# wanzysky/SlenderObjDet

Measured on AMD Instinct MI355X. Metric: training img/sec FCOS R50-FPN 1333x800, higher is better.
Workload: dtype bf16; 1 GPU; FCOS R50-FPN (FCOSV2, giou, center-sampling 1.5), fwd+bwd+SGD, synthetic 1333x800 padded to 800x1344 (BASELINE.json configs[1]); global_batch=16, parallelism=dp1

## Files before the change

### include/slender_hip.h

```cpp
#ifndef SLENDER_HIP_H_
#define SLENDER_HIP_H_

#ifdef __cplusplus
extern "C" {
#endif

#define SOD_MAX_LEVELS 8
#define SOD_CONV_MAX_LEVELS 6

#define SOD_CONV_RELU 1
#define SOD_CONV_RES_UP2 2
#define SOD_CONV_CWIN 4

#define SOD_IOU_LOSS_IOU 0
#define SOD_IOU_LOSS_LINEAR 1
#define SOD_IOU_LOSS_GIOU 2

const char* sod_version(void);
int sod_stream_create_cumask(const unsigned* mask_words, int nwords, void** out_stream);
int sod_stream_destroy(void* stream);
int sod_debug_occupy(int wgs, int usec, void* stream);

long long sod_reduce_workspace_bytes(void);

int sod_conv2d_fwd(const void* x, const void* w, const float* bias, const void* res, void* y,
                   int N, int H, int W, int C, int K, int R, int S, int stride, int pad, int dil,
                   long long x_img_stride, long long y_img_stride, long long res_img_stride,
                   int flags, int out_f32, void* stream);
int sod_conv2d_dgrad(const void* dy, const void* wt, const void* accum, const void* relu_mask, void* dx,
                     int N, int H, int W, int C, int K, int R, int S, int stride, int pad, int dil,
                     long long dy_img_stride, long long dx_img_stride, void* stream);
#define SOD_WGRAD_DETERMINISTIC 1
#define SOD_WGRAD_DIAG 2
long long sod_conv2d_wgrad_workspace_bytes(void);
int sod_conv2d_wgrad(const void* dy, const void* x, float* dw, const float* qscale,
                     int N, int H, int W, int C, int K, int R, int S, int stride, int pad, int dil,
                     long long dy_img_stride, long long x_img_stride, int splits, int flags,
                     void* ws, long long ws_bytes, void* stream);

int sod_conv2d_fwd_bits(const void* x, const void* w, const float* bias, const void* res, void* y, void* relu_bits,
                        int N, int H, int W, int C, int K, int R, int S, int stride, int pad, int dil, int flags, void* stream);
int sod_conv2d_dgrad_bits(const void* dy, const void* wt, const void* accum, int accum_even, const void* relu_bits, void* dx,
                          int N, int H, int W, int C, int K, int R, int S, int stride, int pad, int dil, void* stream);

int sod_conv2d_fwd_ml(int nlev, const void* const* x, const void* w, const float* bias, void* const* y,
                      int N, const int* H, const int* W, int C, int K, int R, int S, int stride, int pad, int dil,
                      long long y_img_stride, int flags, int out_f32, void* stream);
int sod_conv2d_fwd_ml_gnsum(int nlev, const void* const* x, const void* w, const float* bias, void* const* y,
                            int N, const int* H, const int* W, int C, int K, int R, int S, int stride, int pad, int dil,
                            long long y_img_stride, int flags, float* gn_sums, int G, void* stream);
int sod_conv2d_dgrad_ml(int nlev, const void* const* dy, const void* wt, void* const* dx,
                        int N, const int* H, const int* W, int C, int K, int R, int S, int stride, int pad, int dil,
                        long long dy_img_stride, void* stream);
int sod_conv2d_dgrad_ml_mask(int nlev, const void* const* dy, const void* wt, const void* const* relu_mask, void* const* dx,
                             int N, const int* H, const int* W, int C, int K, int R, int S, int stride, int pad, int dil,
                             long long dy_img_stride, void* stream);
int sod_conv2d_dgrad_ml_kpitch(int nlev, const void* const* dy, const void* wt_pad, void* const* dx,
                               int N, const int* H, const int* W, int C, int Kp, int Kpitch, int R, int S, int pad, int dil,
                               long long dy_img_stride, void* stream);
int sod_conv2d_dgrad_ml_accum(int nlev, const void* const* dy, const void* wt, const void* const* accum, const void* const* relu_mask,
                              void* const* dx, int N, const int* H, const int* W, int C, int K, int R, int S, int stride, int pad, int dil,
                              long long dy_img_stride, void* stream);
int sod_conv2d_wgrad_ml(int nlev, const void* const* dy, const void* const* x, float* dw, const float* qscale,
                        int N, const int* H, const int* W, int C, int K, int R, int S, int stride, int pad, int dil,
                        long long dy_img_stride, int splits, int flags, void* ws, long long ws_bytes, void* stream);
int sod_conv2d_dgrad_cwin(const void* dy, const void* wt_win, const void* relu_mask, void* dx,
                          int N, int H, int W, int C, int K, int R, int S, int stride, int pad, int dil, void* stream);
int sod_conv_set_tile256(int mode);
int sod_conv_set_pw(int on);
int sod_conv_set_ws3(int mode);
int sod_conv_set_wgrad_variant(int variant);
int sod_conv_set_reverse(int on);
int sod_conv_last_variant(void);
int sod_conv_prof_enable(int on);
int sod_conv_prof_collect(float* ms, int* variant, float* frac, int* mode, int max);

int sod_groupnorm_fwd(const void* x, const float* gamma, const float* beta, void* y, float* mean_rstd,
                      int N, int HW, int C, int G, long long img_stride, float eps, int relu,
                      float* det_ws, long long det_ws_bytes, void* stream);
int sod_groupnorm_bwd(const void* dy, const void* x, const float* gamma, const float* beta, const float* mean_rstd,
                      void* dx, float* dgamma, float* dbeta, float* dxsum , float* red_ws ,
                      int N, int HW, int C, int G, long long img_stride, int relu, float* det_ws, long long det_ws_bytes, void* stream);
int sod_groupnorm_fwd_ml(int nlev, const void* const* x, const float* gamma, const float* beta, void* const* y, float* mean_rstd,
                         int N, const int* hw, int C, int G, float eps, int relu, float* det_ws, long long det_ws_bytes, void* stream);
int sod_groupnorm_apply_ml(int nlev, const void* const* x, const float* gamma, const float* beta, void* const* y, float* sums_to_mean_rstd,
                           int N, const int* hw, int C, int G, float eps, int relu, void* stream);
int sod_groupnorm_bwd_ml(int nlev, const void* const* dy, const void* const* x, const float* gamma, const float* beta,
                         const float* mean_rstd, void* const* dx, float* dgamma, float* dbeta, float* dxsum, float* red_ws,
                         int N, const int* hw, int C, int G, int relu, float* det_ws, long long det_ws_bytes, void* stream);

int sod_relu_fwd(const void* x, void* y, long long n, void* stream);
int sod_relu_bwd(const void* dy, const void* y, void* dx, long long n, void* stream);
int sod_add_bf16(const void* a, const void* b, void* out, long long n, void* stream);
int sod_add_up2_bf16(const void* a, const void* b, void* out, int N, int H, int W, int C, void* stream);
int sod_bias_grad(const void* dy, float* dbias, int N, int HW, int C, long long img_stride, float* det_ws, long long det_ws_bytes, void* stream);
int sod_bias_grad_scaled(const void* dy, float* dbias, const float* scale_num, const float* scale_den, float den_mul, float den_min,
                         int N, int HW, int C, long long img_stride, float* det_ws, long long det_ws_bytes, void* stream);
int sod_bias_grad_ml(int nlev, const void* const* dy, float* dbias, int N, const int* hw, int C, void* stream);
int sod_maxpool3x3s2(const void* x, void* y, int N, int H, int W, int C, void* stream);
int sod_upsample2x_bwd(const void* g, void* dprev, int N, int Hc, int Wc, int C, void* stream);

int sod_weight_prep(const float* w, const float* scale, void* w_krsc, void* w_crsk, int K, int RS, int C, int Cpad, void* stream);
int sod_weight_prep_batched(const float* params, const float* scales, const void* table_dev, int n, long long total_elems,
                            void* krsc_arena, void* crsk_arena, void* stream);
int sod_scale_rows(float* g, const float* scale, int K, long long row, void* stream);

int sod_sgd_step(float* params, const float* grads, float* momentum_buf, const void* segments_dev, int nseg,
                 const float* lr_dev, float lr, float momentum, int nesterov, int first_step, float grad_scale, void* stream);

int sod_adaptive_step(float* params, const float* grads, float* exp_avg, float* exp_avg_sq, const void* segments_dev, int nseg,
                      int mode, float lr, float beta1, float beta2, float eps, float bias_correction1, float bias_correction2_sqrt,
                      float grad_scale, void* stream);

int sod_preprocess_image(const void* img, int is_uint8, int C, int H, int W, void* out, int Hp, int Wp, int Cpad,
                         const float* mean3, const float* std3, void* stream);
int sod_preprocess_batch(int n, const void* const* imgs, int is_uint8, int C, const int* H, const int* W, void* out, int Hp, int Wp,
                         int Cpad, const float* mean3, const float* std3, void* stream);
int sod_stem_fused(int n, const void* const* imgs, const int* H, const int* W, const void* w_packed, const float* bias,
                   void* out, int Hp, int Wp, const float* mean3, const float* std3, void* stream);
int sod_bottleneck_frozen_fwd(const void* x, int N, int H, int W, int Cin, const void* w1, const float* b1, const void* w2,
                              const float* b2, const void* w3, const float* b3, const void* wsc, void* out, void* stream);
int sod_resize_flip_preprocess_batch(int n, const void* const* imgs, const int* H, const int* W, const int* newH, const int* newW,
                                     const int* const* xbounds, const int* const* xcoef, const int* kx,
                                     const int* const* ybounds, const int* const* ycoef, const int* ky, const int* flip,
                                     void* out, int Hp, int Wp, int Cpad, const float* mean3, const float* std3, void* stream);
int sod_nchw_f32_to_nhwc_bf16(const float* x, void* y, int N, int C, int HW, void* stream);

int sod_sigmoid_focal_loss_fwd(const float* logits, const int* labels, const float* dense_targets,
                               long long M, int K, int ld, float alpha, float gamma, float* elem_out,
                               float* sum_out, float* ws, void* stream);
int sod_sigmoid_focal_loss_fwd_grad(const float* logits, const int* labels, long long M, int K, int ld, float alpha, float gamma,
                                    float* sum_out, float* ws, void* dlogits_bf16, int ld_out, void* stream);
int sod_sigmoid_focal_loss_bwd(const float* logits, const int* labels, const float* dense_targets,
                               long long M, int K, int ld, float alpha, float gamma,
                               const float* scale_num, const float* scale_den, float den_mul, float den_min,
                               void* dlogits, int ld_out, int out_bf16, void* stream);
int sod_iou_loss_fwd(const float* pred, const float* target, const float* weight, const int* mask, int mask_bg,
                     long long P, int loss_type, float* elem_out, float* sum_out, float* ws, void* stream);
int sod_iou_loss_bwd(const float* pred, const float* target, const float* weight, const int* mask, int mask_bg,
                     long long P, int loss_type, const float* grad_scale, float* dpred, void* stream);
int sod_fcos_assign(const float* boxes, const int* classes, const int* box_offsets, int N,
                    int nlevels, const int* lvl_h, const int* lvl_w, const int* lvl_stride,
                    const float* lvl_lo, const float* lvl_hi, float radius, int num_classes,
                    int* labels, float* reg_targets, float* ctr_targets, float* stats, float* ws, void* stream);
int sod_fcos_regctr_loss_fwd(const float* box_raw, int ld_box, const float* ctr_logit, int ld_ctr,
                             const int* labels, const float* reg_targets, const float* ctr_targets,
                             const float* scales, int N, int nlevels, const int* lvl_h, const int* lvl_w,
                             const int* lvl_stride, int num_classes, int loss_type, int norm_reg_targets,
                             float* sums, float* ws, void* stream);
int sod_fcos_regctr_loss_bwd(const float* box_raw, int ld_box, const float* ctr_logit, int ld_ctr,
                             const int* labels, const float* reg_targets, const float* ctr_targets,
                             const float* scales, int N, int nlevels, const int* lvl_h, const int* lvl_w,
                             const int* lvl_stride, int num_classes, int loss_type, int norm_reg_targets,
                             const float* grad_reg, const float* grad_ctr, const float* norm, float inv_world,
                             void* dbox, int ld_out, int ctr_col, void* dctr, int ld_dctr, int dctr_col,
                             float* dscales, float* ws, void* stream);
int sod_fcos_assign_topk(const float* boxes, const int* classes, const int* box_offsets, int N,
                         int nlevels, const int* lvl_h, const int* lvl_w, const int* lvl_stride,
                         const float* lvl_lo, const float* lvl_hi, float radius, int num_classes, int topk,
                         int* labels, float* reg_targets, float* ctr_targets, int* gt_index, unsigned char* sel,
                         float* stats3, float* ws, void* stream);
int sod_fcos_regctr_loss_sel_fwd(const float* box_raw, int ld_box, const float* ctr_logit, int ld_ctr,
                                 const int* labels, const float* reg_targets, const float* ctr_targets,
                                 const float* scales, int N, int nlevels, const int* lvl_h, const int* lvl_w,
                                 const int* lvl_stride, int num_classes, int loss_type, int norm_reg_targets,
                                 const unsigned char* sel, float* sums, float* ws, void* stream);
int sod_fcos_regctr_loss_sel_bwd(const float* box_raw, int ld_box, const float* ctr_logit, int ld_ctr,
                                 const int* labels, const float* reg_targets, const float* ctr_targets,
                                 const float* scales, int N, int nlevels, const int* lvl_h, const int* lvl_w,
                                 const int* lvl_stride, int num_classes, int loss_type, int norm_reg_targets,
                                 const unsigned char* sel,
                                 const float* grad_reg, const float* grad_ctr, const float* norm, float inv_world,
                                 void* dbox, int ld_out, int ctr_col, void* dctr, int ld_dctr, int dctr_col,
                                 float* dscales, float* ws, void* stream);
int sod_fcos_finalize_losses(const float* focal_sum, const float* regctr_sums, const float* stats,
                             float inv_world, float* out3, void* stream);

long long sod_nms_workspace_bytes(int n);
int sod_nms(const float* boxes, const long long* order, int n, float iou_threshold, long long* keep, int* num_keep,
            void* mask_ws, void* stream);
int sod_fcos_decode(const float* cls_logits, int ld_cls, const float* box_raw, int ld_box, const float* scales,
                    int N, int nlev, const int* H, const int* W, const int* strides, int num_classes,
                    int ctr_col_box, int ctr_col_cls, int norm_reg_targets, float pre_nms_thresh, int pre_nms_top_n,
                    float* out_boxes, float* out_scores, int* out_classes, int* out_counts, void* stream);
int sod_dense_topk_select(const float* logits, int ld, int N, int nlev, const int* rows, int num_classes, int by_row_max,
                          float score_thresh, int top_n, int* out_rows, float* out_scores, int* out_classes, int* out_counts, void* stream);
long long sod_batched_nms_workspace_bytes(int B, int M, int box_dim);
int sod_batched_nms_prepare(const float* boxes, const float* scores, const int* classes, int B, int M, int box_dim, void* ws, void* stream);
int sod_batched_nms_run(const long long* order, int B, int M, int box_dim, float iou_threshold, int max_keep, long long* keep, int* num_keep,
                        void* ws, void* stream);
int sod_rpn_clip_filter(float* boxes, float* scores, const float* image_hw, int B, int M, int box_dim, float min_size, int* bad_count,
                        void* stream);
int sod_nms_rotated(const float* boxes, const long long* order, int n, float iou_threshold, long long* keep, int* num_keep,
                    void* mask_ws, void* stream);
int sod_box_iou_rotated(const float* boxes1, int n1, const float* boxes2, int n2, float* iou_out, void* stream);
int sod_roi_align_fwd(const void* x, const float* rois, float* out, int R, int N, int H, int W, int C, int PH, int PW,
                      float spatial_scale, int sampling_ratio, int rotated, void* stream);
int sod_roi_align_fwd_f32(const float* x, const float* rois, float* out, int R, int N, int H, int W, int C, int PH, int PW,
                          float spatial_scale, int sampling_ratio, int rotated, void* stream);
int sod_roi_align_bwd(const float* dout, const float* rois, float* dx, int R, int N, int H, int W, int C, int PH, int PW,
                      float spatial_scale, int sampling_ratio, int rotated, void* stream);
int sod_giou_loss_xyxy(const float* boxes1, const float* boxes2, long long P, float eps, float* elem_out, float* sum_out,
                       const float* grad_scale, float* dboxes1, float* ws, void* stream);
int sod_smooth_l1_loss(const float* input, const float* target, long long n, float beta, float* elem_out, float* sum_out,
                       const float* grad_scale, float* dinput, float* ws, void* stream);
int sod_anchor_match(const float* gt_boxes, int G, const float* anchors, int A, float thr_lo, float thr_hi,
                     int label_below, int label_between, int label_above, int allow_low_quality,
                     float* matched_vals, int* matches, signed char* labels, unsigned* gt_best_ws, void* stream);

int sod_deform_conv_fwd_fused(const void* x, const float* offset, const float* mask, const void* w, const float* bias, void* y,
                              int N, int H, int W, int C, int K, int KH, int KW, int stride, int pad, int dil, int deformable_groups,
                              int off_ld, int mask_ld, int mask_is_logit, int relu, void* stream);
int sod_deform_conv_fwd_f32(const float* x, const float* offset, const float* mask, const float* w, const float* bias, float* y,
                            int N, int H, int W, int C, int K, int KH, int KW, int stride, int pad, int dil, int deformable_groups,
                            int off_ld, int mask_ld, int mask_is_logit, void* stream);
int sod_deform_conv_wgrad_fused(const void* dy, const void* x, const float* offset, const float* mask, float* dw, const float* qscale,
                                int N, int H, int W, int C, int K, int KH, int KW, int stride, int pad, int dil, int deformable_groups,
                                int off_ld, int mask_ld, int mask_is_logit, void* ws, long long ws_bytes, void* stream);
int sod_deform_im2col(const void* x, const float* offset, const float* mask, void* cols,
                      int N, int H, int W, int C, int KH, int KW, int stride, int pad, int dil, int deformable_groups,
                      int off_ld, int mask_ld, int mask_is_logit, void* stream);
int sod_deform_conv_bwd_fused(const void* dy, const void* wt, const void* x, const float* offset, const float* mask, float* dx_f32,
                              float* doffset, float* dmask, float* wnorm_ws, int N, int H, int W, int C, int K, int KH, int KW, int stride,
                              int pad, int dil, int deformable_groups, int off_ld, int mask_ld, int mask_is_logit, void* stream);
int sod_deform_conv_set_window_counter(unsigned long long* device_counter);
int sod_deform_conv_set_window_slack(int pixels);
int sod_deform_conv_bwd_fused_supported(int C, int K, int KH, int KW, int stride, int dil, int deformable_groups);
int sod_deform_col2im(const void* dcols, const void* x, const float* offset, const float* mask,
                      float* dx_f32, float* doffset, float* dmask,
                      int N, int H, int W, int C, int KH, int KW, int stride, int pad, int dil, int deformable_groups,
                      int off_ld, int mask_ld, int mask_is_logit, void* stream);

int sod_deform_im2col_f32(const float* x, const float* offset, const float* mask, float* cols,
                          int N, int H, int W, int C, int KH, int KW, int stride, int pad, int dil, int deformable_groups,
                          int off_ld, int mask_ld, int mask_is_logit, void* stream);
int sod_deform_col2im_f32(const float* dcols, const float* x, const float* offset, const float* mask,
                          float* dx_f32, float* doffset, float* dmask,
                          int N, int H, int W, int C, int KH, int KW, int stride, int pad, int dil, int deformable_groups,
                          int off_ld, int mask_ld, int mask_is_logit, void* stream);
int sod_f32_to_bf16(const float* x, void* y, long long n, void* stream);

int sod_retina_targets(const float* anchors, int A, const float* gt_boxes, const int* gt_classes, int G, const int* matches,
                       const signed char* match_labels, int num_classes, const float* weights4, int* gt_labels, float* gt_deltas,
                       void* stream);
int sod_retina_box_loss_fwd(const float* pred, int pitch, const int* gt_labels, const float* gt_deltas, int N, int R, int A,
                            int num_classes, float beta, float* sums2, float* normalizer, float momentum, float* ws, void* stream);
int sod_retina_box_loss_bwd(const float* pred, int pitch, const int* gt_labels, const float* gt_deltas, int N, int R, int A,
                            int num_classes, float beta, const float* grad_num, const float* grad_den, void* dpred_bf16, void* stream);

int sod_anchor_match_rotated(const float* gt_boxes, int G, const float* anchors, int A, float thr_lo, float thr_hi,
                             int label_below, int label_between, int label_above, int allow_low_quality,
                             float* matched_vals, int* matches, signed char* labels, unsigned* gt_best_ws, void* stream);
int sod_roi_label_batched(const float* boxes, const int* counts, int N, int R, int box_dim, const float* gt_boxes, const int* gt_classes,
                          const int* gt_off, float iou_threshold, int label_below, int label_above, int num_classes, int* matches,
                          signed char* classes, void* stream);
int sod_box2box_get_deltas(const float* src, const float* tgt, long long n, int box_dim, const float* weights, float* deltas, void* stream);
int sod_box2box_apply_deltas(const float* deltas, const float* boxes, long long n, int k, int box_dim, int ld, const float* weights,
                             float scale_clamp, float* out, void* stream);
int sod_bce_logits_loss_fwd(const float* logits, const signed char* labels, long long n, float* sum_out, float* ws, void* stream);
int sod_bce_logits_loss_bwd(const float* logits, const signed char* labels, long long n, const float* grad_scale, float scale_mul,
                            float* dlogits, void* stream);
int sod_bce_logits_soft_fwd(const float* logits, const float* targets, const int* labels, int bg_label, long long n, float* sum_out,
                            float* ws, void* stream);
int sod_bce_logits_soft_bwd(const float* logits, const float* targets, const int* labels, int bg_label, long long n,
                            const float* grad_scale, float scale_mul, float* dlogits, void* stream);
int sod_rpn_loc_loss_fwd(const float* pred, const float* target, const signed char* labels, long long n, int box_dim, float beta,
                         float* sum_out, float* ws, void* stream);
int sod_rpn_loc_loss_bwd(const float* pred, const float* target, const signed char* labels, long long n, int box_dim, float beta,
                         const float* grad_scale, float scale_mul, float* dpred, void* stream);
int sod_softmax_ce_fwd(const float* scores, const int* labels, int R, int C, int ld, float* sum_out, float* ws, void* stream);
int sod_softmax_ce_bwd(const float* scores, const int* labels, int R, int C, int ld, const float* grad_scale, float scale_mul,
                       float* dscores, void* stream);
int sod_fastrcnn_box_loss_fwd(const float* pred, const int* gt_classes, const float* gt_deltas, int R, int K, int box_dim, int ld,
                              float beta, float* sum_out, float* ws, void* stream);
int sod_fastrcnn_box_loss_bwd(const float* pred, const int* gt_classes, const float* gt_deltas, int R, int K, int box_dim, int ld,
                              float beta, const float* grad_scale, float scale_mul, float* dpred, void* stream);

int sod_reppoints_dcn_offset(const float* pts, float* out, long long rows, int ld, int num_points, float scale, int subtract_base,
                             int flip_xy, void* stream);
int sod_points2bbox_fwd(const float* pts, const float* add, int ld, int N, int H, int W, float grid_stride, float point_stride,
                        int num_points, float* boxes, long long box_img_stride, unsigned* argidx, long long arg_img_stride, void* stream);
int sod_points2bbox_bwd(const float* dboxes, long long box_img_stride, const unsigned* argidx, long long arg_img_stride, int ld,
                        int N, int H, int W, float point_stride, int num_points, float* dpts_f32, void* dpts_bf16, void* stream);
int sod_points2bbox_moment_fwd(const float* pts, const float* add, int ld, int N, int H, int W, float grid_stride, float point_stride,
                               int num_points, const float* moment_transfer, float* boxes, long long box_img_stride, void* stream);
int sod_points2bbox_moment_bwd(const float* dboxes, long long box_img_stride, const float* pts, const float* add, int ld, int N, int H,
                               int W, float grid_stride, float point_stride, int num_points, const float* moment_transfer,
                               float moment_mul, float* dpts_f32, void* dpts_bf16, float* dmoment2, void* stream);
int sod_reppoints_point_match(const float* centers, const float* strides, int X, const int* lvl_start, int num_levels,
                              const float* gt_boxes, const int* box_offsets, int N, int max_gt, int mode, float scale,
                              int* objectness, float* box_labels, void* stream);
int sod_reppoints_labels(const int* matches, const signed char* match_labels, const float* gt_boxes, const int* gt_classes,
                         const int* box_offsets, const float* centers, const float* image_hw, int N, int X, int num_classes,
                         int* cls_labels, float* refine_boxes, int* objectness, void* stream);
int sod_reppoints_box_loss_fwd(const float* pred, const float* target, const int* labels, const float* strides, int N, int X,
                               int bg_label, float beta, float* sums2, float* ws, void* stream);
int sod_reppoints_box_loss_bwd(const float* pred, const float* target, const int* labels, const float* strides, int N, int X,
                               int bg_label, float beta, const float* grad_num, const float* grad_den, float den_min, float mul,
                               float* dpred, void* stream);
int sod_reppoints_finalize(const float* focal_sum, const float* init_sums2, const float* refine_sums2, float* normalizer,
                           float momentum, int num_images, float init_weight, float* out3, void* stream);

int sod_retina_giou_loss_fwd(const float* pred, int pitch, const int* gt_labels, const float* anchors, const float* matched_boxes,
                             int N, int R, int A, int num_classes, const float* weights4, float scale_clamp, float* sums2,
                             float* normalizer, float momentum, float* ws, void* stream);
int sod_retina_giou_loss_bwd(const float* pred, int pitch, const int* gt_labels, const float* anchors, const float* matched_boxes,
                             int N, int R, int A, int num_classes, const float* weights4, float scale_clamp,
                             const float* grad_num, const float* grad_den, void* dpred_bf16, void* stream);

int sod_border_align_fwd(const float* feature, const float* boxes, float* out, int B, int C, int K, int H, int W, int pool_size,
                         void* stream);
int sod_border_align_bwd(const float* dout, const float* feature, const float* boxes, float* dfeature, int B, int C, int K, int H,
                         int W, int pool_size, void* stream);
int sod_corner_pool_fwd(const float* x, float* y, long long planes, int H, int W, int mode, void* stream);
int sod_corner_pool_bwd(const float* x, const float* dy, float* dx, long long planes, int H, int W, int mode, int tie_latest,
                        void* stream);

int sod_sample_labels(const signed char* labels, int N, int R, int num_samples, float positive_fraction, int bg_label,
                      unsigned long long seed, signed char* out, int* counts, void* stream);
int sod_sample_labels_list(const signed char* labels, int N, int R, int num_samples, float positive_fraction, int bg_label,
                           unsigned long long seed, signed char* out, int* counts, int* idx, int* list_n, void* stream);
int sod_compact_samples(const signed char* mask, int N, int R, int S, int* idx, int* num, void* stream);

int sod_rpn_gather_sampled(int nlev, const void* const* logits, const void* const* deltas, const int* hw, const int* logit_pitch,
                           const int* delta_pitch, const int* idx, int N, int S, int A, int D, float* row_logits, float* row_deltas,
                           void* stream);
int sod_rpn_scatter_sampled(int nlev, void* const* dlogits, void* const* ddeltas, const int* hw, const int* logit_pitch,
                            const int* delta_pitch, const int* idx, int N, int S, int A, int D, const float* row_dlogits,
                            const float* row_ddeltas, void* stream);

int sod_conv2d_fwd_f32(const float* x, const float* w_krsc, const float* bias, const float* res, float* y, int N, int H, int W, int C, int K,
                       int R, int S, int stride, int pad, int dil, long long x_img_stride, long long y_img_stride, int flags, void* stream);
int sod_conv2d_dgrad_f32(const float* dy, const float* w_krsc, const float* accum, const float* relu_mask, float* dx, int N, int H, int W, int C,
                         int K, int R, int S, int stride, int pad, int dil, long long dy_img_stride, int accum_even, void* stream);
int sod_conv2d_wgrad_f32(const float* dy, const float* x, float* dw, const float* qscale, int N, int H, int W, int C, int K, int R, int S,
                         int stride, int pad, int dil, long long dy_img_stride, long long x_img_stride, void* stream);
int sod_groupnorm_fwd_f32(const float* x, const float* gamma, const float* beta, float* y, float* mean_rstd, int N, int HW, int C, int G,
                          float eps, int relu, void* stream);
int sod_groupnorm_bwd_f32(const float* dy, const float* x, const float* gamma, const float* beta, const float* mean_rstd, float* dx,
                          float* dgamma, float* dbeta, float* dxsum, int N, int HW, int C, int G, int relu, void* stream);
int sod_eltwise_f32(int op, const float* a, const float* b, float* out, long long n, void* stream);
int sod_add_up2_f32(const float* a, const float* b, float* out, int N, int H, int W, int C, void* stream);
int sod_upsample2x_bwd_f32(const float* g, float* dprev, int N, int Hc, int Wc, int C, void* stream);
int sod_maxpool3x3s2_f32(const float* x, float* y, int N, int H, int W, int C, void* stream);
int sod_bias_grad_f32(const float* dy, float* dbias, int N, int HW, int C, long long img_stride, void* stream);
int sod_preprocess_image_f32(const void* img, int is_uint8, int C, int H, int W, float* out, int Hp, int Wp, int Cpad, const float* mean3,
                             const float* std3, void* stream);
int sod_weight_prep_f32(const float* w, const float* scale, float* w_krsc, float* w_crsk, int K, int RS, int C, int Cpad, void* stream);
int sod_retina_box_loss_bwd_f32(const float* pred, int pitch, const int* gt_labels, const float* gt_deltas, int N, int R, int A,
                                int num_classes, float beta, const float* grad_num, const float* grad_den, float* dpred, void* stream);
int sod_retina_giou_loss_bwd_f32(const float* pred, int pitch, const int* gt_labels, const float* anchors, const float* matched_boxes,
                                 int N, int R, int A, int num_classes, const float* weights4, float scale_clamp,
                                 const float* grad_num, const float* grad_den, float* dpred, void* stream);
int sod_fcos_regctr_loss_bwd_f32(const float* box_raw, int ld_box, const float* ctr_logit, int ld_ctr, const int* labels,
                                 const float* reg_targets, const float* ctr_targets, const float* scales, int N, int nlevels, const int* lvl_h,
                                 const int* lvl_w, const int* lvl_stride, int num_classes, int loss_type, int norm_reg_targets,
                                 const float* grad_reg, const float* grad_ctr, const float* norm, float inv_world, void* dbox, int ld_out,
                                 int ctr_col, void* dctr, int ld_dctr, int dctr_col, float* dscales, float* ws, void* stream);
int sod_fcos_regctr_loss_sel_bwd_f32(const float* box_raw, int ld_box, const float* ctr_logit, int ld_ctr, const int* labels,
                                     const float* reg_targets, const float* ctr_targets, const float* scales, int N, int nlevels,
                                     const int* lvl_h, const int* lvl_w, const int* lvl_stride, int num_classes, int loss_type,
                                     int norm_reg_targets, const unsigned char* sel, const float* grad_reg, const float* grad_ctr,
                                     const float* norm, float inv_world, void* dbox, int ld_out, int ctr_col, void* dctr, int ld_dctr,
                                     int dctr_col, float* dscales, float* ws, void* stream);

long long sod_coco_match_scratch_doubles(int num_gts, int max_det);
int sod_coco_match(const int* gt_off, const double* gt_box, const unsigned char* gt_crowd, const double* gt_ratio, const int* dt_off,
                   const float* dt_box, int num_seg, int num_img, int max_det, const double* iou_thr, int T, const double* ranges, int A,
                   const long long* scratch_off, double* scratch, unsigned long long* dt_matched, unsigned long long* dt_ignored,
                   int* npig, void* stream);
int sod_coco_accumulate(const int* cat_off, const long long* order, const float* score, const int* rank,
                        const unsigned long long* dt_matched, const unsigned long long* dt_ignored, const int* npig, int K, int T, int A,
                        const int* max_dets, int M, const double* rec_thr, int R, double* precision, double* recall, double* scores,
                        void* stream);
long long sod_proposal_ar_scratch_floats(int num_gts, int limit);
int sod_proposal_ar(const int* gt_off, const float* gt_box, const int* gt_cls, const float* gt_ratio, const int* dt_off,
                    const long long* dt_order, const float* dt_box, const int* dt_cls, int num_img, int limit, int K1, const float* thr,
                    int T, const float* ratio_rng, int R, const float* area_rng, int A, const long long* scratch_off, float* scratch,
                    int* hits, int* counts, float* recalls, void* stream);

long long sod_coco_match_rotated_scratch_floats(int num_gts, int max_det);
int sod_coco_match_rotated(const int* gt_off, const float* gt_box5, const unsigned char* gt_crowd, const double* gt_val,
                           const int* dt_off, const float* dt_box5, const double* dt_val, int num_seg, int num_img, int max_det,
                           const double* iou_thr, int T, const double* ranges, int A, const long long* scratch_off, float* scratch,
                           unsigned long long* dt_matched, unsigned long long* dt_ignored, int* npig, void* stream);

#ifdef __cplusplus
}
#endif
#endif
```

### slenderobjdet_amd/_C.py

```python
import ctypes
import os
from ctypes import c_char_p, c_float, c_int, c_longlong, c_void_p

_HERE = os.path.dirname(os.path.abspath(__file__))
LIB_PATH = os.environ.get("SOD_HIP_LIB") or os.path.join(_HERE, "libslender_hip.so")

_lib = None

_P = c_void_p
_I = c_int
_L = c_longlong
_F = c_float

_SIGS = {
    "sod_conv2d_fwd": [_P, _P, _P, _P, _P, _I, _I, _I, _I, _I, _I, _I, _I, _I, _I, _L, _L, _L, _I, _I, _P],
    "sod_conv2d_dgrad": [_P, _P, _P, _P, _P, _I, _I, _I, _I, _I, _I, _I, _I, _I, _I, _L, _L, _P],
    "sod_conv2d_fwd_bits": [_P, _P, _P, _P, _P, _P, _I, _I, _I, _I, _I, _I, _I, _I, _I, _I, _I, _P],
    "sod_conv2d_dgrad_bits": [_P, _P, _P, _I, _P, _P, _I, _I, _I, _I, _I, _I, _I, _I, _I, _I, _P],
    "sod_conv2d_wgrad": [_P, _P, _P, _P, _I, _I, _I, _I, _I, _I, _I, _I, _I, _I, _L, _L, _I, _I, _P, _L, _P],
    "sod_conv2d_wgrad_workspace_bytes": [],
    "sod_conv2d_fwd_ml": [_I, _P, _P, _P, _P, _I, _P, _P, _I, _I, _I, _I, _I, _I, _I, _L, _I, _I, _P],
    "sod_conv2d_fwd_ml_gnsum": [_I, _P, _P, _P, _P, _I, _P, _P, _I, _I, _I, _I, _I, _I, _I, _L, _I, _P, _I, _P],
    "sod_groupnorm_apply_ml": [_I, _P, _P, _P, _P, _P, _I, _P, _I, _I, _F, _I, _P],
    "sod_conv2d_dgrad_ml": [_I, _P, _P, _P, _I, _P, _P, _I, _I, _I, _I, _I, _I, _I, _L, _P],
    "sod_conv2d_dgrad_ml_mask": [_I, _P, _P, _P, _P, _I, _P, _P, _I, _I, _I, _I, _I, _I, _I, _L, _P],
    "sod_conv2d_dgrad_ml_kpitch": [_I, _P, _P, _P, _I, _P, _P, _I, _I, _I, _I, _I, _I, _I, _L, _P],
    "sod_conv2d_dgrad_ml_accum": [_I, _P, _P, _P, _P, _P, _I, _P, _P, _I, _I, _I, _I, _I, _I, _I, _L, _P],
    "sod_conv2d_wgrad_ml": [_I, _P, _P, _P, _P, _I, _P, _P, _I, _I, _I, _I, _I, _I, _I, _L, _I, _I, _P, _L, _P],
    "sod_groupnorm_fwd": [_P, _P, _P, _P, _P, _I, _I, _I, _I, _L, _F, _I, _P, _L, _P],
    "sod_groupnorm_bwd": [_P, _P, _P, _P, _P, _P, _P, _P, _P, _P, _I, _I, _I, _I, _L, _I, _P, _L, _P],
    "sod_groupnorm_fwd_ml": [_I, _P, _P, _P, _P, _P, _I, _P, _I, _I, _F, _I, _P, _L, _P],
    "sod_groupnorm_bwd_ml": [_I, _P, _P, _P, _P, _P, _P, _P, _P, _P, _P, _I, _P, _I, _I, _I, _P, _L, _P],
    "sod_relu_fwd": [_P, _P, _L, _P],
    "sod_relu_bwd": [_P, _P, _P, _L, _P],
    "sod_add_bf16": [_P, _P, _P, _L, _P],
    "sod_add_up2_bf16": [_P, _P, _P, _I, _I, _I, _I, _P],
    "sod_bias_grad": [_P, _P, _I, _I, _I, _L, _P, _L, _P],
    "sod_bias_grad_scaled": [_P, _P, _P, _P, _F, _F, _I, _I, _I, _L, _P, _L, _P],
    "sod_bias_grad_ml": [_I, _P, _P, _I, _P, _I, _P],
    "sod_maxpool3x3s2": [_P, _P, _I, _I, _I, _I, _P],
    "sod_upsample2x_bwd": [_P, _P, _I, _I, _I, _I, _P],
    "sod_conv2d_dgrad_cwin": [_P, _P, _P, _P, _I, _I, _I, _I, _I, _I, _I, _I, _I, _I, _P],
    "sod_conv_set_tile256": [_I],
    "sod_conv_set_pw": [_I],
    "sod_conv_set_ws3": [_I],
    "sod_conv_set_wgrad_variant": [_I],
    "sod_conv_set_reverse": [_I],
    "sod_conv_last_variant": [],
    "sod_conv_prof_enable": [_I],
    "sod_conv_prof_collect": [_P, _P, _P, _P, _I],
    "sod_weight_prep_batched": [_P, _P, _P, _I, _L, _P, _P, _P],
    "sod_weight_prep": [_P, _P, _P, _P, _I, _I, _I, _I, _P],
    "sod_scale_rows": [_P, _P, _I, _L, _P],
    "sod_sgd_step": [_P, _P, _P, _P, _I, _P, _F, _F, _I, _I, _F, _P],
    "sod_adaptive_step": [_P, _P, _P, _P, _P, _I, _I, _F, _F, _F, _F, _F, _F, _F, _P],
    "sod_preprocess_image": [_P, _I, _I, _I, _I, _P, _I, _I, _I, _P, _P, _P],
    "sod_preprocess_batch": [_I, _P, _I, _I, _P, _P, _P, _I, _I, _I, _P, _P, _P],
    "sod_nchw_f32_to_nhwc_bf16": [_P, _P, _I, _I, _I, _P],
    "sod_stem_fused": [_I, _P, _P, _P, _P, _P, _P, _I, _I, _P, _P, _P],
    "sod_bottleneck_frozen_fwd": [_P, _I, _I, _I, _I, _P, _P, _P, _P, _P, _P, _P, _P, _P],
    "sod_resize_flip_preprocess_batch": [_I, _P, _P, _P, _P, _P, _P, _P, _P, _P, _P, _P, _P, _P, _I, _I, _I, _P, _P, _P],
    "sod_sigmoid_focal_loss_fwd": [_P, _P, _P, _L, _I, _I, _F, _F, _P, _P, _P, _P],
    "sod_sigmoid_focal_loss_fwd_grad": [_P, _P, _L, _I, _I, _F, _F, _P, _P, _P, _I, _P],
    "sod_sigmoid_focal_loss_bwd": [_P, _P, _P, _L, _I, _I, _F, _F, _P, _P, _F, _F, _P, _I, _I, _P],
    "sod_iou_loss_fwd": [_P, _P, _P, _P, _I, _L, _I, _P, _P, _P, _P],
    "sod_iou_loss_bwd": [_P, _P, _P, _P, _I, _L, _I, _P, _P, _P],
    "sod_fcos_assign": [_P, _P, _P, _I, _I, _P, _P, _P, _P, _P, _F, _I, _P, _P, _P, _P, _P, _P],
    "sod_fcos_regctr_loss_fwd": [_P, _I, _P, _I, _P, _P, _P, _P, _I, _I, _P, _P, _P, _I, _I, _I, _P, _P, _P],
    "sod_fcos_regctr_loss_bwd": [_P, _I, _P, _I, _P, _P, _P, _P, _I, _I, _P, _P, _P, _I, _I, _I, _P, _P, _P, _F,
                                 _P, _I, _I, _P, _I, _I, _P, _P, _P],
    "sod_fcos_assign_topk": [_P, _P, _P, _I, _I, _P, _P, _P, _P, _P, _F, _I, _I, _P, _P, _P, _P, _P, _P, _P, _P],
    "sod_fcos_regctr_loss_sel_fwd": [_P, _I, _P, _I, _P, _P, _P, _P, _I, _I, _P, _P, _P, _I, _I, _I, _P, _P, _P, _P],
    "sod_fcos_regctr_loss_sel_bwd": [_P, _I, _P, _I, _P, _P, _P, _P, _I, _I, _P, _P, _P, _I, _I, _I, _P, _P, _P, _P, _F,
                                     _P, _I, _I, _P, _I, _I, _P, _P, _P],
    "sod_fcos_finalize_losses": [_P, _P, _P, _F, _P, _P],
    "sod_nms_workspace_bytes": [_I],
    "sod_fcos_decode": [_P, _I, _P, _I, _P, _I, _I, _P, _P, _P, _I, _I, _I, _I, _F, _I, _P, _P, _P, _P, _P],
    "sod_dense_topk_select": [_P, _I, _I, _I, _P, _I, _I, _F, _I, _P, _P, _P, _P, _P],
    "sod_batched_nms_workspace_bytes": [_I, _I, _I],
    "sod_batched_nms_prepare": [_P, _P, _P, _I, _I, _I, _P, _P],
    "sod_batched_nms_run": [_P, _I, _I, _I, _F, _I, _P, _P, _P, _P],
    "sod_rpn_clip_filter": [_P, _P, _P, _I, _I, _I, _F, _P, _P],
    "sod_nms": [_P, _P, _I, _F, _P, _P, _P, _P],
    "sod_nms_rotated": [_P, _P, _I, _F, _P, _P, _P, _P],
    "sod_box_iou_rotated": [_P, _I, _P, _I, _P, _P],
    "sod_roi_align_fwd": [_P, _P, _P, _I, _I, _I, _I, _I, _I, _I, _F, _I, _I, _P],
    "sod_roi_align_fwd_f32": [_P, _P, _P, _I, _I, _I, _I, _I, _I, _I, _F, _I, _I, _P],
    "sod_roi_align_bwd": [_P, _P, _P, _I, _I, _I, _I, _I, _I, _I, _F, _I, _I, _P],
    "sod_giou_loss_xyxy": [_P, _P, _L, _F, _P, _P, _P, _P, _P, _P],
    "sod_smooth_l1_loss": [_P, _P, _L, _F, _P, _P, _P, _P, _P, _P],
    "sod_anchor_match": [_P, _I, _P, _I, _F, _F, _I, _I, _I, _I, _P, _P, _P, _P, _P],
    "sod_retina_targets": [_P, _I, _P, _P, _I, _P, _P, _I, _P, _P, _P, _P],
    "sod_retina_box_loss_fwd": [_P, _I, _P, _P, _I, _I, _I, _I, _F, _P, _P, _F, _P, _P],
    "sod_retina_giou_loss_fwd": [_P, _I, _P, _P, _P, _I, _I, _I, _I, _P, _F, _P, _P, _F, _P, _P],
    "sod_retina_giou_loss_bwd": [_P, _I, _P, _P, _P, _I, _I, _I, _I, _P, _F, _P, _P, _P, _P],
    "sod_retina_box_loss_bwd": [_P, _I, _P, _P, _I, _I, _I, _I, _F, _P, _P, _P, _P],
    "sod_deform_conv_fwd_fused": [_P, _P, _P, _P, _P, _P, _I, _I, _I, _I, _I, _I, _I, _I, _I, _I, _I, _I, _I, _I, _I, _P],
    "sod_deform_conv_fwd_f32": [_P, _P, _P, _P, _P, _P, _I, _I, _I, _I, _I, _I, _I, _I, _I, _I, _I, _I, _I, _I, _P],
    "sod_deform_conv_wgrad_fused": [_P, _P, _P, _P, _P, _P, _I, _I, _I, _I, _I, _I, _I, _I, _I, _I, _I, _I, _I, _I, _P, _L, _P],
    "sod_deform_im2col": [_P, _P, _P, _P, _I, _I, _I, _I, _I, _I, _I, _I, _I, _I, _I, _I, _I, _P],
    "sod_deform_col2im": [_P, _P, _P, _P, _P, _P, _P, _I, _I, _I, _I, _I, _I, _I, _I, _I, _I, _I, _I, _I, _P],
    "sod_deform_im2col_f32": [_P, _P, _P, _P, _I, _I, _I, _I, _I, _I, _I, _I, _I, _I, _I, _I, _I, _P],
    "sod_deform_col2im_f32": [_P, _P, _P, _P, _P, _P, _P, _I, _I, _I, _I, _I, _I, _I, _I, _I, _I, _I, _I, _I, _P],
    "sod_deform_conv_set_window_counter": [_P],
    "sod_deform_conv_set_window_slack": [_I],
    "sod_deform_conv_bwd_fused_supported": [_I, _I, _I, _I, _I, _I, _I],
    "sod_deform_conv_bwd_fused": [_P, _P, _P, _P, _P, _P, _P, _P, _P, _I, _I, _I, _I, _I, _I, _I, _I, _I, _I, _I, _I, _I, _I, _P],
    "sod_f32_to_bf16": [_P, _P, _L, _P],
    "sod_border_align_fwd": [_P, _P, _P, _I, _I, _I, _I, _I, _I, _P],
    "sod_border_align_bwd": [_P, _P, _P, _P, _I, _I, _I, _I, _I, _I, _P],
    "sod_corner_pool_fwd": [_P, _P, _L, _I, _I, _I, _P],
    "sod_corner_pool_bwd": [_P, _P, _P, _L, _I, _I, _I, _I, _P],
    "sod_anchor_match_rotated": [_P, _I, _P, _I, _F, _F, _I, _I, _I, _I, _P, _P, _P, _P, _P],
    "sod_box2box_get_deltas": [_P, _P, _L, _I, _P, _P, _P],
    "sod_box2box_apply_deltas": [_P, _P, _L, _I, _I, _I, _P, _F, _P, _P],
    "sod_bce_logits_loss_fwd": [_P, _P, _L, _P, _P, _P],
    "sod_bce_logits_loss_bwd": [_P, _P, _L, _P, _F, _P, _P],
    "sod_bce_logits_soft_fwd": [_P, _P, _P, _I, _L, _P, _P, _P],
    "sod_bce_logits_soft_bwd": [_P, _P, _P, _I, _L, _P, _F, _P, _P],
    "sod_rpn_loc_loss_fwd": [_P, _P, _P, _L, _I, _F, _P, _P, _P],
    "sod_rpn_loc_loss_bwd": [_P, _P, _P, _L, _I, _F, _P, _F, _P, _P],
    "sod_softmax_ce_fwd": [_P, _P, _I, _I, _I, _P, _P, _P],
    "sod_softmax_ce_bwd": [_P, _P, _I, _I, _I, _P, _F, _P, _P],
    "sod_fastrcnn_box_loss_fwd": [_P, _P, _P, _I, _I, _I, _I, _F, _P, _P, _P],
    "sod_fastrcnn_box_loss_bwd": [_P, _P, _P, _I, _I, _I, _I, _F, _P, _F, _P, _P],
    "sod_reppoints_dcn_offset": [_P, _P, _L, _I, _I, _F, _I, _I, _P],
    "sod_points2bbox_fwd": [_P, _P, _I, _I, _I, _I, _F, _F, _I, _P, _L, _P, _L, _P],
    "sod_points2bbox_bwd": [_P, _L, _P, _L, _I, _I, _I, _I, _F, _I, _P, _P, _P],
    "sod_points2bbox_moment_fwd": [_P, _P, _I, _I, _I, _I, _F, _F, _I, _P, _P, _L, _P],
    "sod_points2bbox_moment_bwd": [_P, _L, _P, _P, _I, _I, _I, _I, _F, _F, _I, _P, _F, _P, _P, _P, _P],
    "sod_reppoints_point_match": [_P, _P, _I, _P, _I, _P, _P, _I, _I, _I, _F, _P, _P, _P],
    "sod_reppoints_labels": [_P, _P, _P, _P, _P, _P, _P, _I, _I, _I, _P, _P, _P, _P],
    "sod_reppoints_box_loss_fwd": [_P, _P, _P, _P, _I, _I, _I, _F, _P, _P, _P],
    "sod_reppoints_box_loss_bwd": [_P, _P, _P, _P, _I, _I, _I, _F, _P, _P, _F, _F, _P, _P],
    "sod_reppoints_finalize": [_P, _P, _P, _P, _F, _I, _F, _P, _P],
    "sod_conv2d_fwd_f32": [_P, _P, _P, _P, _P, _I, _I, _I, _I, _I, _I, _I, _I, _I, _I, _L, _L, _I, _P],
    "sod_conv2d_dgrad_f32": [_P, _P, _P, _P, _P, _I, _I, _I, _I, _I, _I, _I, _I, _I, _I, _L, _I, _P],
    "sod_conv2d_wgrad_f32": [_P, _P, _P, _P, _I, _I, _I, _I, _I, _I, _I, _I, _I, _I, _L, _L, _P],
    "sod_groupnorm_fwd_f32": [_P, _P, _P, _P, _P, _I, _I, _I, _I, _F, _I, _P],
    "sod_groupnorm_bwd_f32": [_P, _P, _P, _P, _P, _P, _P, _P, _P, _I, _I, _I, _I, _I, _P],
    "sod_eltwise_f32": [_I, _P, _P, _P, _L, _P],
    "sod_add_up2_f32": [_P, _P, _P, _I, _I, _I, _I, _P],
    "sod_upsample2x_bwd_f32": [_P, _P, _I, _I, _I, _I, _P],
    "sod_maxpool3x3s2_f32": [_P, _P, _I, _I, _I, _I, _P],
    "sod_bias_grad_f32": [_P, _P, _I, _I, _I, _L, _P],
    "sod_preprocess_image_f32": [_P, _I, _I, _I, _I, _P, _I, _I, _I, _P, _P, _P],
    "sod_weight_prep_f32": [_P, _P, _P, _P, _I, _I, _I, _I, _P],
    "sod_fcos_regctr_loss_bwd_f32": [_P, _I, _P, _I, _P, _P, _P, _P, _I, _I, _P, _P, _P, _I, _I, _I, _P, _P, _P, _F,
                                     _P, _I, _I, _P, _I, _I, _P, _P, _P],
    "sod_fcos_regctr_loss_sel_bwd_f32": [_P, _I, _P, _I, _P, _P, _P, _P, _I, _I, _P, _P, _P, _I, _I, _I, _P, _P, _P, _P, _F,
                                         _P, _I, _I, _P, _I, _I, _P, _P, _P],
    "sod_sample_labels": [_P, _I, _I, _I, _F, _I, ctypes.c_ulonglong, _P, _P, _P],
    "sod_sample_labels_list": [_P, _I, _I, _I, _F, _I, ctypes.c_ulonglong, _P, _P, _P, _P, _P],
    "sod_compact_samples": [_P, _I, _I, _I, _P, _P, _P],
    "sod_roi_label_batched": [_P, _P, _I, _I, _I, _P, _P, _P, _F, _I, _I, _I, _P, _P, _P],
    "sod_rpn_gather_sampled": [_I, _P, _P, _P, _P, _P, _P, _I, _I, _I, _I, _P, _P, _P],
    "sod_rpn_scatter_sampled": [_I, _P, _P, _P, _P, _P, _P, _I, _I, _I, _I, _P, _P, _P],
    "sod_retina_box_loss_bwd_f32": [_P, _I, _P, _P, _I, _I, _I, _I, _F, _P, _P, _P, _P],
    "sod_retina_giou_loss_bwd_f32": [_P, _I, _P, _P, _P, _I, _I, _I, _I, _P, _F, _P, _P, _P, _P],
    "sod_reduce_workspace_bytes": [],
    "sod_version": [],
    "sod_stream_create_cumask": [_P, _I, _P],
    "sod_stream_destroy": [_P],
    "sod_debug_occupy": [_I, _I, _P],
    "sod_coco_match_scratch_doubles": [_I, _I],
    "sod_coco_match": [_P, _P, _P, _P, _P, _P, _I, _I, _I, _P, _I, _P, _I, _P, _P, _P, _P, _P, _P],
    "sod_coco_accumulate": [_P, _P, _P, _P, _P, _P, _P, _I, _I, _I, _P, _I, _P, _I, _P, _P, _P, _P],
    "sod_proposal_ar_scratch_floats": [_I, _I],
    "sod_proposal_ar": [_P, _P, _P, _P, _P, _P, _P, _P, _I, _I, _I, _P, _I, _P, _I, _P, _I, _P, _P, _P, _P, _P, _P],
    "sod_coco_match_rotated_scratch_floats": [_I, _I],
    "sod_coco_match_rotated": [_P, _P, _P, _P, _P, _P, _P, _I, _I, _I, _P, _I, _P, _I, _P, _P, _P, _P, _P, _P],
}
_RESTYPES = {"sod_reduce_workspace_bytes": c_longlong, "sod_conv2d_wgrad_workspace_bytes": c_longlong, "sod_nms_workspace_bytes": c_longlong, "sod_batched_nms_workspace_bytes": c_longlong, "sod_version": c_char_p,
             "sod_coco_match_scratch_doubles": c_longlong, "sod_proposal_ar_scratch_floats": c_longlong,
             "sod_coco_match_rotated_scratch_floats": c_longlong}


class SlenderHipError(RuntimeError):
    pass


def exported_symbols():
    return sorted(_SIGS)


def load():
    global _lib
    if _lib is not None:
        return _lib
    if not os.path.exists(LIB_PATH):
        raise SlenderHipError(
            f"{LIB_PATH} is missing: build it with `python -c 'import __graft_entry__ as g; g.build()'` "
            "(make -C slenderobjdet_amd/csrc). There is no CPU fallback for the HIP ops."
        )
    import torch

    lib = ctypes.CDLL(LIB_PATH)
    for name, argtypes in _SIGS.items():
        fn = getattr(lib, name)
        fn.argtypes = argtypes
        fn.restype = _RESTYPES.get(name, c_int)
    _lib = lib
    return lib


_ERRS = {-1: "SOD_EARG (bad argument / unsupported shape)", -2: "SOD_ESIZE (operand exceeds 2 GiB)", -3: "SOD_EALIGN"}


def call(name, *args):
    rc = getattr(load(), name)(*args)
    if rc != 0:
        raise SlenderHipError(f"{name} failed: {_ERRS.get(rc, 'hipError_t %d' % rc)}")


def ptr(t):
    if t is None:
        return None
    return ctypes.c_void_p(t.data_ptr())


def stream_ptr(stream=None):
    import torch

    return ctypes.c_void_p((stream if stream is not None else torch.cuda.current_stream()).cuda_stream)


def reduce_workspace_floats():
    return int(load().sod_reduce_workspace_bytes()) // 4
```

### slenderobjdet_amd/csrc/conv_args.h

```cpp
#pragma once
#include "common.h"
#include "../../include/slender_hip.h"
#include <stdlib.h>

namespace sodconv {

enum { MODE_FWD = 0, MODE_DGRAD = 1 };
enum {
  F_BIAS = 1, F_RELU = 2, F_RES = 4, F_RES_UP2 = 8, F_MASK = 16,
  F_WBITS = 64,
  F_MASKBITS = 128,
  F_GNSTATS = 32,
  F_REVERSE = 1024,
  F_RES_EVEN = 512,
};
constexpr int MAXLEV = SOD_CONV_MAX_LEVELS;

struct LevelGeo {
  const void* src;
  void* dst;
  const void* res;
  const void* mask;
  void* bits;
  float* gn_sum;
  uint32_t src_bytes;
  int Hs, Ws, Hp, Wp, P;
  int tile0;
  int pstart;
  int src_img_stride, dst_img_stride, res_img_stride;
  FastDiv div_hw, div_w;
};

struct ConvArgs {
  LevelGeo lev[MAXLEV];
  int nlev;
  const void* w;
  const float* bias;
  uint32_t w_bytes;
  int N, Cred, Nout;
  int R, S, stride, pad, dil;
  int Kred, T;
  int flags;
  int nq_tiles, np_tiles;
  FastDiv div_cpt , div_s, div_stride;
  FastDiv div_rs;
  int gn_G;
  int tap_inner;
  int Cpitch;
  int cwin;
};

inline int conv_tap_inner(int dflt) { return dflt; }

struct GnAcc {
  float s, ss;
  int n;
};
__device__ __forceinline__ void gn_acc_flush(const GnAcc& g, float* sums, int G, int grp) {
  if (g.n >= 0) {
    atomicAdd(sums + ((size_t)g.n * G + grp) * 2, g.s);
    atomicAdd(sums + ((size_t)g.n * G + grp) * 2 + 1, g.ss);
  }
}
__device__ __forceinline__ void gn_acc_add(GnAcc& g, int n, const bf16x8_t& o, float* sums, int G, int grp) {
  float s = 0.f, ss = 0.f;
#pragma unroll
  for (int e = 0; e < 8; ++e) { const float f = (float)o[e]; s += f; ss += f * f; }
  if (n != g.n) { gn_acc_flush(g, sums, G, grp); g.n = n; g.s = 0.f; g.ss = 0.f; }
  g.s += s; g.ss += ss;
}
template <int LPR>
__device__ __forceinline__ void gn_acc_finish(GnAcc& g, uint32_t pa, uint32_t pb, uint32_t P, const FastDiv& div_hw, float* sums, int G, int grp,
                                              bool qok, int lane) {
  if (pa >= P) return;
  if (pb >= P) pb = P - 1;
  const int na = (int)fd_div(pa, div_hw), nb = (int)fd_div(pb, div_hw);
  if (na == nb) {
    float s = (g.n >= 0) ? g.s : 0.f, ss = (g.n >= 0) ? g.ss : 0.f;
#pragma unroll
    for (int o = LPR; o < 64; o <<= 1) { s += __shfl_xor(s, o, 64); ss += __shfl_xor(ss, o, 64); }
    if (lane < LPR && qok) {
      atomicAdd(sums + ((size_t)na * G + grp) * 2, s);
      atomicAdd(sums + ((size_t)na * G + grp) * 2 + 1, ss);
    }
  } else if (qok) {
    gn_acc_flush(g, sums, G, grp);
  }
}

enum ConvTile { TILE_16x256, TILE_64x256, TILE_64x256_K32, TILE_128x128, TILE_128x128_K32 };
int launch_conv128(const ConvArgs& a, int mode, bool out_f32, ConvTile tile, bool generic, hipStream_t st, int* variant);

bool conv256_supported(const ConvArgs& a, int mode);
int launch_conv256(const ConvArgs& a, int mode, bool out_f32, int max_pt_tiles, hipStream_t st);

bool pw_supported(const ConvArgs& a, int mode, bool out_f32, int cus);
int launch_pw(const ConvArgs& a, int mode, hipStream_t st);

bool ws3_supported(const ConvArgs& a, int mode, bool out_f32, int cus, bool any_size);
int launch_ws3(const ConvArgs& a, int mode, hipStream_t st);

struct WLevel {
  const void* dy;
  const void* x;
  uint32_t dy_bytes, x_bytes;
  int Hx, Wx, Ho, Wo, P;
  int v0;
  int dy_img_stride, x_img_stride;
  FastDiv div_hw, div_w;
};

struct WgradArgs {
  WLevel lev[MAXLEV];
  int nlev;
  float* dw;
  const float* qscale;
  int dbg_plain_store;
  float* partial;
  int det;
  int N, C, K;
  int R, S, stride, pad, dil;
  int V, nz, v_per_split;
  int QT, CT;
  FastDiv div_s;
  int diag;
};

enum { WGRAD_DETERMINISTIC = 1, WGRAD_DIAG = 2 };

int launch_wgrad128(WgradArgs& a, int cus, int splits, float* ws, long long ws_bytes, hipStream_t st);
int launch_wgrad_reduce(const WgradArgs& a, hipStream_t st);

bool wgrad256_supported(const WgradArgs& a);
long long wgrad256_workspace_bytes(const WgradArgs& a, int cus);
int launch_wgrad256(WgradArgs& a, int cus, float* ws, long long ws_bytes, hipStream_t st);

bool wgrad9_supported(const WgradArgs& a);
long long wgrad9_workspace_bytes(const WgradArgs& a, int cus);
int wgrad9_tiles_per_block(const WgradArgs& a, int cus);
int launch_wgrad9(const WgradArgs& a, int cus, float* ws, long long ws_bytes, hipStream_t st);

bool wgrad_fold_supported(const WgradArgs& a);
int launch_wgrad_fold(WgradArgs& a, int cus, hipStream_t st);

int launch_wgrad_ring(const WgradArgs& a, int variant, hipStream_t st);

}
```

### slenderobjdet_amd/csrc/conv_dispatch.hip

```cpp
#include "conv_args.h"
#include <stdlib.h>
#include <atomic>
#include <algorithm>

using namespace sodconv;

int device_cus() {
  static const int cus = [] {
    int dev = 0, n = 0;
    if (hipGetDevice(&dev) != hipSuccess || hipDeviceGetAttribute(&n, hipDeviceAttributeMultiprocessorCount, dev) != hipSuccess || n <= 0) n = 256;
    return n;
  }();
  return cus;
}

namespace {

thread_local int g_last_variant = 0;
thread_local int g_conv_reverse = 0;

struct ConvKnobs {
  int conv256 = -1;
  int pw = -1;
  int ws3 = -1;
// ... 185 lines not shown
}

int dispatch_wgrad(WgradArgs& a, int splits, int flags, hipStream_t st, float* ws, long long ws_bytes) {
  const int cus = device_cus();
  a.det = (flags & WGRAD_DETERMINISTIC) ? 1 : 0;
  a.diag = (flags & WGRAD_DIAG) ? 1 : 0;
  if (a.diag && (a.C != a.K || (a.C & 127) || splits < 0)) return SOD_EARG;
  if (splits == -2 && (!ws || !wgrad9_supported(a) || wgrad9_workspace_bytes(a, cus) > ws_bytes)) return SOD_EARG;
  if (splits == -2 || (splits == 0 && use_wgrad9(a, ws, ws_bytes)))
    return timed(st, 9009, 1.f, 2, [&] { return launch_wgrad9(a, cus, ws, ws_bytes, st); });
  if (splits == -1 && (!ws || !wgrad256_supported(a) || wgrad256_workspace_bytes(a, cus) > ws_bytes)) return SOD_EARG;
  if (splits == -1 || (splits == 0 && !a.diag && use_wgrad256(a, ws, ws_bytes)))
    return timed(st, 256, 1.f, 2, [&] { return launch_wgrad256(a, cus, ws, ws_bytes, st); });
  if (splits == 0 && wgrad_fold_supported(a))
    return timed(st, 32004, 1.f, 2, [&] { return launch_wgrad_fold(a, cus, st); });
  a.QT = (a.K + 127) / 128; a.CT = a.diag ? 1 : (a.C + 127) / 128;
  const int tiles = a.QT * a.CT * a.R * a.S;
  int V = 0;
  long long Ptot = 0;
  for (int l = 0; l < a.nlev; ++l) {
    a.lev[l].v0 = V;
    V += (a.lev[l].P + 63) / 64 * 64;
    Ptot += a.lev[l].P;
  }
  a.V = V;
  const int variant = ring_variant_for(a, tiles, splits, ws, ws_bytes);
  if (variant > 0) {
    const int G = (variant % 10000) / 1000;
    int epi = (variant / 10) % 10;
    long long total = splits > 0 ? splits : (long long)G * std::max(1, (G == 1 ? 2 : 1) * cus / tiles);
    const long long maxs = (Ptot + 255) / 256;
    if (total > maxs) total = maxs;
    if (total < 1) total = 1;
    int vps = (int)((V + total - 1) / total);
    vps = (vps + 63) / 64 * 64;
    const int nsplit = (V + vps - 1) / vps;
    a.v_per_split = vps;
    a.nz = (nsplit + G - 1) / G;
    a.dbg_plain_store = 0;
    const long long need = (long long)a.nz * tiles * 128 * 128 * (long long)sizeof(float);
    if (a.det || epi == 1) {
      if (!ws || need > ws_bytes) {
        if (a.det) return SOD_EARG;
        epi = 0;
      }
    }
    a.partial = (a.det || epi == 1) ? ws : nullptr;
    const int v = variant - ((variant / 10) % 10) * 10 + (a.partial ? 10 : 0);
    return timed(st, v % 10000, 1.f, 2, [&] {
      const int rc = launch_wgrad_ring(a, v, st);
      return rc || !a.partial ? rc : launch_wgrad_reduce(a, st);
    });
  }
  return timed(st, 32003, 1.f, 2, [&] { return launch_wgrad128(a, cus, splits, ws, ws_bytes, st); });
}

int fill_wlevel(WgradArgs& a, int l, const void* dy, const void* x, int H, int W, long long dy_img_stride, long long x_img_stride) {
  if (!dy || !x || H <= 0 || W <= 0) return SOD_EARG;
  const int Ho = out_size(H, a.pad, a.dil, a.R, a.stride), Wo = out_size(W, a.pad, a.dil, a.S, a.stride);
  if (Ho <= 0 || Wo <= 0) return SOD_EARG;
  if (dy_img_stride <= 0) dy_img_stride = (long long)Ho * Wo * a.K;
  if (x_img_stride <= 0) x_img_stride = (long long)H * W * a.C;
  const unsigned long long yb = (unsigned long long)a.N * dy_img_stride * 2ull, xb = (unsigned long long)a.N * x_img_stride * 2ull;
  if (yb >= 0x80000000ull || xb >= 0x80000000ull || (long long)a.N * Ho * Wo >= (1ll << 30)) return SOD_ESIZE;
  WLevel& g = a.lev[l];
  g.dy = dy; g.x = x; g.dy_bytes = (uint32_t)yb; g.x_bytes = (uint32_t)xb;
  g.Hx = H; g.Wx = W; g.Ho = Ho; g.Wo = Wo; g.P = a.N * Ho * Wo;
  g.dy_img_stride = (int)dy_img_stride; g.x_img_stride = (int)x_img_stride;
  g.div_hw = make_fastdiv((uint32_t)(Ho * Wo));
  g.div_w = make_fastdiv((uint32_t)Wo);
  return SOD_OK;
}


struct Geo {
  int N;
  const int *H, *W;
  int C, K, R, S, stride, pad, dil;
};

bool out_positive(const Geo& g, int l) {
  return out_size(g.H[l], g.pad, g.dil, g.R, g.stride) > 0 && out_size(g.W[l], g.pad, g.dil, g.S, g.stride) > 0;
}

struct FwdExtra {
  const void* res = nullptr;
  long long res_img_stride = 0;
  void* relu_bits = nullptr;
  float* gn_sums = nullptr;
  int G = 0;
  long long x_img_stride = 0;
  bool reverse = false;
};

int conv_fwd(int nlev, const void* const* x, const void* w, const float* bias, void* const* y, const Geo& g, long long y_img_stride,
             int flags, int out_f32, const FwdExtra& e, void* stream) {
  ConvArgs a{};
  const bool cwin = (flags & SOD_CONV_CWIN) != 0;
  int rc = fill_common(a, nlev, g.N, cwin ? 128 : g.C, g.K, g.R, g.S, g.stride, g.pad, g.dil);
  if (rc) return rc;
  if (cwin) { a.Cpitch = g.C; a.cwin = 1; }
  for (int l = 0; l < nlev; ++l) {
    if (!out_positive(g, l)) return SOD_EARG;
    rc = fill_level(a, l, x[l], y[l], g.H[l], g.W[l], out_size(g.H[l], g.pad, g.dil, g.R, g.stride), out_size(g.W[l], g.pad, g.dil, g.S, g.stride),
                    e.x_img_stride, y_img_stride, out_f32 ? 4 : 2);
    if (rc) return rc;
    if (e.gn_sums) a.lev[l].gn_sum = e.gn_sums + (size_t)l * g.N * e.G * 2;
  }
  a.w = w; a.bias = bias;
  a.gn_G = e.G;
  a.flags = (bias ? F_BIAS : 0) | ((flags & SOD_CONV_RELU) ? F_RELU : 0) | (e.gn_sums ? F_GNSTATS : 0);
  if (e.res) {
    LevelGeo& v = a.lev[0];
    v.res = e.res;
    if (flags & SOD_CONV_RES_UP2) {
      if ((v.Hp & 1) || (v.Wp & 1)) return SOD_EARG;
      a.flags |= F_RES_UP2;
      v.res_img_stride = (int)(e.res_img_stride > 0 ? e.res_img_stride : (long long)(v.Hp / 2) * (v.Wp / 2) * g.K);
    } else {
      a.flags |= F_RES;
      v.res_img_stride = (int)(e.res_img_stride > 0 ? e.res_img_stride : v.dst_img_stride);
    }
  }
  if (e.relu_bits) { a.flags |= F_WBITS; a.lev[0].bits = e.relu_bits; }
  if (e.reverse) a.flags |= F_REVERSE;
  hipStream_t st = (hipStream_t)stream;
  if (e.gn_sums) {
    hipError_t err = hipMemsetAsync(e.gn_sums, 0, sizeof(float) * 2 * (size_t)g.N * e.G * nlev, st);
    if (err != hipSuccess) return (int)err;
  }
  return dispatch_conv(a, MODE_FWD, out_f32 != 0, st);
}

struct DgradExtra {
  const void* const* accum = nullptr;
  bool accum_even = false;
  const void* const* mask = nullptr;
  bool mask_bits = false;
  int Cpitch = 0;
  bool cwin = false;
  long long dx_img_stride = 0;
  bool reverse = false;
};

int conv_dgrad(int nlev, const void* const* dy, const void* wt, void* const* dx, const Geo& g, long long dy_img_stride, const DgradExtra& e,
               void* stream) {
  ConvArgs a{};
  int rc = fill_common(a, nlev, g.N, g.K, g.C, g.R, g.S, g.stride, g.pad, g.dil);
  if (rc) return rc;
  if (e.Cpitch > 0) a.Cpitch = e.Cpitch;
  a.cwin = e.cwin ? 1 : 0;
  for (int l = 0; l < nlev; ++l) {
    if (!out_positive(g, l) || (e.accum && !e.accum[l]) || (e.mask && !e.mask[l])) return SOD_EARG;
    rc = fill_level(a, l, dy[l], dx[l], out_size(g.H[l], g.pad, g.dil, g.R, g.stride), out_size(g.W[l], g.pad, g.dil, g.S, g.stride), g.H[l], g.W[l],
                    dy_img_stride, e.dx_img_stride, 2);
    if (rc) return rc;
    LevelGeo& v = a.lev[l];
    if (e.accum) { v.res = e.accum[l]; v.res_img_stride = e.accum_even ? (g.H[l] / 2) * (g.W[l] / 2) * g.C : v.dst_img_stride; }
    if (e.mask) v.mask = e.mask[l];
  }
  a.w = wt; a.bias = nullptr;
  a.flags = (e.accum ? (e.accum_even ? F_RES_UP2 | F_RES_EVEN : F_RES) : 0) | (e.mask ? (e.mask_bits ? F_MASKBITS : F_MASK) : 0) |
            (e.reverse ? F_REVERSE : 0);
  return dispatch_conv(a, MODE_DGRAD, false, (hipStream_t)stream);
}

int conv_wgrad(int nlev, const void* const* dy, const void* const* x, float* dw, const float* qscale, const Geo& g, long long dy_img_stride,
               long long x_img_stride, int splits, int flags, void* ws, long long ws_bytes, void* stream) {
  if (!dy || !x || !dw || !g.H || !g.W || nlev <= 0 || nlev > MAXLEV || ws_bytes < 0 || ((uintptr_t)ws & 15)) return SOD_EARG;
  if (g.N <= 0 || g.C <= 0 || g.K <= 0 || (g.C & 7) || (g.K & 7) || g.R <= 0 || g.S <= 0 || g.stride <= 0 || g.dil <= 0 || g.pad < 0) return SOD_EARG;
  WgradArgs a{};
  a.nlev = nlev; a.dw = dw; a.qscale = qscale; a.N = g.N; a.C = g.C; a.K = g.K;
  a.R = g.R; a.S = g.S; a.stride = g.stride; a.pad = g.pad; a.dil = g.dil;
  for (int l = 0; l < nlev; ++l) {
    const int rc = fill_wlevel(a, l, dy[l], x[l], g.H[l], g.W[l], dy_img_stride, x_img_stride);
    if (rc) return rc;
  }
  return dispatch_wgrad(a, splits, flags, (hipStream_t)stream, (float*)ws, ws ? ws_bytes : 0);
}

}

extern "C" int sod_conv2d_fwd(const void* x, const void* w, const float* bias, const void* res, void* y,
                              int N, int H, int W, int C, int K, int R, int S, int stride, int pad, int dil,
                              long long x_img_stride, long long y_img_stride, long long res_img_stride,
                              int flags, int out_f32, void* stream) {
  const Geo g{N, &H, &W, C, K, R, S, stride, pad, dil};
  if (!x || !w || !y || !out_positive(g, 0)) return SOD_EARG;
  if ((flags & SOD_CONV_CWIN) && (C != K || (C & 127))) return SOD_EARG;
  FwdExtra e;
  e.res = res; e.res_img_stride = res_img_stride; e.x_img_stride = x_img_stride; e.reverse = g_conv_reverse != 0;
  return conv_fwd(1, &x, w, bias, &y, g, y_img_stride, flags, out_f32, e, stream);
}

extern "C" int sod_conv2d_fwd_bits(const void* x, const void* w, const float* bias, const void* res, void* y, void* relu_bits,
                                   int N, int H, int W, int C, int K, int R, int S, int stride, int pad, int dil, int flags, void* stream) {
  const Geo g{N, &H, &W, C, K, R, S, stride, pad, dil};
  if (!relu_bits || !x || !w || !y || (K & 7) || !out_positive(g, 0)) return SOD_EARG;
  if (flags & SOD_CONV_CWIN) return SOD_EARG;
  FwdExtra e;
  e.res = res; e.relu_bits = relu_bits; e.reverse = g_conv_reverse != 0;
  return conv_fwd(1, &x, w, bias, &y, g, 0, flags, 0, e, stream);
}

extern "C" int sod_conv2d_fwd_ml(int nlev, const void* const* x, const void* w, const float* bias, void* const* y,
                                 int N, const int* H, const int* W, int C, int K, int R, int S, int stride, int pad, int dil,
                                 long long y_img_stride, int flags, int out_f32, void* stream) {
  if (!x || !w || !y || !H || !W) return SOD_EARG;
  return conv_fwd(nlev, x, w, bias, y, Geo{N, H, W, C, K, R, S, stride, pad, dil}, y_img_stride, flags & SOD_CONV_RELU, out_f32, FwdExtra{}, stream);
}

extern "C" int sod_conv2d_fwd_ml_gnsum(int nlev, const void* const* x, const void* w, const float* bias, void* const* y,
                                       int N, const int* H, const int* W, int C, int K, int R, int S, int stride, int pad, int dil,
                                       long long y_img_stride, int flags, float* gn_sums, int G, void* stream) {
  if (!x || !w || !y || !H || !W || !gn_sums) return SOD_EARG;
  if (G <= 0 || K != G * 8) return SOD_EARG;
  FwdExtra e;
  e.gn_sums = gn_sums; e.G = G;
  return conv_fwd(nlev, x, w, bias, y, Geo{N, H, W, C, K, R, S, stride, pad, dil}, y_img_stride, flags & SOD_CONV_RELU, 0, e, stream);
}

extern "C" int sod_conv2d_dgrad(const void* dy, const void* wt, const void* accum, const void* relu_mask, void* dx,
                                int N, int H, int W, int C, int K, int R, int S, int stride, int pad, int dil,
                                long long dy_img_stride, long long dx_img_stride, void* stream) {
  const Geo g{N, &H, &W, C, K, R, S, stride, pad, dil};
  if (!dy || !wt || !dx || !out_positive(g, 0)) return SOD_EARG;
  DgradExtra e;
  e.accum = accum ? &accum : nullptr; e.mask = relu_mask ? &relu_mask : nullptr;
  e.dx_img_stride = dx_img_stride; e.reverse = g_conv_reverse != 0;
  return conv_dgrad(1, &dy, wt, &dx, g, dy_img_stride, e, stream);
}

extern "C" int sod_conv2d_dgrad_cwin(const void* dy, const void* wt_win, const void* relu_mask, void* dx,
                                     int N, int H, int W, int C, int K, int R, int S, int stride, int pad, int dil, void* stream) {
  const Geo g{N, &H, &W, C, 128, R, S, stride, pad, dil};
  if (!dy || !wt_win || !dx || C != K || (C & 127) || !out_positive(g, 0)) return SOD_EARG;
  DgradExtra e;
  e.mask = relu_mask ? &relu_mask : nullptr; e.Cpitch = K; e.cwin = true;
  return conv_dgrad(1, &dy, wt_win, &dx, g, 0, e, stream);
}

extern "C" int sod_conv2d_dgrad_bits(const void* dy, const void* wt, const void* accum, int accum_even, const void* relu_bits, void* dx,
                                     int N, int H, int W, int C, int K, int R, int S, int stride, int pad, int dil, void* stream) {
  const Geo g{N, &H, &W, C, K, R, S, stride, pad, dil};
  if (!dy || !wt || !dx || !relu_bits || (C & 7)) return SOD_EARG;
  if (accum_even && (!accum || (H & 1) || (W & 1))) return SOD_EARG;
  if (!out_positive(g, 0)) return SOD_EARG;
  DgradExtra e;
  e.accum = accum ? &accum : nullptr; e.accum_even = accum_even != 0;
  e.mask = &relu_bits; e.mask_bits = true;
  return conv_dgrad(1, &dy, wt, &dx, g, 0, e, stream);
}

extern "C" int sod_conv2d_dgrad_ml(int nlev, const void* const* dy, const void* wt, void* const* dx,
                                   int N, const int* H, const int* W, int C, int K, int R, int S, int stride, int pad, int dil,
                                   long long dy_img_stride, void* stream) {
  if (!dy || !wt || !dx || !H || !W) return SOD_EARG;
  return conv_dgrad(nlev, dy, wt, dx, Geo{N, H, W, C, K, R, S, stride, pad, dil}, dy_img_stride, DgradExtra{}, stream);
}

extern "C" int sod_conv2d_dgrad_ml_mask(int nlev, const void* const* dy, const void* wt, const void* const* relu_mask, void* const* dx,
                                        int N, const int* H, const int* W, int C, int K, int R, int S, int stride, int pad, int dil,
                                        long long dy_img_stride, void* stream) {
  if (!dy || !wt || !dx || !relu_mask || !H || !W) return SOD_EARG;
  DgradExtra e;
  e.mask = relu_mask;
  return conv_dgrad(nlev, dy, wt, dx, Geo{N, H, W, C, K, R, S, stride, pad, dil}, dy_img_stride, e, stream);
}

extern "C" int sod_conv2d_dgrad_ml_kpitch(int nlev, const void* const* dy, const void* wt_pad, void* const* dx,
                                          int N, const int* H, const int* W, int C, int Kp, int Kpitch, int R, int S, int pad, int dil,
                                          long long dy_img_stride, void* stream) {
  if (!dy || !wt_pad || !dx || !H || !W || Kpitch <= 0 || (Kpitch & 7) || Kp < Kpitch || (Kp & 63)) return SOD_EARG;
  DgradExtra e;
  e.Cpitch = Kpitch;
  return conv_dgrad(nlev, dy, wt_pad, dx, Geo{N, H, W, C, Kp, R, S, 1, pad, dil}, dy_img_stride, e, stream);
}

extern "C" int sod_conv2d_dgrad_ml_accum(int nlev, const void* const* dy, const void* wt, const void* const* accum, const void* const* relu_mask,
                                         void* const* dx, int N, const int* H, const int* W, int C, int K, int R, int S, int stride, int pad, int dil,
                                         long long dy_img_stride, void* stream) {
  if (!dy || !wt || !dx || !accum || !H || !W) return SOD_EARG;
  DgradExtra e;
  e.accum = accum; e.mask = relu_mask;
  return conv_dgrad(nlev, dy, wt, dx, Geo{N, H, W, C, K, R, S, stride, pad, dil}, dy_img_stride, e, stream);
}

extern "C" int sod_conv2d_wgrad(const void* dy, const void* x, float* dw, const float* qscale,
                                int N, int H, int W, int C, int K, int R, int S, int stride, int pad, int dil,
                                long long dy_img_stride, long long x_img_stride, int splits, int flags,
                                void* ws, long long ws_bytes, void* stream) {
  return conv_wgrad(1, &dy, &x, dw, qscale, Geo{N, &H, &W, C, K, R, S, stride, pad, dil}, dy_img_stride, x_img_stride, splits, flags, ws, ws_bytes,
                    stream);
}

extern "C" long long sod_conv2d_wgrad_workspace_bytes(void) { return 160ll << 20; }

extern "C" int sod_conv2d_wgrad_ml(int nlev, const void* const* dy, const void* const* x, float* dw, const float* qscale,
                                   int N, const int* H, const int* W, int C, int K, int R, int S, int stride, int pad, int dil,
                                   long long dy_img_stride, int splits, int flags, void* ws, long long ws_bytes, void* stream) {
  return conv_wgrad(nlev, dy, x, dw, qscale, Geo{N, H, W, C, K, R, S, stride, pad, dil}, dy_img_stride, 0, splits, flags, ws, ws_bytes, stream);
}

extern "C" int sod_conv_last_variant(void) { return g_last_variant; }

extern "C" int sod_conv_prof_enable(int on) {
  ConvProf& p = g_prof;
  if (on && !p.ev) {
    constexpr int CAP = 8192;
    p.ev = (hipEvent_t*)malloc(sizeof(hipEvent_t) * 2 * CAP);
    p.variant = (int*)malloc(sizeof(int) * CAP);
    p.mode = (int*)malloc(sizeof(int) * CAP);
    p.frac = (float*)malloc(sizeof(float) * CAP);
    if (!p.ev || !p.variant || !p.mode || !p.frac) return SOD_EARG;
    for (int i = 0; i < 2 * CAP; ++i)
      if (hipEventCreate(&p.ev[i]) != hipSuccess) return SOD_EARG;
    p.cap = CAP;
  }
  p.on.store(on ? 1 : 0);
  return SOD_OK;
}

extern "C" int sod_conv_prof_collect(float* ms, int* variant, float* frac, int* mode, int max) {
  ConvProf& p = g_prof;
  const int have = p.n.load();
  const int n = have < max ? have : max;
  if (n > 0 && (!ms || !variant || !frac || !mode)) return SOD_EARG;
  for (int i = 0; i < n; ++i) {
    if (hipEventSynchronize(p.ev[2 * i + 1]) != hipSuccess) return SOD_EARG;
    float t = 0.f;
    if (hipEventElapsedTime(&t, p.ev[2 * i], p.ev[2 * i + 1]) != hipSuccess) return SOD_EARG;
    ms[i] = t; variant[i] = p.variant[i]; frac[i] = p.frac[i]; mode[i] = p.mode[i];
  }
  p.n.store(0);
  return n;
}

extern "C" int sod_conv_set_reverse(int on) {
  g_conv_reverse = on ? 1 : 0;
  return SOD_OK;
}

extern "C" int sod_conv_set_wgrad_variant(int variant) {
  if (variant < -1) return SOD_EARG;
  knobs().wgrad_variant = variant;
  return SOD_OK;
}

extern "C" int sod_conv_set_ws3(int mode) {
  if (mode < -1 || mode > 2) return SOD_EARG;
  knobs().ws3 = mode;
  return SOD_OK;
}

extern "C" int sod_conv_set_pw(int on) {
  if (on < -1 || on > 1) return SOD_EARG;
  knobs().pw = on;
  return SOD_OK;
}

extern "C" int sod_conv_set_tile256(int mode) {
  if (mode < -1 || mode > 2) return SOD_EARG;
  knobs().conv256 = mode;
  return SOD_OK;
}
```

### slenderobjdet_amd/csrc/conv_wgrad9.hip

```cpp
#include "conv_args.h"
#include <stdlib.h>

namespace sodconv {
namespace {

constexpr int G9_D = 3;
constexpr int G9_XROWB = 128, G9_YROWB = 256;
constexpr int G9_NXC = 10, G9_RX = 64 * G9_NXC;
constexpr int G9_XBYTES = (G9_RX + 64) * G9_XROWB;
constexpr int G9_YTILE = 64 * G9_YROWB;
constexpr int G9_LDS = G9_XBYTES + 4 * G9_YTILE;
constexpr int G9_SLAB = 128 * 64 * 9;

#ifndef SOD_W9_ABL
#define SOD_W9_ABL 0
#endif

template <int OFF_LO, int OFF_HI>
__device__ __forceinline__ bf16x8_t tr_read2(uint32_t addr) {
  s16x4_t lo, hi;
#if SOD_W9_ABL & 2
  asm volatile("; no read %0 %1 %2" : "=&v"(lo), "=&v"(hi) : "v"(addr));
#else
  asm volatile("ds_read_b64_tr_b16 %0, %2 offset:%3\n\tds_read_b64_tr_b16 %1, %2 offset:%4"
               : "=&v"(lo), "=&v"(hi) : "v"(addr), "n"(OFF_LO), "n"(OFF_HI));
#endif
  s16x8_t v = {lo[0], lo[1], lo[2], lo[3], hi[0], hi[1], hi[2], hi[3]};
  return __builtin_bit_cast(bf16x8_t, v);
}

#if SOD_W9_ABL & 4
#define G9_MFMA(ACC, A, B) asm volatile("; no mfma %0 %1 %2" : "+v"(ACC) : "v"(A), "v"(B))
#else
#define G9_MFMA(ACC, A, B) ACC = __builtin_amdgcn_mfma_f32_16x16x32_bf16(A, B, ACC, 0, 0, 0)
#endif
#define G9_WAIT_LGKM(N) do { asm volatile("s_waitcnt lgkmcnt(" #N ")" ::: "memory"); __builtin_amdgcn_sched_barrier(0); } while (0)

}

struct W9Level {
  const void* dy;
  const void* x;
  uint32_t dy_bytes, x_bytes;
  int H, W, Wp, HWp;
  int Npad;
  int T, t0;
  int E;
  int dy_img_stride, x_img_stride;
  FastDiv div_hwp, div_wp;
};

struct W9Args {
  W9Level lev[MAXLEV];
  int nlev;
  float* dw;
  const float* qscale;
  float* partial;
  int N, C, K, QT, CT;
  int Ttot, nz, t_per_split;
};

namespace {

__global__ __launch_bounds__(512, 2) void conv_wgrad9_kernel(const W9Args a) {
  extern __shared__ __attribute__((aligned(16))) char smem[];
  const int tid = threadIdx.x, lane = tid & 63;
  const int wave = __builtin_amdgcn_readfirstlane(tid >> 6);
  const int wr = wave >> 2, wc = wave & 3;
  const uint32_t bid = xcd_remap(blockIdx.x, gridDim.x);
  const int tiles = a.QT * a.CT;
  const int tile = (int)(bid % (uint32_t)tiles), z = (int)(bid / (uint32_t)tiles);
  const int ct = tile % a.CT, qt = tile / a.CT;
  const int q0 = qt * 128, c0 = ct * 64;
  const int kt_beg = z * a.t_per_split;
  int kt_end = kt_beg + a.t_per_split; if (kt_end > a.Ttot) kt_end = a.Ttot;

  const int x_row = wave * 8 + (lane >> 3);
  const int x_ps = lane & 7;
  const int x_log = ((((x_ps >> 1) ^ ((x_row >> 1) & 3)) << 1) | (x_ps & 1));
  const uint32_t x_cadd = (uint32_t)(c0 + x_log * 8) * 2u;
  const int y_row0 = wave * 4 + (lane >> 4);
  const int y_ps = lane & 15;
  const int y_log = ((((y_ps >> 1) ^ (y_row0 & 7)) << 1) | (y_ps & 1));
  const uint32_t y_qadd = (uint32_t)(q0 + y_log * 8) * 2u;
  const bool y_live = q0 + y_log * 8 < a.K;

  const int tg = lane >> 4, tq = (lane & 15) >> 2, tp = lane & 3;
  const int il = 4 * tg + tq;
  uint32_t aoff[4];
#pragma unroll
  for (int i = 0; i < 4; ++i) aoff[i] = (uint32_t)G9_XBYTES + (uint32_t)il * G9_YROWB + (uint32_t)(((wr * 4 + i) ^ (il & 7)) << 5) + (uint32_t)tp * 8u;
  const uint32_t bxor = (uint32_t)(wc << 5) | (uint32_t)(tp << 3);

  f32x4_t acc[4][9];
#pragma unroll
  for (int i = 0; i < 4; ++i)
#pragma unroll
    for (int t = 0; t < 9; ++t) acc[i][t] = f32x4_t{0.f, 0.f, 0.f, 0.f};

  for (int lv = 0; lv < a.nlev; ++lv) {
    const W9Level& g = a.lev[lv];
    int sa = (kt_beg > g.t0 ? kt_beg : g.t0) - g.t0;
    int sb = (kt_end < g.t0 + g.T ? kt_end : g.t0 + g.T) - g.t0;
    if (sa >= sb) continue;
    const int T = sb - sa, j0 = sa * 64, E = g.E;
    const int W = g.W, Wp = g.Wp, HWp = g.HWp, sh0 = g.W + 2;
    auto yrsrc = __builtin_amdgcn_make_buffer_rsrc(const_cast<void*>(g.dy), 0, g.dy_bytes, 0x00020000);
    auto xrsrc = __builtin_amdgcn_make_buffer_rsrc(const_cast<void*>(g.x), 0, g.x_bytes, 0x00020000);

    auto pix = [&](int j, uint32_t& n, uint32_t& hw) -> bool {
      if ((unsigned)j >= (unsigned)g.Npad) return false;
      n = fd_div((uint32_t)j, g.div_hwp);
      const uint32_t rem = (uint32_t)j - n * (uint32_t)HWp;
      const uint32_t hp = fd_div(rem, g.div_wp);
      const uint32_t wp = rem - hp * (uint32_t)Wp;
      hw = (hp - 1u) * (uint32_t)W + wp;
      return hp != 0u && wp < (uint32_t)W;
    };
    auto stage_x = [&](int m, int slot) {
      uint32_t n, hw, off = SOD_OOB;
      if (pix(j0 + 64 * m + x_row - sh0, n, hw)) off = (n * (uint32_t)g.x_img_stride + hw * (uint32_t)a.C) * 2u + x_cadd;
      char* dst = smem + (slot * 64 + wave * 8) * G9_XROWB;
      __builtin_amdgcn_raw_ptr_buffer_load_lds(xrsrc, SOD_LDS(dst), 16, off, 0, 0, 0);
      if (slot == 0) __builtin_amdgcn_raw_ptr_buffer_load_lds(xrsrc, SOD_LDS(dst + G9_RX * G9_XROWB), 16, off, 0, 0, 0);
    };
    auto stage_y = [&](int t) {
      char* dst = smem + G9_XBYTES + (t & 3) * G9_YTILE + wave * 4 * G9_YROWB;
#pragma unroll
      for (int k = 0; k < 2; ++k) {
        uint32_t n, hw, off = SOD_OOB;
        if (t < T && y_live && pix(j0 + 64 * t + k * 32 + y_row0, n, hw)) off = (n * (uint32_t)g.dy_img_stride + hw * (uint32_t)a.K) * 2u + y_qadd;
        __builtin_amdgcn_raw_ptr_buffer_load_lds(yrsrc, SOD_LDS(dst + k * 32 * G9_YROWB), 16, off, 0, 0, 0);
      }
    };

    int sh[9];
#pragma unroll
    for (int t = 0; t < 9; ++t) sh[t] = sh0 + (t / 3 - 1) * Wp + (t % 3 - 1);

    int xslot = 0;
    for (int m = 0; m <= E; ++m) { stage_x(m, xslot); xslot = (xslot + 1 == G9_NXC) ? 0 : xslot + 1; }
    stage_y(0);
#pragma unroll
    for (int d = 1; d < G9_D; ++d) {
      stage_x(E + d, xslot); xslot = (xslot + 1 == G9_NXC) ? 0 : xslot + 1;
      stage_y(d);
    }
    const uint32_t hwp_mul = g.div_hwp.mul, hwp_shr = g.div_hwp.shr, wp_mul = g.div_wp.mul, wp_shr = g.div_wp.shr;
    const uint32_t Npad = (uint32_t)g.Npad, xis = (uint32_t)g.x_img_stride, yis = (uint32_t)g.dy_img_stride, aC = (uint32_t)a.C, aK = (uint32_t)a.K;
#define G9_PIX1(J, N_, REM, INR) { const uint32_t j_ = (uint32_t)(J); INR = j_ < Npad; N_ = (__umulhi(j_, hwp_mul) + j_) >> hwp_shr; REM = j_ - N_ * (uint32_t)HWp; }
#define G9_PIX2(REM, HW, OK) { const uint32_t hp_ = (__umulhi(REM, wp_mul) + REM) >> wp_shr; const uint32_t wq_ = REM - hp_ * (uint32_t)Wp; \
                               HW = (hp_ - 1u) * (uint32_t)W + wq_; OK = OK && hp_ != 0u && wq_ < (uint32_t)W; }
#define G9_PIX3(TAB, N_, HW, OK, IS, CH) { const uint32_t v_ = OK ? (N_ * (IS) + HW * (CH)) * 2u : SOD_OOB;                                \
                                           asm volatile("ds_write_b32 %0, %1" :: "v"((uint32_t)(uintptr_t)SOD_LDS(TAB)), "v"(v_) : "memory"); }
    uint32_t* const tab = reinterpret_cast<uint32_t*>(smem + G9_LDS);
    uint32_t pn, prem, phw; bool pok;
    if (wave == 0) {
      G9_PIX1(j0 + 64 * (G9_D + E) + lane - sh0, pn, prem, pok) G9_PIX2(prem, phw, pok) G9_PIX3(tab + lane, pn, phw, pok, xis, aC)
      G9_PIX1(j0 + 64 * G9_D + lane, pn, prem, pok) pok = pok && G9_D < T; G9_PIX2(prem, phw, pok) G9_PIX3(tab + 64 + lane, pn, phw, pok, yis, aK)
    }
#define G9_BADDR(DST, XB, TAP) { int sbt_ = (XB) + sh[TAP]; if (sbt_ >= G9_RX) sbt_ -= G9_RX; const uint32_t row_ = (uint32_t)sbt_ + (uint32_t)il; \
                                 DST = ((row_ << 7) | ((row_ << 4) & 0x60u)) ^ bxor; }
    uint32_t baddr[9];
#pragma unroll
    for (int tap = 0; tap < 9; ++tap) G9_BADDR(baddr[tap], 0, tap)
    int xb = 0;
    asm volatile("s_waitcnt lgkmcnt(0)" ::: "memory");

    for (int t = 0; t < T; ++t) {
#if !(SOD_W9_ABL & 16)
      asm volatile("s_waitcnt vmcnt(6)" ::: "memory");
#endif
#if !(SOD_W9_ABL & 8)
      __builtin_amdgcn_s_barrier();
#endif
      const uint32_t* tb = tab + (t & 1) * 128;
      uint32_t ox, oy0, oy1;
      asm volatile("ds_read_b32 %0, %1" : "=v"(ox) : "v"((uint32_t)(uintptr_t)SOD_LDS(tb + x_row)));
      asm volatile("ds_read_b32 %0, %1" : "=v"(oy0) : "v"((uint32_t)(uintptr_t)SOD_LDS(tb + 64 + y_row0)));
      asm volatile("ds_read_b32 %0, %1 offset:128" : "=v"(oy1) : "v"((uint32_t)(uintptr_t)SOD_LDS(tb + 64 + y_row0)));
      const uint32_t ybase = (uint32_t)((t & 3) * G9_YTILE);
      const int xb_prev = xb;
      xb += 64; if (xb >= G9_RX) xb -= G9_RX;
      const int jn = j0 + 64 * (t + 1);
      const bool ylive = t + 1 + G9_D < T;
      const bool mine = (wave == ((t + 1) & 7));
      uint32_t* const tn = tab + ((t + 1) & 1) * 128 + lane;
      int binc[9];
#pragma unroll
      for (int tap = 0; tap < 9; ++tap) {
        int s0_ = xb_prev + sh[tap]; if (s0_ >= G9_RX) s0_ -= G9_RX;
        binc[tap] = (s0_ + 64 >= G9_RX) ? (64 - G9_RX) * G9_XROWB : 64 * G9_XROWB;
      }

      bf16x8_t af0[4], af1[4], b0, b1, b2;
#pragma unroll
      for (int i = 0; i < 4; ++i) af0[i] = tr_read2<0, 4096>(ybase + aoff[i]);
      b0 = tr_read2<0, 2048>(baddr[0]);
      b1 = tr_read2<0, 2048>(baddr[1]);

#define G9_MMA(AF, B, TAP, WORK)                                                                                   \
  _Pragma("unroll") for (int i = 0; i < 4; ++i)                                                                   \
      G9_MFMA(acc[i][TAP], AF[i], B);                                                                             \
  __builtin_amdgcn_sched_barrier(0);                                                                               \
  WORK                                                                                                             \
  __builtin_amdgcn_sched_barrier(0);
#if !(SOD_W9_ABL & 32)
      __builtin_amdgcn_s_setprio(1);
#endif
      b2 = tr_read2<0, 2048>(baddr[2]);       G9_WAIT_LGKM(4);  G9_MMA(af0, b0, 0, if (mine) G9_PIX1(jn + 64 * (G9_D + E) + lane - sh0, pn, prem, pok))
      {
        char* xd = smem + (xslot * 64 + wave * 8) * G9_XROWB;
#if SOD_W9_ABL & 1
        ox = oy0 = oy1 = SOD_OOB;
#endif
        __builtin_amdgcn_raw_ptr_buffer_load_lds(xrsrc, SOD_LDS(xd), 16, ox + x_cadd, 0, 0, 0);
        if (xslot == 0) __builtin_amdgcn_raw_ptr_buffer_load_lds(xrsrc, SOD_LDS(xd + G9_RX * G9_XROWB), 16, ox + x_cadd, 0, 0, 0);
        xslot = (xslot + 1 == G9_NXC) ? 0 : xslot + 1;
        char* yd = smem + G9_XBYTES + ((t + G9_D) & 3) * G9_YTILE + wave * 4 * G9_YROWB;
        __builtin_amdgcn_raw_ptr_buffer_load_lds(yrsrc, SOD_LDS(yd), 16, y_live ? oy0 + y_qadd : SOD_OOB, 0, 0, 0);
        __builtin_amdgcn_raw_ptr_buffer_load_lds(yrsrc, SOD_LDS(yd + 32 * G9_YROWB), 16, y_live ? oy1 + y_qadd : SOD_OOB, 0, 0, 0);
      }
      __builtin_amdgcn_sched_barrier(0);
      b0 = tr_read2<0, 2048>(baddr[3]);       G9_WAIT_LGKM(4);  G9_MMA(af0, b1, 1, if (mine) G9_PIX2(prem, phw, pok))
      b1 = tr_read2<0, 2048>(baddr[4]);       G9_WAIT_LGKM(4);  G9_MMA(af0, b2, 2, if (mine) G9_PIX3(tn, pn, phw, pok, xis, aC))
      b2 = tr_read2<0, 2048>(baddr[5]);       G9_WAIT_LGKM(4);  G9_MMA(af0, b0, 3, if (mine) { G9_PIX1(jn + 64 * G9_D + lane, pn, prem, pok) pok = pok && ylive; })
      b0 = tr_read2<0, 2048>(baddr[6]);
#pragma unroll
      for (int i = 0; i < 4; ++i) af1[i] = tr_read2<8192, 8192 + 4096>(ybase + aoff[i]);
                                              G9_WAIT_LGKM(12); G9_MMA(af0, b1, 4, if (mine) G9_PIX2(prem, phw, pok))
      b1 = tr_read2<0, 2048>(baddr[7]);       G9_WAIT_LGKM(12); G9_MMA(af0, b2, 5, if (mine) G9_PIX3(tn + 64, pn, phw, pok, yis, aK))
      b2 = tr_read2<0, 2048>(baddr[8]);       G9_WAIT_LGKM(12); G9_MMA(af0, b0, 6, )
      b0 = tr_read2<4096, 6144>(baddr[0]);    G9_WAIT_LGKM(4);  G9_MMA(af0, b1, 7, )
      b1 = tr_read2<4096, 6144>(baddr[1]);    G9_WAIT_LGKM(4);  G9_MMA(af0, b2, 8, )
      b2 = tr_read2<4096, 6144>(baddr[2]);    G9_WAIT_LGKM(4);  G9_MMA(af1, b0, 0, baddr[0] += (uint32_t)binc[0];)
      b0 = tr_read2<4096, 6144>(baddr[3]);    G9_WAIT_LGKM(4);  G9_MMA(af1, b1, 1, baddr[1] += (uint32_t)binc[1];)
      b1 = tr_read2<4096, 6144>(baddr[4]);    G9_WAIT_LGKM(4);  G9_MMA(af1, b2, 2, baddr[2] += (uint32_t)binc[2];)
      b2 = tr_read2<4096, 6144>(baddr[5]);    G9_WAIT_LGKM(4);  G9_MMA(af1, b0, 3, baddr[3] += (uint32_t)binc[3];)
      b0 = tr_read2<4096, 6144>(baddr[6]);    G9_WAIT_LGKM(4);  G9_MMA(af1, b1, 4, baddr[4] += (uint32_t)binc[4];)
      b1 = tr_read2<4096, 6144>(baddr[7]);    G9_WAIT_LGKM(4);  G9_MMA(af1, b2, 5, baddr[5] += (uint32_t)binc[5];)
      b2 = tr_read2<4096, 6144>(baddr[8]);    G9_WAIT_LGKM(4);  G9_MMA(af1, b0, 6, baddr[6] += (uint32_t)binc[6];)
                                              G9_WAIT_LGKM(2);  G9_MMA(af1, b1, 7, baddr[7] += (uint32_t)binc[7];)
                                              G9_WAIT_LGKM(0);  G9_MMA(af1, b2, 8, baddr[8] += (uint32_t)binc[8];)
      __builtin_amdgcn_s_setprio(0);
#undef G9_MMA
    }
#undef G9_PIX1
#undef G9_PIX2
#undef G9_PIX3
#undef G9_BADDR
    asm volatile("s_waitcnt vmcnt(0)" ::: "memory");
    __builtin_amdgcn_s_barrier();
  }

  float* slab = a.partial + ((size_t)z * (size_t)tiles + (size_t)tile) * G9_SLAB + (size_t)wave * (36 * 256) + (size_t)lane * 4;
#pragma unroll
  for (int i = 0; i < 4; ++i)
#pragma unroll
    for (int t = 0; t < 9; ++t) *reinterpret_cast<f32x4_t*>(slab + (i * 9 + t) * 256) = acc[i][t];
}

__global__ __launch_bounds__(256) void wgrad9_reduce_kernel(const W9Args a) {
  const int tiles = a.QT * a.CT;
  const uint32_t idx = blockIdx.x * 256u + threadIdx.x;
  const int lane = idx & 63;
  const uint32_t fi = idx >> 6;
  const int tile = (int)(fi / 288u), frag = (int)(fi % 288u);
  if (tile >= tiles) return;
  const float* src = a.partial + (size_t)tile * G9_SLAB + (size_t)frag * 256 + (size_t)lane * 4;
  const size_t zstride = (size_t)tiles * G9_SLAB;
  f32x4_t s0 = {0.f, 0.f, 0.f, 0.f}, s1 = s0, s2 = s0, s3 = s0;
  int zz = 0;
  for (; zz + 4 <= a.nz; zz += 4) {
    const f32x4_t v0 = *reinterpret_cast<const f32x4_t*>(src + (size_t)zz * zstride);
    const f32x4_t v1 = *reinterpret_cast<const f32x4_t*>(src + (size_t)(zz + 1) * zstride);
    const f32x4_t v2 = *reinterpret_cast<const f32x4_t*>(src + (size_t)(zz + 2) * zstride);
    const f32x4_t v3 = *reinterpret_cast<const f32x4_t*>(src + (size_t)(zz + 3) * zstride);
    s0 += v0; s1 += v1; s2 += v2; s3 += v3;
  }
  for (; zz < a.nz; ++zz) s0 += *reinterpret_cast<const f32x4_t*>(src + (size_t)zz * zstride);
  const f32x4_t sum = (s0 + s1) + (s2 + s3);
  const int wave = frag / 36, i = (frag % 36) / 9, tap = frag % 9;
  const int wr = wave >> 2, wc = wave & 3, fr = lane & 15, fg = lane >> 4;
  const int ct = tile % a.CT, qt = tile / a.CT;
  const int c = ct * 64 + wc * 16 + fr;
#pragma unroll
  for (int e = 0; e < 4; ++e) {
    const int q = qt * 128 + wr * 64 + i * 16 + fg * 4 + e;
    if (q >= a.K) continue;
    float* dst = a.dw + ((size_t)q * 9 + tap) * a.C + c;
    *dst += sum[e] * (a.qscale ? a.qscale[q] : 1.f);
  }
}

int w9_fill(const WgradArgs& a, W9Args& w) {
  w.nlev = a.nlev; w.dw = a.dw; w.qscale = a.qscale; w.N = a.N; w.C = a.C; w.K = a.K;
  w.QT = (a.K + 127) / 128; w.CT = a.C / 64;
  int t0 = 0;
  for (int l = 0; l < a.nlev; ++l) {
    const WLevel& s = a.lev[l];
    W9Level& g = w.lev[l];
    g.dy = s.dy; g.x = s.x; g.dy_bytes = s.dy_bytes; g.x_bytes = s.x_bytes;
    g.H = s.Hx; g.W = s.Wx; g.Wp = s.Wx + 1; g.HWp = (s.Hx + 1) * (s.Wx + 1);
    g.Npad = a.N * g.HWp;
    g.T = (g.Npad + 63) / 64; g.t0 = t0; t0 += g.T;
    g.E = (2 * (s.Wx + 2) + 63) / 64;
    g.dy_img_stride = s.dy_img_stride; g.x_img_stride = s.x_img_stride;
    g.div_hwp = make_fastdiv((uint32_t)g.HWp); g.div_wp = make_fastdiv((uint32_t)g.Wp);
  }
  w.Ttot = t0;
  return t0;
}

}

bool wgrad9_supported(const WgradArgs& a) {
  if (a.R != 3 || a.S != 3 || a.stride != 1 || a.pad != 1 || a.dil != 1 || a.diag) return false;
  if ((a.K & 7) || (a.C & 63) || a.K < 128 || a.C < 64) return false;
  long long tot = 0;
  for (int l = 0; l < a.nlev; ++l) {
    const WLevel& s = a.lev[l];
    if (s.Ho != s.Hx || s.Wo != s.Wx || s.Wx > 190) return false;
    if ((2 * (s.Wx + 2) + 63) / 64 + G9_D + 1 > G9_NXC) return false;
    const long long np = (long long)a.N * (s.Hx + 1) * (s.Wx + 1);
    if (np >= (1ll << 30)) return false;
    tot += np;
  }
  return tot >= 1 && tot < (1ll << 30);
}

static int w9_splits(const W9Args& w, int cus, int* per_out) {
  const int tiles = w.QT * w.CT;
  int nz = cus / tiles; if (nz < 1) nz = 1;
  if (nz > w.Ttot) nz = w.Ttot;
  const int per = (w.Ttot + nz - 1) / nz;
  *per_out = per;
  return (w.Ttot + per - 1) / per;
}

long long wgrad9_workspace_bytes(const WgradArgs& a, int cus) {
  W9Args w{};
  w9_fill(a, w);
  int per = 0;
  const int nz = w9_splits(w, cus, &per);
  return (long long)nz * w.QT * w.CT * G9_SLAB * (long long)sizeof(float);
}

int wgrad9_tiles_per_block(const WgradArgs& a, int cus) {
  W9Args w{};
  w9_fill(a, w);
  int per = 0;
  w9_splits(w, cus, &per);
  return per;
}

int launch_wgrad9(const WgradArgs& a, int cus, float* ws, long long ws_bytes, hipStream_t st) {
  if (!wgrad9_supported(a)) return SOD_EARG;
  W9Args w{};
  w9_fill(a, w);
  int per = 0;
  w.nz = w9_splits(w, cus, &per);
  w.t_per_split = per;
  const int tiles = w.QT * w.CT;
  const long long need = (long long)w.nz * tiles * G9_SLAB * (long long)sizeof(float);
  if (!ws || need > ws_bytes) return SOD_EARG;
  if ((long long)tiles * 18432 >= (1ll << 31)) return SOD_ESIZE;
  w.partial = ws;
  const hipError_t e = sod_max_dynamic_lds_once<conv_wgrad9_kernel>(G9_LDS + 1024);
  if (e != hipSuccess) return (int)e;
  SOD_LAUNCH(conv_wgrad9_kernel, dim3(w.nz * tiles), dim3(512), G9_LDS + 1024, st, w);
  SOD_LAUNCH(wgrad9_reduce_kernel, dim3(tiles * 72), dim3(256), 0, st, w);
  SOD_CHECK_LAUNCH();
  return SOD_OK;
}

}
```

### slenderobjdet_amd/csrc/stem_fused.hip

```cpp
#include "common.h"
#include "../../include/slender_hip.h"

namespace {

constexpr int ST_MAX_IMAGES = 64;
constexpr int ST_PT = 39;
constexpr int ST_PSTR = 48;
constexpr int ST_CT = 17;
constexpr int ST_NPX = ST_CT * ST_CT;
constexpr int ST_OSTR = 72;
constexpr int ST_PATCH_BYTES = 3 * ST_PT * ST_PSTR * 2;
constexpr int ST_LDS = ST_PATCH_BYTES + ST_NPX * ST_OSTR * 2;

struct StemArgs {
  const uint8_t* img[ST_MAX_IMAGES];
  int H[ST_MAX_IMAGES], W[ST_MAX_IMAGES];
  const __bf16* w;
  const float* bias;
  __bf16* out;
  int N, Hc, Wc, Hq, Wq;
  float mean[3], stdv[3];
};

__global__ __launch_bounds__(256) void stem_fused_kernel(const StemArgs a) {
  extern __shared__ __attribute__((aligned(16))) char smem[];
  __bf16* patch = reinterpret_cast<__bf16*>(smem);
  __bf16* cout = reinterpret_cast<__bf16*>(smem + ST_PATCH_BYTES);
  const int tid = threadIdx.x, lane = tid & 63;
  const int wave = __builtin_amdgcn_readfirstlane(tid >> 6);
  const int tx = blockIdx.x, ty = blockIdx.y, n = blockIdx.z;
  const int H = a.H[n], W = a.W[n];
  const uint8_t* __restrict__ img = a.img[n];
  const int cy0 = 16 * ty - 1, cx0 = 16 * tx - 1;
  const int iy0 = 2 * cy0 - 3, ix0 = 2 * cx0 - 3;

  const int fr = lane & 15, fg = lane >> 4;
  bf16x8_t af[4][6];
#pragma unroll
  for (int mi = 0; mi < 4; ++mi)
#pragma unroll
    for (int ks = 0; ks < 6; ++ks) af[mi][ks] = *reinterpret_cast<const bf16x8_t*>(a.w + ((mi * 16 + fr) * 24 + ks * 4 + fg) * 8);

  __bf16* lut = cout;
  for (int i = tid; i < 3 * 256; i += 256) lut[i] = (__bf16)(((float)(i & 255) - a.mean[i >> 8]) / a.stdv[i >> 8]);
  constexpr int PER_THREAD = (3 * ST_PT + 4) / 5;
  const int px = tid % 48, r0 = tid / 48;
  const int ix = ix0 + px;
  const bool colok = tid < 240 && px < ST_PT && (unsigned)ix < (unsigned)W;
  auto irsrc = __builtin_amdgcn_make_buffer_rsrc(const_cast<uint8_t*>(img), 0, (uint32_t)(3 * H * W), 0x00020000);
  uint8_t raw[PER_THREAD];
#pragma unroll
  for (int j = 0; j < PER_THREAD; ++j) {
    const int t = r0 + 5 * j;
    const int c = t >= 2 * ST_PT ? 2 : (t >= ST_PT ? 1 : 0), py = t - c * ST_PT;
    const int iy = iy0 + py;
    const bool ok = colok && t < 3 * ST_PT && (unsigned)iy < (unsigned)H;
    raw[j] = __builtin_amdgcn_raw_buffer_load_b8(irsrc, ok ? (uint32_t)((c * H + iy) * W + ix) : SOD_OOB, 0, 0);
  }
  __syncthreads();
#pragma unroll
  for (int j = 0; j < PER_THREAD; ++j) {
    const int t = r0 + 5 * j;
    if (tid < 240 && t < 3 * ST_PT) {
      const int c = t >= 2 * ST_PT ? 2 : (t >= ST_PT ? 1 : 0), py = t - c * ST_PT;
      const bool ok = colok && (unsigned)(iy0 + py) < (unsigned)H;
      const __bf16 v = lut[(c << 8) + raw[j]];
      patch[t * ST_PSTR + px] = ok ? v : (__bf16)0.f;
    }
  }
  __syncthreads();

  float bv[4][4];
#pragma unroll
  for (int mi = 0; mi < 4; ++mi)
#pragma unroll
    for (int e = 0; e < 4; ++e) bv[mi][e] = a.bias[mi * 16 + fg * 4 + e];
  for (int nt = wave; nt < (ST_NPX + 15) / 16; nt += 4) {
    const int px = nt * 16 + fr;
    const int pc = px < ST_NPX ? px : ST_NPX - 1;
    const int cy = pc / ST_CT, cx = pc - cy * ST_CT;
    f32x4_t acc[4];
#pragma unroll
    for (int mi = 0; mi < 4; ++mi) acc[mi] = f32x4_t{0.f, 0.f, 0.f, 0.f};
#pragma unroll
    for (int ks = 0; ks < 6; ++ks) {
      const int kc = ks * 4 + fg;
      bf16x8_t bf;
      if (kc < 21) {
        const int c = kc / 7, r = kc - c * 7;
        const uint32_t* src = reinterpret_cast<const uint32_t*>(patch + (c * ST_PT + 2 * cy + r) * ST_PSTR + 2 * cx);
        typedef __attribute__((ext_vector_type(4))) unsigned int u4;
        const u4 raw = {src[0], src[1], src[2], src[3]};
        bf = __builtin_bit_cast(bf16x8_t, raw);
      } else {
#pragma unroll
        for (int e = 0; e < 8; ++e) bf[e] = (__bf16)0.f;
      }
#pragma unroll
      for (int mi = 0; mi < 4; ++mi) acc[mi] = __builtin_amdgcn_mfma_f32_16x16x32_bf16(af[mi][ks], bf, acc[mi], 0, 0, 0);
    }
    if (px < ST_NPX) {
#pragma unroll
      for (int mi = 0; mi < 4; ++mi) {
        bf16x4_t o;
#pragma unroll
        for (int e = 0; e < 4; ++e) o[e] = (__bf16)fmaxf(acc[mi][e] + bv[mi][e], 0.f);
        *reinterpret_cast<bf16x4_t*>(cout + px * ST_OSTR + mi * 16 + fg * 4) = o;
      }
    }
  }
  __syncthreads();

  for (int item = tid; item < 64 * 8; item += 256) {
    const int ch = item & 7, pp = item >> 3;
    const int py = pp >> 3, pxx = pp & 7;
    const int gy = ty * 8 + py, gx = tx * 8 + pxx;
    if (gy >= a.Hq || gx >= a.Wq) continue;
    float m[8];
#pragma unroll
    for (int e = 0; e < 8; ++e) m[e] = -3.0e38f;
#pragma unroll
    for (int dy = 0; dy < 3; ++dy) {
      const int ly = 2 * py + dy;
      if ((unsigned)(cy0 + ly) >= (unsigned)a.Hc) continue;
#pragma unroll
      for (int dx = 0; dx < 3; ++dx) {
        const int lx = 2 * pxx + dx;
        if ((unsigned)(cx0 + lx) >= (unsigned)a.Wc) continue;
        const bf16x8_t v = *reinterpret_cast<const bf16x8_t*>(cout + (ly * ST_CT + lx) * ST_OSTR + ch * 8);
#pragma unroll
        for (int e = 0; e < 8; ++e) m[e] = fmaxf(m[e], (float)v[e]);
      }
    }
    bf16x8_t o;
#pragma unroll
    for (int e = 0; e < 8; ++e) o[e] = (__bf16)m[e];
    *reinterpret_cast<bf16x8_t*>(a.out + (((long long)n * a.Hq + gy) * a.Wq + gx) * 64 + ch * 8) = o;
  }
}

}

extern "C" int sod_stem_fused(int n, const void* const* imgs, const int* H, const int* W, const void* w_packed, const float* bias,
                              void* out, int Hp, int Wp, const float* mean3, const float* std3, void* stream) {
  if (!imgs || !H || !W || !w_packed || !bias || !out || !mean3 || !std3) return SOD_EARG;
  if (n <= 0 || n > ST_MAX_IMAGES || Hp <= 0 || Wp <= 0 || (Hp & 3) || (Wp & 3)) return SOD_EARG;
  StemArgs a{};
  for (int i = 0; i < n; ++i) {
    if (!imgs[i] || H[i] <= 0 || W[i] <= 0 || H[i] > Hp || W[i] > Wp) return SOD_EARG;
    a.img[i] = (const uint8_t*)imgs[i]; a.H[i] = H[i]; a.W[i] = W[i];
  }
  a.w = (const __bf16*)w_packed; a.bias = bias; a.out = (__bf16*)out; a.N = n;
  a.Hc = (Hp + 6 - 7) / 2 + 1; a.Wc = (Wp + 6 - 7) / 2 + 1;
  a.Hq = (a.Hc + 2 - 3) / 2 + 1; a.Wq = (a.Wc + 2 - 3) / 2 + 1;
  for (int c = 0; c < 3; ++c) { a.mean[c] = mean3[c]; a.stdv[c] = std3[c]; }
  const hipError_t e = sod_max_dynamic_lds_once<stem_fused_kernel>(ST_LDS);
  if (e != hipSuccess) return (int)e;
  SOD_LAUNCH(stem_fused_kernel, dim3((a.Wq + 7) / 8, (a.Hq + 7) / 8, n), dim3(256), ST_LDS, (hipStream_t)stream, a);
  SOD_CHECK_LAUNCH();
  return SOD_OK;
}
```

### slenderobjdet_amd/layers/functional.py

```python
import ctypes
import os

import torch

from .. import _C
from .._C import call, ptr, stream_ptr

IOU_TYPES = {"iou": 0, "linear_iou": 1, "giou": 2}

PRECISION = "bf16"
ACT_DTYPE = torch.bfloat16


def set_precision(p):
    global PRECISION, ACT_DTYPE
    if p not in ("bf16", "fp32"):
        raise ValueError(f"precision must be 'bf16' or 'fp32', got {p!r}")
    prev, PRECISION = PRECISION, p
    ACT_DTYPE = torch.float32 if p == "fp32" else torch.bfloat16
    return prev


def is_f32():
    return PRECISION == "fp32"


def _precision_dispatch(fn):
    import functools

    @functools.wraps(fn)
    def wrapper(*args, **kwargs):
        if PRECISION == "fp32":
            from . import functional_f32 as F32

            impl = getattr(F32, fn.__name__, None)
            if impl is None:
                raise _C.SlenderHipError(f"{fn.__name__} has no fp32 validation variant")
            return impl(*args, **kwargs)
        return fn(*args, **kwargs)
    return wrapper

RELU_TAP = None

PROFILE = None
PROFILE_KINDS = None


PROFILE_LIB = False


def _prof_begin(stream=None, kind=None):
    if PROFILE is None or (PROFILE_KINDS is not None and kind not in PROFILE_KINDS):
        return None
    if PROFILE_LIB and kind in ("conv_fwd", "conv_dgrad", "conv_wgrad"):
        return "lib"
    e = torch.cuda.Event(enable_timing=True)
    e.record(stream)
    return e


def _nbytes(t):
    return 0 if t is None else t.numel() * t.element_size()


def _prof_end(kind, flops, e0, desc=None, stream=None):
    if e0 is None:
        return
    if e0 == "lib":
        PROFILE.append((kind, flops, None, None, desc, None))
        return
    e1 = torch.cuda.Event(enable_timing=True)
    e1.record(stream)
    variant = int(_C.load().sod_conv_last_variant()) if kind in ("conv_fwd", "conv_dgrad") else 0
    PROFILE.append((kind, flops, e0, e1, desc, variant))


WGRAD_SIDE_STREAM = os.environ.get("SOD_WGRAD_STREAM", "1") != "0"
_side_streams = {}
_side_keep = []
_side_join_queued = False


_aux_streams = {}


def cu_mask_words(lo, hi, total=256):
    words = [0] * ((total + 31) // 32)
    for i in range(max(0, lo), min(hi, total)):
        words[i // 32] |= 1 << (i % 32)
    return words


def make_stream(device, priority=0, role=None):
    spec = os.environ.get(f"SOD_CUMASK_{role}") if role else None
    if not spec:
        return torch.cuda.Stream(device=device, priority=priority)
    lo, hi = (int(v) for v in spec.split(":"))
    words = cu_mask_words(lo, hi)
    arr = (ctypes.c_uint * len(words))(*words)
    out = ctypes.c_void_p()
    with torch.cuda.device(device):
        call("sod_stream_create_cumask", ctypes.cast(arr, ctypes.c_void_p), len(words), ctypes.byref(out))
    return torch.cuda.ExternalStream(out.value, device=device)


def register_compute_stream(device, stream):
    lst = _aux_streams.setdefault(device.index, [])
    if all(s.cuda_stream != stream.cuda_stream for s in lst):
        lst.append(stream)


def aux_compute_streams(device):
    return list(_aux_streams.get(device.index, ()))




def wgrad_side_streams(device):
    return list(_side_streams.get(device.index, ())) if _side_join_queued else []


HOLD_HEAD_WGRAD = os.environ.get("SOD_HOLD_HEAD_WGRAD", "1") != "0"
_held = []


def hold_or_call(fn):
    if HOLD_HEAD_WGRAD and _side_join_queued_or_in_backward():
        _held.append(fn)
    else:
        fn()


def _side_join_queued_or_in_backward():
    global _side_join_queued
    if _side_join_queued:
        return True
    try:
        torch.autograd.Variable._execution_engine.queue_callback(_wgrad_join)
    except RuntimeError:
        return False
    _side_join_queued = True
    return True


def release_held():
    if _held:
        items = list(_held)
        _held.clear()
        for fn in items:
            fn()


def drop_held():
    _held.clear()


def _wgrad_join():
    global _side_join_queued
    release_held()
    _side_join_queued = False
    for idx, sides in _side_streams.items():
        main = torch.cuda.current_stream(idx)
        for side in sides:
            main.wait_stream(side)
    _side_keep.clear()


def wgrad_join():
    if _side_streams:
        _wgrad_join()


import threading as _threading

_batch_tls = _threading.local()


class wgrad_batch:
    def __enter__(self):
        self.outer = getattr(_batch_tls, "items", None)
        if self.outer is None:
            _batch_tls.items = []
        return self

    def __exit__(self, et, ev, tb):
        if self.outer is None:
            items, _batch_tls.items = _batch_tls.items, None
            if et is None and items:
                _batch_tls.flushing, _batch_tls.waited = True, set()
                try:
                    for fn in items:
                        fn()
                finally:
                    _batch_tls.flushing, _batch_tls.waited = False, None
        return False


def _batch_defer(fn):
    items = getattr(_batch_tls, "items", None)
    if items is None or not WGRAD_BATCH:
        return False
    items.append(fn)
    return True


def batch_or_call(fn):
    if not _batch_defer(fn):
        fn()


WGRAD_BATCH = True


def _wgrad_stream(device, tensors, key=None):
    global _side_join_queued
    if not WGRAD_SIDE_STREAM or device.type != "cuda":
        return None
    if not _side_join_queued:
        try:
            torch.autograd.Variable._execution_engine.queue_callback(_wgrad_join)
        except RuntimeError:
            return None
        _side_join_queued = True
    sides = _side_streams.get(device.index)
    if sides is None:
        sides = _side_streams[device.index] = [make_stream(device, 1, "WGRAD")]
    side = sides[0]
    cur = torch.cuda.current_stream(device)
    if getattr(_batch_tls, "flushing", False):
        tag = (side.cuda_stream, cur.cuda_stream)
        if tag not in _batch_tls.waited:
            side.wait_stream(cur)
            _batch_tls.waited.add(tag)
    else:
        side.wait_stream(cur)
    _side_keep.extend(t for t in tensors if t is not None)
    return side
CONV_RELU = 1
CONV_RES_UP2 = 2


def _chk(t, dtype=None, name="tensor"):
    if t is None:
        return
    if not t.is_cuda:
        raise _C.SlenderHipError(f"{name} must be a CUDA/HIP tensor (the HIP ops have no CPU fallback)")
    if not t.is_contiguous():
        raise _C.SlenderHipError(f"{name} must be contiguous")
    if dtype is not None and t.dtype != dtype:
        raise _C.SlenderHipError(f"{name} must be {dtype}, got {t.dtype}")


_ws_cache = {}


def reduce_ws(device):
    key = (device.index, torch.cuda.current_stream().cuda_stream)
    ws = _ws_cache.get(key)
    if ws is None:
        ws = torch.empty(_C.reduce_workspace_floats(), dtype=torch.float32, device=device)
        _ws_cache[key] = ws
    return ws


def conv_out_size(H, W, R, S, stride, pad, dil):
    Ho = (H + 2 * pad - dil * (R - 1) - 1) // stride + 1
    Wo = (W + 2 * pad - dil * (S - 1) - 1) // stride + 1
    return Ho, Wo


def conv2d_fwd(x, w, bias=None, res=None, stride=1, pad=0, dil=1, relu=False, res_up2=False, out_f32=False,
               out=None, y_img_stride=0, x_img_stride=0, x_shape=None, c_real=None, relu_bits=None):
    _chk(x, torch.bfloat16, "x"); _chk(w, torch.bfloat16, "w"); _chk(bias, torch.float32, "bias"); _chk(res, torch.bfloat16, "res")
    N, H, W, C = x_shape if x_shape is not None else x.shape
    K, R, S, Cw = w.shape
    cwin = Cw != C and is_channel_window(C, K, Cw)
    if Cw != C and not cwin:
        raise _C.SlenderHipError(f"weight channels {Cw} != input channels {C}")
    Ho, Wo = conv_out_size(H, W, R, S, stride, pad, dil)
    if out is None:
        out = torch.empty((N, Ho, Wo, K), dtype=torch.float32 if out_f32 else torch.bfloat16, device=x.device)
    flags = (CONV_RELU if relu else 0) | (CONV_RES_UP2 if res_up2 else 0) | (CONV_CWIN if cwin else 0)
    if cwin and (relu_bits is not None or res is not None):
        raise _C.SlenderHipError("conv2d_fwd: the channel-window mode takes neither a residual nor 1-bit ReLU masks")
    e0 = _prof_begin(None, "conv_fwd")
    if relu_bits is not None:
        _chk(relu_bits, torch.uint8, "relu_bits")
        if out_f32 or res_up2 or x_img_stride or y_img_stride or relu_bits.numel() * 8 != out.numel():
            raise _C.SlenderHipError("conv2d_fwd: relu_bits needs a dense bf16 output of 8 * relu_bits.numel() elements")
        call("sod_conv2d_fwd_bits", ptr(x), ptr(w), ptr(bias), ptr(res), ptr(out), ptr(relu_bits), N, H, W, C, K, R, S, stride, pad, dil, flags,
             stream_ptr())
    else:
        call("sod_conv2d_fwd", ptr(x), ptr(w), ptr(bias), ptr(res), ptr(out), N, H, W, C, K, R, S, stride, pad, dil,
             x_img_stride, y_img_stride, 0, flags, 1 if out_f32 else 0, stream_ptr())
    _prof_end("conv_fwd", 2.0 * N * Ho * Wo * K * R * S * (c_real or (Cw if cwin else C)), e0,
              (N, H, W, C, K, R, stride, _nbytes(res) + _nbytes(relu_bits)))
    if relu and RELU_TAP is not None and not x_img_stride and not y_img_stride:
        RELU_TAP("conv", w.data_ptr(), out)
    return out


CONV_CWIN = 4
WGRAD_DIAG = 2
CWIN = 128


def is_channel_window(C, K, Cw):
    return Cw == CWIN and C == K and C > CWIN and C % CWIN == 0 and not is_f32()


def conv2d_dgrad(dy, wt, x_hw, stride=1, pad=0, dil=1, accum=None, relu_mask=None, dy_img_stride=0, dy_shape=None, out=None, relu_bits=None,
                 accum_even=False):
    _chk(dy, torch.bfloat16, "dy"); _chk(wt, torch.bfloat16, "wt"); _chk(accum, torch.bfloat16, "accum"); _chk(relu_mask, torch.bfloat16, "relu_mask")
    N = dy_shape[0] if dy_shape is not None else dy.shape[0]
    C, R, S, K = wt.shape
    H, W = x_hw
    if out is None:
        out = torch.empty((N, H, W, C), dtype=torch.bfloat16, device=dy.device)
    if dy_shape is None and dy.shape[-1] != K and is_channel_window(C, dy.shape[-1], K):
        if accum is not None or relu_bits is not None or dy_img_stride:
            raise _C.SlenderHipError("conv2d_dgrad: the channel-window mode takes a ReLU mask tensor only")
        e0 = _prof_begin(None, "conv_dgrad")
        call("sod_conv2d_dgrad_cwin", ptr(dy), ptr(wt), ptr(relu_mask), ptr(out), N, H, W, C, C, R, S, stride, pad, dil, stream_ptr())
        Ho, Wo = conv_out_size(H, W, R, S, stride, pad, dil)
        _prof_end("conv_dgrad", 2.0 * N * Ho * Wo * C * R * S * K, e0, (N, H, W, C, C, R, stride))
        return out
    e0 = _prof_begin(None, "conv_dgrad")
    if relu_bits is not None:
        _chk(relu_bits, torch.uint8, "relu_bits")
        if relu_mask is not None or dy_img_stride or relu_bits.numel() * 8 != out.numel():
            raise _C.SlenderHipError("conv2d_dgrad: relu_bits replaces relu_mask and needs 8 * relu_bits.numel() == dx.numel()")
        if accum_even and (accum is None or tuple(accum.shape) != (N, H // 2, W // 2, C) or H % 2 or W % 2):
            raise _C.SlenderHipError("conv2d_dgrad: accum_even needs accum of shape (N, H/2, W/2, C) with even H, W")
        call("sod_conv2d_dgrad_bits", ptr(dy), ptr(wt), ptr(accum), 1 if accum_even else 0, ptr(relu_bits), ptr(out), N, H, W, C, K, R, S, stride,
             pad, dil, stream_ptr())
    else:
        if accum_even:
            raise _C.SlenderHipError("conv2d_dgrad: accum_even is available with relu_bits only")
        call("sod_conv2d_dgrad", ptr(dy), ptr(wt), ptr(accum), ptr(relu_mask), ptr(out), N, H, W, C, K, R, S, stride, pad, dil,
             dy_img_stride, 0, stream_ptr())
    Ho, Wo = conv_out_size(H, W, R, S, stride, pad, dil)
    _prof_end("conv_dgrad", 2.0 * N * Ho * Wo * K * R * S * C, e0,
              (N, H, W, C, K, R, stride, _nbytes(accum) + _nbytes(relu_mask) + _nbytes(relu_bits)))
    return out


DETERMINISTIC = os.environ.get("SOD_DETERMINISTIC", "0") == "1"
WGRAD_DETERMINISTIC = 1

_wgrad_ws = {}


def wgrad_workspace(device, stream=None):
    key = (device.index, (stream or torch.cuda.current_stream(device)).cuda_stream)
    ws = _wgrad_ws.get(key)
    if ws is None:
        ws = _wgrad_ws[key] = torch.empty(int(_C.load().sod_conv2d_wgrad_workspace_bytes()), dtype=torch.uint8, device=device)
    return ws


def conv2d_wgrad(dy, x, dw, R, S, stride=1, pad=0, dil=1, dy_img_stride=0, x_img_stride=0, K=None, x_shape=None, splits=0, qscale=None,
                 k_real=None, c_real=None):
    _chk(dy, torch.bfloat16, "dy"); _chk(x, torch.bfloat16, "x"); _chk(dw, torch.float32, "dw")
    if _batch_defer(lambda: conv2d_wgrad(dy, x, dw, R, S, stride, pad, dil, dy_img_stride, x_img_stride, K, x_shape, splits, qscale, k_real, c_real)):
        return dw
    N, H, W, C = x_shape if x_shape is not None else x.shape
    if K is None:
        K = dy.shape[-1]
    side = _wgrad_stream(dw.device, (dy, x, qscale), dw.data_ptr())
    ws = wgrad_workspace(dw.device, side)
    diag = dw.shape[-1] != C and is_channel_window(C, K, dw.shape[-1])
    e0 = _prof_begin(side, "conv_wgrad")
    call("sod_conv2d_wgrad", ptr(dy), ptr(x), ptr(dw), ptr(qscale), N, H, W, C, K, R, S, stride, pad, dil, dy_img_stride, x_img_stride,
         splits, (WGRAD_DETERMINISTIC if DETERMINISTIC else 0) | (WGRAD_DIAG if diag else 0), ptr(ws), ws.numel(), stream_ptr(side))
    Ho, Wo = conv_out_size(H, W, R, S, stride, pad, dil)
    _prof_end("conv_wgrad", 2.0 * N * Ho * Wo * (k_real or K) * R * S * (c_real or (CWIN if diag else C)), e0, (N, H, W, C, K, R, stride), side)
    return dw


def _ptr_arr(ts):
    return (ctypes.c_void_p * len(ts))(*[t.data_ptr() for t in ts])


def conv2d_fwd_ml(xs, w, bias=None, stride=1, pad=0, dil=1, relu=False, out_f32=False, outs=None, y_img_stride=0, k_real=None):
    _chk(w, torch.bfloat16, "w"); _chk(bias, torch.float32, "bias")
    for x in xs:
        _chk(x, torch.bfloat16, "x")
    N, C = xs[0].shape[0], xs[0].shape[3]
    K, R, S, Cw = w.shape
    if Cw != C:
        raise _C.SlenderHipError(f"weight channels {Cw} != input channels {C}")
    hs, ws = [x.shape[1] for x in xs], [x.shape[2] for x in xs]
    if outs is None:
        outs = [torch.empty((N,) + conv_out_size(h, wd, R, S, stride, pad, dil) + (K,), dtype=torch.float32 if out_f32 else torch.bfloat16,
                            device=xs[0].device) for h, wd in zip(hs, ws)]
    e0 = _prof_begin(None, "conv_fwd")
    call("sod_conv2d_fwd_ml", len(xs), _ptr_arr(xs), ptr(w), ptr(bias), _ptr_arr(outs), N, _int_arr(hs), _int_arr(ws), C, K, R, S,
         stride, pad, dil, y_img_stride, CONV_RELU if relu else 0, 1 if out_f32 else 0, stream_ptr())
    fl = sum(2.0 * N * ho * wo * (k_real or K) * R * S * C for ho, wo in (conv_out_size(h, wd, R, S, stride, pad, dil) for h, wd in zip(hs, ws)))
    _prof_end("conv_fwd", fl, e0, ("ml", N, tuple(hs), C, K, R, stride, tuple(ws)))
    if relu and RELU_TAP is not None and not y_img_stride:
        for o in outs:
            RELU_TAP("conv", w.data_ptr(), o)
    return outs


def conv_gn_fwd_ml(xs, w, bias, gamma, beta, G, eps=1e-5, relu=True, pad=1):
    _chk(w, torch.bfloat16, "w"); _chk(bias, torch.float32, "bias"); _chk(gamma, torch.float32, "gamma"); _chk(beta, torch.float32, "beta")
    for x in xs:
        _chk(x, torch.bfloat16, "x")
    N, C = xs[0].shape[0], xs[0].shape[3]
    K, R, S, Cw = w.shape
    if Cw != C or K != 8 * G:
        raise _C.SlenderHipError("conv_gn_fwd_ml: needs matching channels and 8 channels per group")
    hs, ws = [x.shape[1] for x in xs], [x.shape[2] for x in xs]
    outs = [torch.empty((N,) + conv_out_size(h, wd, R, S, 1, pad, 1) + (K,), dtype=torch.bfloat16, device=xs[0].device) for h, wd in zip(hs, ws)]
    stats = torch.empty((len(xs), N, G, 2), dtype=torch.float32, device=xs[0].device)
    e0 = _prof_begin(None, "conv_fwd")
    call("sod_conv2d_fwd_ml_gnsum", len(xs), _ptr_arr(xs), ptr(w), ptr(bias), _ptr_arr(outs), N, _int_arr(hs), _int_arr(ws), C, K, R, S,
         1, pad, 1, 0, 0, ptr(stats), G, stream_ptr())
    fl = sum(2.0 * N * o.shape[1] * o.shape[2] * K * R * S * C for o in outs)
    _prof_end("conv_fwd", fl, e0, ("ml", N, tuple(hs), C, K, R, 1, tuple(ws)))
    ys = [torch.empty_like(o) for o in outs]
    hw = [o.shape[1] * o.shape[2] for o in outs]
    call("sod_groupnorm_apply_ml", len(outs), _ptr_arr(outs), ptr(gamma), ptr(beta), _ptr_arr(ys), ptr(stats), N, ctypes.cast(_int_arr(hw), ctypes.c_void_p),
         K, G, eps, 1 if relu else 0, stream_ptr())
    if relu and RELU_TAP is not None:
        for y in ys:
            RELU_TAP("gn", gamma.data_ptr(), y)
    return outs, ys, stats


def conv2d_dgrad_ml(dys, wt, x_hws, stride=1, pad=0, dil=1, dy_img_stride=0, N=None, k_real=None, relu_masks=None, accums=None, k_pitch=None):
    _chk(wt, torch.bfloat16, "wt")
    C, R, S, K = wt.shape
    if N is None:
        N = dys[0].shape[0]
    dev = dys[0].device
    outs = [torch.empty((N, h, w, C), dtype=torch.bfloat16, device=dev) for h, w in x_hws]
    e0 = _prof_begin(None, "conv_dgrad")
    if k_pitch is not None and k_pitch != K:
        if relu_masks is not None or accums is not None or stride != 1:
            raise _C.SlenderHipError("conv2d_dgrad_ml: k_pitch comes without masks / accums, stride 1")
        call("sod_conv2d_dgrad_ml_kpitch", len(dys), _ptr_arr(dys), ptr(wt), _ptr_arr(outs), N, _int_arr([h for h, _ in x_hws]),
             _int_arr([w for _, w in x_hws]), C, K, int(k_pitch), R, S, pad, dil, dy_img_stride, stream_ptr())
    elif accums is not None:
        if len(accums) != len(outs) or (relu_masks is not None and len(relu_masks) != len(outs)):
            raise _C.SlenderHipError("conv2d_dgrad_ml: accums (and relu_masks) come one per level")
        for t, o in zip(list(accums) + list(relu_masks or ()), list(outs) * 2):
            _chk(t, torch.bfloat16, "accum / relu_mask")
            if tuple(t.shape) != tuple(o.shape) or not t.is_contiguous():
                raise _C.SlenderHipError("conv2d_dgrad_ml: accums / relu_masks must be contiguous tensors of the data gradients' shapes")
        call("sod_conv2d_dgrad_ml_accum", len(dys), _ptr_arr(dys), ptr(wt), _ptr_arr(accums), _ptr_arr(relu_masks) if relu_masks is not None else None,
             _ptr_arr(outs), N, _int_arr([h for h, _ in x_hws]), _int_arr([w for _, w in x_hws]), C, K, R, S, stride, pad, dil, dy_img_stride, stream_ptr())
    elif relu_masks is not None:
        for t, o in zip(relu_masks, outs):
            _chk(t, torch.bfloat16, "relu_mask")
            if tuple(t.shape) != tuple(o.shape):
                raise _C.SlenderHipError("conv2d_dgrad_ml: relu_masks must have the data gradients' shapes")
        call("sod_conv2d_dgrad_ml_mask", len(dys), _ptr_arr(dys), ptr(wt), _ptr_arr(relu_masks), _ptr_arr(outs), N, _int_arr([h for h, _ in x_hws]),
             _int_arr([w for _, w in x_hws]), C, K, R, S, stride, pad, dil, dy_img_stride, stream_ptr())
    else:
        call("sod_conv2d_dgrad_ml", len(dys), _ptr_arr(dys), ptr(wt), _ptr_arr(outs), N, _int_arr([h for h, _ in x_hws]), _int_arr([w for _, w in x_hws]),
             C, K, R, S, stride, pad, dil, dy_img_stride, stream_ptr())
    fl = sum(2.0 * N * ho * wo * (k_real or K) * R * S * C for ho, wo in (conv_out_size(h, w, R, S, stride, pad, dil) for h, w in x_hws))
    _prof_end("conv_dgrad", fl, e0, ("ml", N, tuple(h for h, _ in x_hws), C, K, R, stride, tuple(w for _, w in x_hws)))
    return outs


def conv2d_wgrad_ml(dys, xs, dw, R, S, stride=1, pad=0, dil=1, dy_img_stride=0, K=None, splits=0, qscale=None, k_real=None):
    _chk(dw, torch.float32, "dw")
    if _batch_defer(lambda: conv2d_wgrad_ml(dys, xs, dw, R, S, stride, pad, dil, dy_img_stride, K, splits, qscale, k_real)):
        return dw
    N, C = xs[0].shape[0], xs[0].shape[3]
    if K is None:
        K = dys[0].shape[-1]
    hs, ws_ = [x.shape[1] for x in xs], [x.shape[2] for x in xs]
    side = _wgrad_stream(dw.device, list(dys) + list(xs) + [qscale], dw.data_ptr())
    ws = wgrad_workspace(dw.device, side)
    e0 = _prof_begin(side, "conv_wgrad")
    call("sod_conv2d_wgrad_ml", len(xs), _ptr_arr(dys), _ptr_arr(xs), ptr(dw), ptr(qscale), N, _int_arr(hs), _int_arr(ws_), C, K, R, S,
         stride, pad, dil, dy_img_stride, splits, WGRAD_DETERMINISTIC if DETERMINISTIC else 0, ptr(ws), ws.numel(), stream_ptr(side))
    fl = sum(2.0 * N * ho * wo * (k_real or K) * R * S * C for ho, wo in (conv_out_size(h, w, R, S, stride, pad, dil) for h, w in zip(hs, ws_)))
    _prof_end("conv_wgrad", fl, e0, ("ml", N, tuple(hs), C, K, R, stride, tuple(ws_)), side)
    return dw


def weight_prep(w_master, scale=None, want_krsc=True, want_crsk=True, cpad=None):
    _chk(w_master, torch.float32, "w"); _chk(scale, torch.float32, "scale")
    K, R, S, C = w_master.shape
    cpad = C if cpad is None else cpad
    wk = (torch.zeros if cpad != C else torch.empty)((K, R, S, cpad), dtype=torch.bfloat16, device=w_master.device) if want_krsc else None
    wc = torch.empty((C, R, S, K), dtype=torch.bfloat16, device=w_master.device) if want_crsk else None
    call("sod_weight_prep", ptr(w_master), ptr(scale), ptr(wk), ptr(wc), K, R * S, C, cpad, stream_ptr())
    return wk, wc


def _det_ws(device, stream=None):
    if not DETERMINISTIC:
        return None, 0
    ws = wgrad_workspace(device, stream)
    return ptr(ws), ws.numel()


def groupnorm_fwd(x, gamma, beta, G, eps=1e-5, relu=False):
    _chk(x, torch.bfloat16, "x"); _chk(gamma, torch.float32, "gamma"); _chk(beta, torch.float32, "beta")
    N, C = x.shape[0], x.shape[-1]
    HW = x.numel() // (N * C)
    y = torch.empty_like(x)
    stats = torch.empty((N, G, 2), dtype=torch.float32, device=x.device)
    call("sod_groupnorm_fwd", ptr(x), ptr(gamma), ptr(beta), ptr(y), ptr(stats), N, HW, C, G, 0, eps, 1 if relu else 0, *_det_ws(x.device), stream_ptr())
    if relu and RELU_TAP is not None:
        RELU_TAP("gn", gamma.data_ptr(), y)
    return y, stats


def groupnorm_bwd(dy, x, gamma, beta, stats, G, dgamma, dbeta, relu=False, dxsum=None):
    _chk(dy, torch.bfloat16, "dy"); _chk(x, torch.bfloat16, "x"); _chk(dgamma, torch.float32, "dgamma"); _chk(dbeta, torch.float32, "dbeta")
    N, C = x.shape[0], x.shape[-1]
    HW = x.numel() // (N * C)
    dx = torch.empty_like(x)
    red = torch.empty((N, G, 2), dtype=torch.float32, device=x.device)
    call("sod_groupnorm_bwd", ptr(dy), ptr(x), ptr(gamma), ptr(beta), ptr(stats), ptr(dx), ptr(dgamma), ptr(dbeta), ptr(dxsum), ptr(red),
         N, HW, C, G, 0, 1 if relu else 0, *_det_ws(x.device), stream_ptr())
    return dx


def groupnorm_fwd_ml(xs, gamma, beta, G, eps=1e-5, relu=False):
    _chk(gamma, torch.float32, "gamma"); _chk(beta, torch.float32, "beta")
    for x in xs:
        _chk(x, torch.bfloat16, "x")
    N, C = xs[0].shape[0], xs[0].shape[-1]
    hw = [x.numel() // (N * C) for x in xs]
    ys = [torch.empty_like(x) for x in xs]
    stats = torch.empty((len(xs), N, G, 2), dtype=torch.float32, device=xs[0].device)
    call("sod_groupnorm_fwd_ml", len(xs), _ptr_arr(xs), ptr(gamma), ptr(beta), _ptr_arr(ys), ptr(stats), N, ctypes.cast(_int_arr(hw), ctypes.c_void_p),
         C, G, eps, 1 if relu else 0, *_det_ws(xs[0].device), stream_ptr())
    if relu and RELU_TAP is not None:
        for y in ys:
            RELU_TAP("gn", gamma.data_ptr(), y)
    return ys, stats


def groupnorm_bwd_ml(dys, xs, gamma, beta, stats, G, dgamma, dbeta, relu=False, dxsum=None):
    _chk(dgamma, torch.float32, "dgamma"); _chk(dbeta, torch.float32, "dbeta"); _chk(stats, torch.float32, "stats")
    for t in list(dys) + list(xs):
        _chk(t, torch.bfloat16, "dy/x")
    N, C = xs[0].shape[0], xs[0].shape[-1]
    hw = [x.numel() // (N * C) for x in xs]
    dxs = [torch.empty_like(x) for x in xs]
    red = torch.empty((len(xs), N, G, 2), dtype=torch.float32, device=xs[0].device)
    call("sod_groupnorm_bwd_ml", len(xs), _ptr_arr(dys), _ptr_arr(xs), ptr(gamma), ptr(beta), ptr(stats), _ptr_arr(dxs), ptr(dgamma), ptr(dbeta),
         ptr(dxsum), ptr(red), N, ctypes.cast(_int_arr(hw), ctypes.c_void_p), C, G, 1 if relu else 0, *_det_ws(xs[0].device), stream_ptr())
    return dxs


def relu_fwd(x):
    _chk(x, torch.bfloat16, "x")
    y = torch.empty_like(x)
    call("sod_relu_fwd", ptr(x), ptr(y), x.numel(), stream_ptr())
    if RELU_TAP is not None:
        RELU_TAP("relu", 0, y)
    return y


def relu_bwd(dy, y):
    _chk(dy, torch.bfloat16, "dy"); _chk(y, torch.bfloat16, "y")
    dx = torch.empty_like(dy)
    call("sod_relu_bwd", ptr(dy), ptr(y), ptr(dx), dy.numel(), stream_ptr())
    return dx


def add_bf16(a, b):
    _chk(a, torch.bfloat16, "a"); _chk(b, torch.bfloat16, "b")
    o = torch.empty_like(a)
    call("sod_add_bf16", ptr(a), ptr(b), ptr(o), a.numel(), stream_ptr())
    return o


def bias_grad(dy, dbias, N, HW, C, img_stride=0, scale_num=None, scale_den=None, den_mul=1.0, den_min=1.0):
    _chk(dy, torch.bfloat16, "dy"); _chk(dbias, torch.float32, "dbias")
    _chk(scale_num, torch.float32, "scale_num"); _chk(scale_den, torch.float32, "scale_den")
    if _batch_defer(lambda: bias_grad(dy, dbias, N, HW, C, img_stride, scale_num, scale_den, den_mul, den_min)):
        return dbias
    side = _wgrad_stream(dbias.device, (dy, scale_num, scale_den), dbias.data_ptr())
    if scale_num is None and scale_den is None:
        call("sod_bias_grad", ptr(dy), ptr(dbias), N, HW, C, img_stride, *_det_ws(dbias.device, side), stream_ptr(side))
    else:
        call("sod_bias_grad_scaled", ptr(dy), ptr(dbias), ptr(scale_num), ptr(scale_den), float(den_mul), float(den_min), N, HW, C, img_stride,
             *_det_ws(dbias.device, side), stream_ptr(side))
    return dbias


def bias_grad_ml(dys, dbias):
    _chk(dbias, torch.float32, "dbias")
    for t in dys:
        _chk(t, torch.bfloat16, "dy")
    N, C = dys[0].shape[0], dys[0].shape[-1]
    if _batch_defer(lambda: bias_grad_ml(dys, dbias)):
        return dbias
    if DETERMINISTIC or len(dys) > 6:
        for g in dys:
            bias_grad(g, dbias, N, g.numel() // (N * C), C)
        return dbias
    side = _wgrad_stream(dbias.device, list(dys), dbias.data_ptr())
    hw = [g.numel() // (N * C) for g in dys]
    call("sod_bias_grad_ml", len(dys), _ptr_arr(dys), ptr(dbias), N, ctypes.cast(_int_arr(hw), ctypes.c_void_p), C, stream_ptr(side))
    return dbias


def maxpool3x3s2(x):
    _chk(x, torch.bfloat16, "x")
    N, H, W, C = x.shape
    Ho, Wo = (H + 2 - 3) // 2 + 1, (W + 2 - 3) // 2 + 1
    y = torch.empty((N, Ho, Wo, C), dtype=torch.bfloat16, device=x.device)
    call("sod_maxpool3x3s2", ptr(x), ptr(y), N, H, W, C, stream_ptr())
    return y


def upsample2x_bwd(g):
    _chk(g, torch.bfloat16, "g")
    N, H, W, C = g.shape
    d = torch.empty((N, H // 2, W // 2, C), dtype=torch.bfloat16, device=g.device)
    call("sod_upsample2x_bwd", ptr(g), ptr(d), N, H // 2, W // 2, C, stream_ptr())
    return d


def preprocess_image(img, out, mean, std):
    if img.dtype not in (torch.uint8, torch.float32):
        raise _C.SlenderHipError("image must be uint8 or float32")
    _chk(img, None, "image"); _chk(out, torch.bfloat16, "out")
    C, H, W = img.shape
    Hp, Wp, Cp = out.shape
    m = (ctypes.c_float * 3)(*[float(v) for v in mean])
    s = (ctypes.c_float * 3)(*[float(v) for v in std])
    call("sod_preprocess_image", ptr(img), 1 if img.dtype == torch.uint8 else 0, C, H, W, ptr(out), Hp, Wp, Cp,
         ctypes.cast(m, ctypes.c_void_p), ctypes.cast(s, ctypes.c_void_p), stream_ptr())
    return out


def preprocess_batch(imgs, out, mean, std):
    dt = imgs[0].dtype
    if dt not in (torch.uint8, torch.float32) or any(i.dtype != dt for i in imgs) or len(imgs) > 64:
        for i, im in enumerate(imgs):
            preprocess_image(im.contiguous() if im.dtype in (torch.uint8, torch.float32) else im.float().contiguous(), out[i], mean, std)
        return out
    _chk(out, torch.bfloat16, "out")
    imgs = [i.contiguous() for i in imgs]
    for i in imgs:
        _chk(i, None, "image")
    n, Hp, Wp, Cp = out.shape
    C = imgs[0].shape[0]
    m = (ctypes.c_float * 3)(*[float(v) for v in mean])
    s = (ctypes.c_float * 3)(*[float(v) for v in std])
    call("sod_preprocess_batch", len(imgs), _ptr_arr(imgs), 1 if dt == torch.uint8 else 0, C, _int_arr([i.shape[1] for i in imgs]),
         _int_arr([i.shape[2] for i in imgs]), ptr(out), Hp, Wp, Cp, ctypes.cast(m, ctypes.c_void_p), ctypes.cast(s, ctypes.c_void_p), stream_ptr())
    return out


class RawImageBatch:

    def __init__(self, imgs, sizes, padded_hw, mean, std):
        self.imgs, self.sizes, self.padded_hw, self.mean, self.std = imgs, sizes, padded_hw, mean, std
        self._tensor = None

    @property
    def shape(self):
        return (len(self.imgs), self.padded_hw[0], self.padded_hw[1], 8)

    @property
    def device(self):
        return self.imgs[0].device

    def materialize(self):
        if self._tensor is None:
            Hp, Wp = self.padded_hw
            batch = torch.empty((len(self.imgs), Hp, Wp, 8), dtype=torch.bfloat16, device=self.device)
            self._tensor = preprocess_batch(self.imgs, batch, self.mean, self.std)
        return self._tensor


def stem_pack_weights(w_bf16):
    K = w_bf16.shape[0]
    w = w_bf16[..., :3].permute(0, 3, 1, 2).contiguous()
    out = torch.zeros((K, 24, 8), dtype=torch.bfloat16, device=w_bf16.device)
    out[:, :21, :7] = w.reshape(K, 21, 7)
    return out.contiguous()


def stem_fused(raw, w_packed, bias):
    _chk(w_packed, torch.bfloat16, "w_packed"); _chk(bias, torch.float32, "bias")
    n = len(raw.imgs)
    Hp, Wp = raw.padded_hw
    if n > 64 or Hp % 4 or Wp % 4 or tuple(w_packed.shape) != (64, 24, 8):
        raise _C.SlenderHipError("stem_fused: unsupported batch / weight shape")
    for im in raw.imgs:
        _chk(im, torch.uint8, "image")
        if im.dim() != 3 or im.shape[0] != 3:
            raise _C.SlenderHipError("stem_fused: images must be (3, H, W) uint8")
    out = torch.empty((n, Hp // 4, Wp // 4, 64), dtype=torch.bfloat16, device=raw.device)
    prof = PROFILE is not None and (PROFILE_KINDS is None or "conv_fwd" in PROFILE_KINDS)
    if prof:
        e0 = torch.cuda.Event(enable_timing=True)
        e0.record()
    m = (ctypes.c_float * 3)(*[float(v) for v in raw.mean])
    s_ = (ctypes.c_float * 3)(*[float(v) for v in raw.std])
    call("sod_stem_fused", n, _ptr_arr(raw.imgs), _int_arr([i.shape[1] for i in raw.imgs]), _int_arr([i.shape[2] for i in raw.imgs]), ptr(w_packed), ptr(bias),
         ptr(out), Hp, Wp, ctypes.cast(m, ctypes.c_void_p), ctypes.cast(s_, ctypes.c_void_p), stream_ptr())
    if prof:
        e1 = torch.cuda.Event(enable_timing=True)
        e1.record()
        PROFILE.append(("conv_fwd", 2.0 * n * (Hp // 2) * (Wp // 2) * 64 * 49 * 3, e0, e1, (n, Hp, Wp, 3, 64, 7, 2), -7))
    return out


def bottleneck_frozen_fwd(x, w1, b1, w2, b2, w3, b3, wsc=None):
    for t, nm in ((x, "x"), (w1, "w1"), (w2, "w2"), (w3, "w3"), (wsc, "wsc")):
        _chk(t, torch.bfloat16, nm)
    for t, nm in ((b1, "b1"), (b2, "b2"), (b3, "b3")):
        _chk(t, torch.float32, nm)
    N, H, W, Cin = x.shape
    if (tuple(w1.shape) != (64, 1, 1, Cin) or tuple(w2.shape) != (64, 3, 3, 64) or tuple(w3.shape) != (256, 1, 1, 64)
            or (wsc is not None and tuple(wsc.shape) != (256, 1, 1, Cin)) or b1.numel() != 64 or b2.numel() != 64 or b3.numel() != 256):
        raise _C.SlenderHipError("bottleneck_frozen_fwd: unsupported block shape")
    out = torch.empty((N, H, W, 256), dtype=torch.bfloat16, device=x.device)
    prof = PROFILE is not None and (PROFILE_KINDS is None or "conv_fwd" in PROFILE_KINDS)
    if prof:
        e0 = torch.cuda.Event(enable_timing=True)
        e0.record()
    call("sod_bottleneck_frozen_fwd", ptr(x), N, H, W, Cin, ptr(w1), ptr(b1), ptr(w2), ptr(b2), ptr(w3), ptr(b3), ptr(wsc), ptr(out), stream_ptr())
    if prof:
        e1 = torch.cuda.Event(enable_timing=True)
        e1.record()
        macs = Cin * 64 + 9 * 64 * 64 + 64 * 256 + (Cin * 256 if wsc is not None else 0)
        PROFILE.append(("conv_fwd", 2.0 * N * H * W * macs, e0, e1, (N, H, W, Cin, 256, "bneck", 1), -8))
    return out


def nchw_f32_to_nhwc_bf16(x):
    _chk(x, torch.float32, "x")
    N, C, H, W = x.shape
    y = torch.empty((N, H, W, C), dtype=torch.bfloat16, device=x.device)
    call("sod_nchw_f32_to_nhwc_bf16", ptr(x), ptr(y), N, C, H * W, stream_ptr())
    return y


def focal_loss_fwd(logits, labels=None, dense=None, alpha=0.25, gamma=2.0, K=None, want_elem=False):
    _chk(logits, torch.float32, "logits"); _chk(labels, torch.int32, "labels"); _chk(dense, torch.float32, "targets")
    ld = logits.shape[-1]
    K = ld if K is None else K
    M = logits.numel() // ld
    elem = torch.empty((M, K), dtype=torch.float32, device=logits.device) if want_elem else None
    out = torch.empty(1, dtype=torch.float32, device=logits.device)
    call("sod_sigmoid_focal_loss_fwd", ptr(logits), ptr(labels), ptr(dense), M, K, ld, alpha, gamma, ptr(elem), ptr(out),
         ptr(reduce_ws(logits.device)), stream_ptr())
    return out, elem


def focal_loss_fwd_grad(logits, labels, alpha=0.25, gamma=2.0, K=None, ld_out=None, out=None):
    _chk(logits, torch.float32, "logits"); _chk(labels, torch.int32, "labels")
    ld = logits.shape[-1]
    K = ld if K is None else K
    M = logits.numel() // ld
    ld_out = K if ld_out is None else ld_out
    if out is None:
        out = torch.empty((M, ld_out), dtype=torch.bfloat16, device=logits.device)
    s = torch.empty(1, dtype=torch.float32, device=logits.device)
    call("sod_sigmoid_focal_loss_fwd_grad", ptr(logits), ptr(labels), M, K, ld, alpha, gamma, ptr(s), ptr(reduce_ws(logits.device)), ptr(out), ld_out,
         stream_ptr())
    return s, out


def focal_loss_bwd(logits, labels=None, dense=None, alpha=0.25, gamma=2.0, K=None, scale_num=None, scale_den=None,
                   den_mul=1.0, den_min=1.0, ld_out=None, out_bf16=False, out=None):
    _chk(logits, torch.float32, "logits")
    ld = logits.shape[-1]
    K = ld if K is None else K
    M = logits.numel() // ld
    ld_out = K if ld_out is None else ld_out
    if out is None:
        out = torch.empty((M, ld_out), dtype=torch.bfloat16 if out_bf16 else torch.float32, device=logits.device)
    call("sod_sigmoid_focal_loss_bwd", ptr(logits), ptr(labels), ptr(dense), M, K, ld, alpha, gamma, ptr(scale_num), ptr(scale_den),
         den_mul, den_min, ptr(out), ld_out, 1 if out_bf16 else 0, stream_ptr())
    return out


def iou_loss_fwd(pred, target, weight=None, loss_type="iou", mask=None, mask_bg=-1, want_elem=False):
    _chk(pred, torch.float32, "pred"); _chk(target, torch.float32, "target"); _chk(weight, torch.float32, "weight"); _chk(mask, torch.int32, "mask")
    P = pred.shape[0]
    elem = torch.empty(P, dtype=torch.float32, device=pred.device) if want_elem else None
# ... 679 lines not shown
```

### slenderobjdet_amd/layers/nn.py

```python
import math

import torch
from torch import nn
from torch.autograd.function import once_differentiable

from . import functional as HF


def _arena_of(mod):
    return getattr(mod, "_arena", None)


class DeferSlot:
    _offers = {}

    def __init__(self):
        self.g = self.mod = None
        self.comp = None

    @classmethod
    def reset(cls):
        cls._offers.clear()

    @classmethod
# ... 98 lines not shown

    def prepare(self, force=False):
        arena = _arena_of(self)
        key = (self.weight._version, self.bias._version if self.bias is not None else 0,
               arena.generation if (arena is not None and self.weight.requires_grad) else -1, self.weight.data_ptr(), HF.PRECISION)
        if not force and key == self._prep_key:
            return
        if arena is not None and getattr(self, "_b_krsc", None) is not None and self.weight.requires_grad and not HF.is_f32():
            return self._prepare_batched(arena, key)
        w = self.weight.detach()
        if self.frozen_bn:
            bn_key = (self.bn_weight._version, self.bn_bias._version, self.bn_running_mean._version, self.bn_running_var._version,
                      self.bn_weight.data_ptr(), self.bias._version if self.bias is not None else 0, "own")
            if bn_key != getattr(self, "_bn_key", None):
                scale = self.bn_weight * torch.rsqrt(self.bn_running_var + 1e-5)
                shift = self.bn_bias - self.bn_running_mean * scale
                self.bn_scale = scale.contiguous()
                self.bias_eff = (shift + (self.bias.detach() * scale if self.bias is not None else 0)).contiguous()
                self._bn_key = bn_key
        else:
            self.bn_scale = None
            self.bias_eff = self.bias.detach() if self.bias is not None else None
        need_t = self.weight.requires_grad or True
        self.w_bf16, self.wt_bf16 = HF.weight_prep(w.contiguous(), self.bn_scale, True, need_t, self.cin_pad)
        self._prep_key = key

    def forward(self, x, res=None, res_up2=False):
        self.prepare()
        return _ConvFn.apply(x, res, self.weight, self, res_up2)


WINDOWED = _os.environ.get("SOD_GROUPED_WINDOW", "1") != "0"


class HipGroupedConv2d(HipConv2d):

    def __init__(self, in_channels, out_channels, kernel_size, stride=1, padding=0, dilation=1, groups=1, **kw):
        if in_channels % groups or out_channels % groups:
            raise ValueError(f"groups={groups} must divide in_channels={in_channels} and out_channels={out_channels}")
        super().__init__(in_channels, out_channels, kernel_size, stride, padding, dilation, **kw)
        self.groups = groups
        self.weight = nn.Parameter(torch.empty(out_channels, kernel_size, kernel_size, in_channels // groups))

    batched_prep_shape = None

    def init_msra(self):
        fan_out = self.out_channels * self.kernel_size * self.kernel_size
        nn.init.normal_(self.weight, 0.0, math.sqrt(2.0 / fan_out))

    def windowed(self):
        C, K, g = self.in_channels, self.out_channels, self.groups
        return (WINDOWED and not HF.is_f32() and C == K and C > HF.CWIN and C % HF.CWIN == 0 and HF.CWIN % (C // g) == 0)

    def window_weight(self, w):
        K, R, S, Cg = w.shape
        T, gt = K // HF.CWIN, HF.CWIN // Cg
        d = w.new_zeros(T, gt, Cg, R, S, gt, Cg)
        idx = torch.arange(gt, device=w.device)
        d[:, idx, :, :, :, idx, :] = w.reshape(T, gt, Cg, R, S, Cg).permute(1, 0, 2, 3, 4, 5)
        return d.reshape(K, R, S, HF.CWIN)

    def window_blocks(self, win):
        K, R, S, _ = win.shape
        Cg = self.in_channels // self.groups
        T, gt = K // HF.CWIN, HF.CWIN // Cg
        idx = torch.arange(gt, device=win.device)
        v = win.reshape(T, gt, Cg, R, S, gt, Cg)
        return v[:, idx, :, :, :, idx, :].permute(1, 0, 2, 3, 4, 5).reshape(K, R, S, Cg)

    def dense_weight(self, w):
        K, R, S, Cg = w.shape
        g = self.groups
        d = w.new_zeros(K, R, S, Cg * g)
        idx = torch.arange(g, device=w.device)
        d.view(g, K // g, R, S, g, Cg)[idx, :, :, :, idx, :] = w.reshape(g, K // g, R, S, Cg)
        return d

    def blocks_of(self, dense):
        K, R, S, C = dense.shape
        g = self.groups
        idx = torch.arange(g, device=dense.device)
        return dense.view(g, K // g, R, S, g, C // g)[idx, :, :, :, idx, :].reshape(K, R, S, C // g)

    def weight_kcrs(self):
        return self.weight.detach().permute(0, 3, 1, 2).contiguous()

    def prepare(self, force=False):
        arena = _arena_of(self)
        key = (self.weight._version, arena.generation if (arena is not None and self.weight.requires_grad) else -1, self.weight.data_ptr(),
               self._bn_state() if self.frozen_bn else None, HF.PRECISION)
        if not force and key == self._prep_key:
            return
        if self.frozen_bn:
            scale = self.bn_weight * torch.rsqrt(self.bn_running_var + 1e-5)
            self.bn_scale = scale.contiguous()
            self.bias_eff = (self.bn_bias - self.bn_running_mean * scale + (self.bias.detach() * scale if self.bias is not None else 0)).contiguous()
        else:
            self.bn_scale = None
            self.bias_eff = self.bias.detach() if self.bias is not None else None
        with torch.no_grad():
            if self.windowed():
                win = self.window_weight(self.weight.detach())
                if self.bn_scale is not None:
                    win = win * self.bn_scale.view(-1, 1, 1, 1)
                T = self.out_channels // HF.CWIN
                win_t = win.reshape(T, HF.CWIN, self.kernel_size, self.kernel_size, HF.CWIN).permute(0, 4, 2, 3, 1).reshape(win.shape)
                self.w_bf16 = HF.weight_prep(win.contiguous(), None, True, False, None)[0]
                self.wt_bf16 = HF.weight_prep(win_t.contiguous(), None, True, False, None)[0]
                self._prep_key = key
                return
            dense = self.dense_weight(self.weight.detach())
        self.w_bf16, self.wt_bf16 = HF.weight_prep(dense.contiguous(), self.bn_scale, True, True, None)
        self._prep_key = key

    def wgrad_into(self, arena, g, x):
        HF.batch_or_call(lambda: self._wgrad_into_now(arena, g, x))

    def _wgrad_into_now(self, arena, g, x):
        K, k, C = self.out_channels, self.kernel_size, self.in_channels
        win = self.windowed()
        dense = torch.zeros((K, k, k, HF.CWIN if win else C), dtype=torch.float32, device=g.device)
        prev, HF.WGRAD_SIDE_STREAM = HF.WGRAD_SIDE_STREAM, False
        try:
            HF.conv2d_wgrad(g, x, dense, k, k, self.stride, self.padding, self.dilation, qscale=self.bn_scale)
        finally:
            HF.WGRAD_SIDE_STREAM = prev
        arena.grad_view(self.weight).add_(self.window_blocks(dense) if win else self.blocks_of(dense))
        arena.mark_ready(self.weight)


class _ConvFn(torch.autograd.Function):
    @staticmethod
    def forward(ctx, x, res, weight, mod, res_up2):
        y = HF.conv2d_fwd(x, mod.w_bf16, mod.bias_eff, res, mod.stride, mod.padding, mod.dilation, relu=mod.relu, res_up2=res_up2,
                          out_f32=mod.out_f32, c_real=mod.in_channels if mod.cin_pad else None)
        ctx.mod, ctx.res_up2, ctx.has_res = mod, res_up2, res is not None
        ctx.slot = None
        if DEFER_LATERAL_DGRAD and x.requires_grad and mod.kernel_size == 1 and mod.stride == 1 and not mod.mask_input and not mod.relu:
            ctx.slot = DeferSlot.take(x)
        train_w = mod.weight.requires_grad
        if train_w or x.requires_grad or (res is not None and res.requires_grad):
            ctx.save_for_backward(x, y if mod.relu else None)
            if train_w and _arena_of(mod) is not None:
                _arena_of(mod).note_use(mod.weight)
                if mod.bias is not None:
                    _arena_of(mod).note_use(mod.bias)
        return y

    @staticmethod
    @once_differentiable
    def backward(ctx, dy):
        mod = ctx.mod
        x, y = ctx.saved_tensors
        dy = dy.contiguous()
        if dy.dtype == torch.float32:
            dy = HF.f32_to_bf16(dy)
        g = HF.relu_bwd(dy, y) if (mod.relu and not mod.grad_premasked) else dy
        arena = _arena_of(mod)
        N, H, W, C = x.shape
        HF.release_held()
        if mod.weight.requires_grad:
            with HF.wgrad_batch():
                if getattr(mod, "groups", 1) > 1:
                    mod.wgrad_into(arena, g, x)
                else:
                    dw = arena.grad_view(mod.weight)
                    HF.conv2d_wgrad(g, x, dw, mod.kernel_size, mod.kernel_size, mod.stride, mod.padding, mod.dilation, qscale=mod.bn_scale)
                    arena.mark_ready(mod.weight)
                if mod.bias is not None:
                    HF.bias_grad(g, arena.grad_view(mod.bias), N, g.shape[1] * g.shape[2], mod.out_channels)
                    arena.mark_ready(mod.bias)
        dx = None
        if ctx.needs_input_grad[0]:
            if ctx.slot is not None:
                ctx.slot.g, ctx.slot.mod = g, mod
            else:
                dx = HF.conv2d_dgrad(g, mod.wt_bf16, (H, W), mod.stride, mod.padding, mod.dilation,
                                     relu_mask=x if mod.mask_input else None)
        dres = None
        if ctx.has_res and ctx.needs_input_grad[1]:
            dres = HF.upsample2x_bwd(g) if ctx.res_up2 else g
        return dx, dres, None, None, None


class HipGroupNorm(nn.Module):

    def __init__(self, num_groups, num_channels, eps=1e-5):
        super().__init__()
        self.num_groups, self.num_channels, self.eps = num_groups, num_channels, eps
        self.weight = nn.Parameter(torch.ones(num_channels))
        self.bias = nn.Parameter(torch.zeros(num_channels))


class GradPark:
    current = None

    def __init__(self):
        self.consumer_ptrs = set()
        self.parked = {}
        self.done = False
        self.hooked = False

    def put(self, ptr, g):
        self.parked[ptr] = g
        if not self.hooked:
            torch.autograd.Variable._execution_engine.queue_callback(self._check)
            self.hooked = True

    def _check(self):
        self.hooked = False
        if self.parked:
            self.parked.clear()
            raise RuntimeError("GradPark: the ROI pooler parked feature gradients and the RPN head's backward never collected them "
                               "(meta_arch.rcnn.GRAD_PARK = False restores autograd's accumulation)")


class SiblingFold:

    def __init__(self):
        self.partial = self.event = self.stream = None
        self.hooked = False

    def put(self, dxs):
        self.partial = list(dxs)
        self.stream = torch.cuda.current_stream(dxs[0].device)
        self.event = torch.cuda.Event()
        self.event.record(self.stream)
        if not self.hooked:
            torch.autograd.Variable._execution_engine.queue_callback(self._check)
            self.hooked = True

    def take(self):
        part, self.partial = self.partial, None
        cur = torch.cuda.current_stream(part[0].device)
        if cur.cuda_stream != self.stream.cuda_stream:
            cur.wait_event(self.event)
            for t in part:
                t.record_stream(cur)
        return part

    def _check(self):
        self.hooked = False
        if self.partial is not None:
            self.partial = None
            raise RuntimeError("SiblingFold: one tower parked its input gradient and the other never ran in this backward pass "
                               "(SOD_TOWER_FOLD=0 restores autograd's accumulation)")


class ConvGnRelu(nn.Module):

    def __init__(self, channels, num_groups=32):
        super().__init__()
        self.conv = HipConv2d(channels, channels, 3, 1, 1, bias=True)
        self.gn = HipGroupNorm(num_groups, channels)

    def forward(self, xs, fold=None):
        single = isinstance(xs, torch.Tensor)
        if single:
            xs = [xs]
        self.conv.prepare()
        out = _ConvGnReluFn.apply(self.conv.weight, self, fold, *xs)
        return out[0] if single else list(out)


class _ConvGnReluFn(torch.autograd.Function):
    @staticmethod
    def forward(ctx, weight, unit, fold, *xs):
        conv, gn = unit.conv, unit.gn
        ctx.fold = fold
        gw, gb = gn.weight.detach(), gn.bias.detach()
        relu = True
        if (GN_EPILOGUE_STATS and not HF.DETERMINISTIC and not HF.is_f32() and conv.out_channels == 8 * gn.num_groups
                and conv.stride == 1 and conv.dilation == 1 and 2 * conv.padding == conv.kernel_size - 1):
            y1s, y2s, stats = HF.conv_gn_fwd_ml(list(xs), conv.w_bf16, conv.bias_eff, gw, gb, gn.num_groups, gn.eps, relu=relu, pad=conv.padding)
        else:
            y1s = HF.conv2d_fwd_ml(list(xs), conv.w_bf16, conv.bias_eff, conv.stride, conv.padding, conv.dilation)
            y2s, stats = HF.groupnorm_fwd_ml(y1s, gw, gb, gn.num_groups, gn.eps, relu=relu)
        ctx.unit, ctx.nl, ctx.relu = unit, len(xs), relu
        ctx.save_for_backward(*xs, *y1s, stats)
        arena = _arena_of(conv)
        if arena is not None and conv.weight.requires_grad:
            for p in (conv.weight, conv.bias, gn.weight, gn.bias):
                if p is not None:
                    arena.note_use(p)
        return tuple(y2s)

    @staticmethod
    @once_differentiable
    def backward(ctx, *dy2s):
        conv, gn = ctx.unit.conv, ctx.unit.gn
        nl = ctx.nl
        saved = ctx.saved_tensors
        xs, y1s, stats = saved[:nl], saved[nl:2 * nl], saved[2 * nl]
        arena = _arena_of(conv)
        gw, gb = gn.weight.detach(), gn.bias.detach()
        dgw, dgb = arena.grad_view(gn.weight), arena.grad_view(gn.bias)
        relu, k = ctx.relu, conv.kernel_size
        dbias = arena.grad_view(conv.bias) if conv.bias is not None else None
        dy1s = HF.groupnorm_bwd_ml([d.contiguous() for d in dy2s], list(y1s), gw, gb, stats, gn.num_groups, dgw, dgb, relu=relu, dxsum=dbias)
        arena.mark_ready(gn.weight)
        arena.mark_ready(gn.bias)
        if conv.bias is not None:
            arena.mark_ready(conv.bias)
        def wgrad():
            HF.conv2d_wgrad_ml(dy1s, list(xs), arena.grad_view(conv.weight), k, k, conv.stride, conv.padding, conv.dilation)
            arena.mark_ready(conv.weight)
        HF.hold_or_call(wgrad)
        dxs = [None] * nl
        if any(ctx.needs_input_grad[3:]):
            fold, ctx.fold = ctx.fold, None
            hw = [(x.shape[1], x.shape[2]) for x in xs]
            if fold is not None and all(ctx.needs_input_grad[3:]):
                if fold.partial is None:
                    fold.put(HF.conv2d_dgrad_ml(dy1s, conv.wt_bf16, hw, conv.stride, conv.padding, conv.dilation))
                else:
                    dxs = HF.conv2d_dgrad_ml(dy1s, conv.wt_bf16, hw, conv.stride, conv.padding, conv.dilation, accums=fold.take())
            else:
                dxs = HF.conv2d_dgrad_ml(dy1s, conv.wt_bf16, hw, conv.stride, conv.padding, conv.dilation)
        return (None, None, None, *dxs)


class _ReluToken:

    def __init__(self, outs):
        self.out_ptrs = [(t.data_ptr(), tuple(t.shape)) for t in outs]
        self.premasked = False

    def matches(self, xs):
        return len(xs) == len(self.out_ptrs) and all((x.data_ptr(), tuple(x.shape)) == k for x, k in zip(xs, self.out_ptrs))


RELU_CHAIN = True


class ConvReluML(nn.Module):

    def __init__(self, channels):
        super().__init__()
        self.conv = HipConv2d(channels, channels, 3, 1, 1, bias=True)
        self._last_token = None

    def forward(self, xs, chained=None):
        self.conv.prepare()
        tok = None
        if RELU_CHAIN and chained is not None and chained._last_token is not None and chained._last_token.matches(xs):
            tok = chained._last_token
        return list(_ConvReluMLFn.apply(self.conv.weight, self, tok, *xs))


class _ConvReluMLFn(torch.autograd.Function):
    @staticmethod
    def forward(ctx, weight, unit, in_token, *xs):
        conv = unit.conv
        ys = HF.conv2d_fwd_ml(list(xs), conv.w_bf16, conv.bias_eff, 1, 1, 1, relu=True)
        ctx.unit, ctx.nl = unit, len(xs)
        ctx.save_for_backward(*xs, *ys)
        ctx.in_token = in_token
        ctx.token = unit._last_token = None
        arena = _arena_of(conv)
        if arena is not None and conv.weight.requires_grad:
            arena.note_use(conv.weight)
            arena.note_use(conv.bias)
            ctx.token = unit._last_token = _ReluToken(ys)
        if in_token is not None and all(x.requires_grad for x in xs):
            in_token.premasked = True
        else:
            ctx.in_token = None
        return tuple(ys)

    @staticmethod
    @once_differentiable
    def backward(ctx, *dys):
        conv, nl = ctx.unit.conv, ctx.nl
        saved = ctx.saved_tensors
        xs, ys = saved[:nl], saved[nl:]
        arena = _arena_of(conv)
        if ctx.token is not None and ctx.token.premasked:
            gs = [dy.contiguous() for dy in dys]
        else:
            gs = [HF.relu_bwd(dy.contiguous(), y) for dy, y in zip(dys, ys)]
        def wgrad():
            with HF.wgrad_batch():
                HF.conv2d_wgrad_ml(gs, list(xs), arena.grad_view(conv.weight), 3, 3, 1, 1, 1)
                arena.mark_ready(conv.weight)
                HF.bias_grad_ml(gs, arena.grad_view(conv.bias))
                arena.mark_ready(conv.bias)
        HF.hold_or_call(wgrad)
        dxs = [None] * nl
        if any(ctx.needs_input_grad[3:]):
            hw = [(x.shape[1], x.shape[2]) for x in xs]
            dxs = HF.conv2d_dgrad_ml(gs, conv.wt_bf16, hw, 1, 1, 1, relu_masks=list(xs) if ctx.in_token is not None else None)
        return (None, None, None, *dxs)


class ConvML(nn.Module):

    def __init__(self, in_channels, out_channels, kernel_size=1, padding=0, relu=False, out_f32=False):
        super().__init__()
        self.conv = HipConv2d(in_channels, out_channels, kernel_size, 1, padding, bias=True)
        self.relu, self.out_f32 = relu, out_f32

    def forward(self, xs):
        self.conv.prepare()
        return list(_ConvMLFn.apply(self.conv.weight, self, *xs))


class _ConvMLFn(torch.autograd.Function):
    @staticmethod
    def forward(ctx, weight, unit, *xs):
        conv = unit.conv
        ys = HF.conv2d_fwd_ml(list(xs), conv.w_bf16, conv.bias_eff, 1, conv.padding, 1, relu=unit.relu, out_f32=unit.out_f32)
        ctx.unit, ctx.nl = unit, len(xs)
        ctx.save_for_backward(*xs, *(ys if unit.relu else ()))
        arena = _arena_of(conv)
        if arena is not None and conv.weight.requires_grad:
            arena.note_use(conv.weight)
            arena.note_use(conv.bias)
        return tuple(ys)

    @staticmethod
    @once_differentiable
    def backward(ctx, *dys):
        unit, nl = ctx.unit, ctx.nl
        conv = unit.conv
        saved = ctx.saved_tensors
        xs, ys = saved[:nl], saved[nl:]
        arena = _arena_of(conv)
        gs = []
        for i, dy in enumerate(dys):
            dy = dy.contiguous()
            if dy.dtype == torch.float32:
                dy = HF.f32_to_bf16(dy)
            gs.append(HF.relu_bwd(dy, ys[i]) if unit.relu else dy)
        k = conv.kernel_size
        with HF.wgrad_batch():
            HF.conv2d_wgrad_ml(gs, list(xs), arena.grad_view(conv.weight), k, k, 1, conv.padding, 1)
            arena.mark_ready(conv.weight)
            HF.bias_grad_ml(gs, arena.grad_view(conv.bias))
            arena.mark_ready(conv.bias)
        dxs = [None] * nl
        if any(ctx.needs_input_grad[2:]):
            dxs = HF.conv2d_dgrad_ml(gs, conv.wt_bf16, [(x.shape[1], x.shape[2]) for x in xs], 1, conv.padding, 1)
        return (None, None, *dxs)


class _AddUp2Fn(torch.autograd.Function):

    @staticmethod
    def forward(ctx, a, b):
        return HF.add_up2(a, b)

    @staticmethod
    @once_differentiable
    def backward(ctx, dy):
        dy = dy.contiguous()
        return (dy if ctx.needs_input_grad[0] else None), (HF.upsample2x_bwd(dy) if ctx.needs_input_grad[1] else None)


def add_up2(a, b):
    return _AddUp2Fn.apply(a, b)


class _GnReluFn(torch.autograd.Function):

    @staticmethod
    def forward(ctx, x, weight, gn, relu):
        y, stats = HF.groupnorm_fwd(x, gn.weight.detach(), gn.bias.detach(), gn.num_groups, gn.eps, relu=relu)
        ctx.gn, ctx.relu = gn, relu
        ctx.save_for_backward(x, stats)
        arena = _arena_of(gn)
        if arena is not None:
            arena.note_use(gn.weight)
            arena.note_use(gn.bias)
        return y

    @staticmethod
    @once_differentiable
    def backward(ctx, dy):
        gn = ctx.gn
        x, stats = ctx.saved_tensors
        arena = _arena_of(gn)
        dx = HF.groupnorm_bwd(dy.contiguous(), x, gn.weight.detach(), gn.bias.detach(), stats, gn.num_groups,
                              arena.grad_view(gn.weight), arena.grad_view(gn.bias), relu=ctx.relu)
        arena.mark_ready(gn.weight)
        arena.mark_ready(gn.bias)
        return dx, None, None, None


def group_norm_relu(x, gn, relu=True):
    return _GnReluFn.apply(x, gn.weight, gn, relu)


class _ReluFn(torch.autograd.Function):
    @staticmethod
    def forward(ctx, x):
        y = HF.relu_fwd(x)
        ctx.save_for_backward(y)
        return y

    @staticmethod
    @once_differentiable
    def backward(ctx, dy):
        (y,) = ctx.saved_tensors
        return HF.relu_bwd(dy.contiguous(), y)


def relu(x):
    return _ReluFn.apply(x)


class _MaxPoolFn(torch.autograd.Function):
    @staticmethod
    def forward(ctx, x):
        if x.requires_grad:
            raise NotImplementedError("max-pool backward is not built: the stem is frozen (MODEL.BACKBONE.FREEZE_AT >= 1)")
        return HF.maxpool3x3s2(x)


def max_pool_3x3_s2(x):
    return _MaxPoolFn.apply(x)


class Scale(nn.Module):

    def __init__(self, init_value=1.0):
        super().__init__()
        self.scale = nn.Parameter(torch.FloatTensor([init_value]))

    def forward(self, input):
        return input * self.scale


def attach_arena(model, arena):
    for m in model.modules():
        m._arena = arena
    model.register_forward_pre_hook(lambda mod, inputs: arena.on_forward(torch.is_grad_enabled() and mod.training))
```

Before: 668.6 img/s.

## Batch held head wgrads into one multi-problem launch; make stem kernel persistent

```diff
diff --git a/include/slender_hip.h b/include/slender_hip.h
--- a/include/slender_hip.h
+++ b/include/slender_hip.h
@@ -64,6 +64,8 @@
 int sod_conv2d_wgrad_ml(int nlev, const void* const* dy, const void* const* x, float* dw, const float* qscale,
                         int N, const int* H, const int* W, int C, int K, int R, int S, int stride, int pad, int dil,
                         long long dy_img_stride, int splits, int flags, void* ws, long long ws_bytes, void* stream);
+int sod_conv2d_wgrad_ml_batch(int nprob, int nlev, const void* const* dy, const void* const* x, float* const* dw,
+                              int N, const int* H, const int* W, int C, int K, void* ws, long long ws_bytes, void* stream);
 int sod_conv2d_dgrad_cwin(const void* dy, const void* wt_win, const void* relu_mask, void* dx,
                           int N, int H, int W, int C, int K, int R, int S, int stride, int pad, int dil, void* stream);
 int sod_conv_set_tile256(int mode);
@@ -118,6 +120,7 @@
                          int Cpad, const float* mean3, const float* std3, void* stream);
 int sod_stem_fused(int n, const void* const* imgs, const int* H, const int* W, const void* w_packed, const float* bias,
                    void* out, int Hp, int Wp, const float* mean3, const float* std3, void* stream);
+int sod_stem_set_max_workgroups(int n);
 int sod_bottleneck_frozen_fwd(const void* x, int N, int H, int W, int Cin, const void* w1, const float* b1, const void* w2,
                               const float* b2, const void* w3, const float* b3, const void* wsc, void* out, void* stream);
 int sod_resize_flip_preprocess_batch(int n, const void* const* imgs, const int* H, const int* W, const int* newH, const int* newW,
diff --git a/slenderobjdet_amd/_C.py b/slenderobjdet_amd/_C.py
--- a/slenderobjdet_amd/_C.py
+++ b/slenderobjdet_amd/_C.py
@@ -27,6 +27,7 @@
     "sod_conv2d_dgrad_ml_kpitch": [_I, _P, _P, _P, _I, _P, _P, _I, _I, _I, _I, _I, _I, _I, _L, _P],
     "sod_conv2d_dgrad_ml_accum": [_I, _P, _P, _P, _P, _P, _I, _P, _P, _I, _I, _I, _I, _I, _I, _I, _L, _P],
     "sod_conv2d_wgrad_ml": [_I, _P, _P, _P, _P, _I, _P, _P, _I, _I, _I, _I, _I, _I, _I, _L, _I, _I, _P, _L, _P],
+    "sod_conv2d_wgrad_ml_batch": [_I, _I, _P, _P, _P, _I, _P, _P, _I, _I, _P, _L, _P],
     "sod_groupnorm_fwd": [_P, _P, _P, _P, _P, _I, _I, _I, _I, _L, _F, _I, _P, _L, _P],
     "sod_groupnorm_bwd": [_P, _P, _P, _P, _P, _P, _P, _P, _P, _P, _I, _I, _I, _I, _L, _I, _P, _L, _P],
     "sod_groupnorm_fwd_ml": [_I, _P, _P, _P, _P, _P, _I, _P, _I, _I, _F, _I, _P, _L, _P],
@@ -58,6 +59,7 @@
     "sod_preprocess_batch": [_I, _P, _I, _I, _P, _P, _P, _I, _I, _I, _P, _P, _P],
     "sod_nchw_f32_to_nhwc_bf16": [_P, _P, _I, _I, _I, _P],
     "sod_stem_fused": [_I, _P, _P, _P, _P, _P, _P, _I, _I, _P, _P, _P],
+    "sod_stem_set_max_workgroups": [_I],
     "sod_bottleneck_frozen_fwd": [_P, _I, _I, _I, _I, _P, _P, _P, _P, _P, _P, _P, _P, _P],
     "sod_resize_flip_preprocess_batch": [_I, _P, _P, _P, _P, _P, _P, _P, _P, _P, _P, _P, _P, _P, _I, _I, _I, _P, _P, _P],
     "sod_sigmoid_focal_loss_fwd": [_P, _P, _P, _L, _I, _I, _F, _F, _P, _P, _P, _P],
diff --git a/slenderobjdet_amd/csrc/conv_args.h b/slenderobjdet_amd/csrc/conv_args.h
--- a/slenderobjdet_amd/csrc/conv_args.h
+++ b/slenderobjdet_amd/csrc/conv_args.h
@@ -139,6 +139,7 @@
 long long wgrad9_workspace_bytes(const WgradArgs& a, int cus);
 int wgrad9_tiles_per_block(const WgradArgs& a, int cus);
 int launch_wgrad9(const WgradArgs& a, int cus, float* ws, long long ws_bytes, hipStream_t st);
+int launch_wgrad9_batch(const WgradArgs* probs, int P, int cus, float* ws, long long ws_bytes, hipStream_t st);
 
 bool wgrad_fold_supported(const WgradArgs& a);
 int launch_wgrad_fold(WgradArgs& a, int cus, hipStream_t st);
diff --git a/slenderobjdet_amd/csrc/conv_dispatch.hip b/slenderobjdet_amd/csrc/conv_dispatch.hip
--- a/slenderobjdet_amd/csrc/conv_dispatch.hip
+++ b/slenderobjdet_amd/csrc/conv_dispatch.hip
@@ -511,6 +511,26 @@
   return conv_wgrad(nlev, dy, x, dw, qscale, Geo{N, H, W, C, K, R, S, stride, pad, dil}, dy_img_stride, 0, splits, flags, ws, ws_bytes, stream);
 }
 
+extern "C" int sod_conv2d_wgrad_ml_batch(int nprob, int nlev, const void* const* dy, const void* const* x, float* const* dw,
+                                         int N, const int* H, const int* W, int C, int K, void* ws, long long ws_bytes, void* stream) {
+  if (!dy || !x || !dw || !H || !W || nprob < 1 || nprob > 8 || nlev <= 0 || nlev > MAXLEV || !ws || ws_bytes < 0 || ((uintptr_t)ws & 15)) return SOD_EARG;
+  if (N <= 0 || C <= 0 || K <= 0 || (C & 7) || (K & 7)) return SOD_EARG;
+  WgradArgs probs[8];
+  for (int p = 0; p < nprob; ++p) {
+    WgradArgs& a = probs[p];
+    a = WgradArgs{};
+    if (!dw[p]) return SOD_EARG;
+    a.nlev = nlev; a.dw = dw[p]; a.N = N; a.C = C; a.K = K;
+    a.R = 3; a.S = 3; a.stride = 1; a.pad = 1; a.dil = 1;
+    for (int l = 0; l < nlev; ++l) {
+      const int rc = fill_wlevel(a, l, dy[p * nlev + l], x[p * nlev + l], H[l], W[l], 0, 0);
+      if (rc) return rc;
+    }
+  }
+  const hipStream_t st = (hipStream_t)stream;
+  return timed(st, 9009, 1.f, 2, [&] { return launch_wgrad9_batch(probs, nprob, device_cus(), (float*)ws, ws_bytes, st); });
+}
+
 extern "C" int sod_conv_last_variant(void) { return g_last_variant; }
 
 extern "C" int sod_conv_prof_enable(int on) {
diff --git a/slenderobjdet_amd/csrc/conv_wgrad9.hip b/slenderobjdet_amd/csrc/conv_wgrad9.hip
--- a/slenderobjdet_amd/csrc/conv_wgrad9.hip
+++ b/slenderobjdet_amd/csrc/conv_wgrad9.hip
@@ -39,8 +39,6 @@
 }
 
 struct W9Level {
-  const void* dy;
-  const void* x;
   uint32_t dy_bytes, x_bytes;
   int H, W, Wp, HWp;
   int Npad;
@@ -50,10 +48,18 @@
   FastDiv div_hwp, div_wp;
 };
 
+constexpr int W9_MAXP = 8;
+
+struct W9Prob {
+  const void* dy[MAXLEV];
+  const void* x[MAXLEV];
+  float* dw;
+};
+
 struct W9Args {
   W9Level lev[MAXLEV];
-  int nlev;
-  float* dw;
+  W9Prob prob[W9_MAXP];
+  int nlev, P;
   const float* qscale;
   float* partial;
   int N, C, K, QT, CT;
@@ -69,7 +75,10 @@
   const int wr = wave >> 2, wc = wave & 3;
   const uint32_t bid = xcd_remap(blockIdx.x, gridDim.x);
   const int tiles = a.QT * a.CT;
-  const int tile = (int)(bid % (uint32_t)tiles), z = (int)(bid / (uint32_t)tiles);
+  const uint32_t zp = bid / (uint32_t)tiles;
+  const int tile = (int)(bid - zp * (uint32_t)tiles);
+  const int z = (int)(zp / (uint32_t)a.P), p = (int)(zp - (uint32_t)z * (uint32_t)a.P);
+  const W9Prob& pr = a.prob[p];
   const int ct = tile % a.CT, qt = tile / a.CT;
   const int q0 = qt * 128, c0 = ct * 64;
   const int kt_beg = z * a.t_per_split;
@@ -105,8 +114,8 @@
     if (sa >= sb) continue;
     const int T = sb - sa, j0 = sa * 64, E = g.E;
     const int W = g.W, Wp = g.Wp, HWp = g.HWp, sh0 = g.W + 2;
-    auto yrsrc = __builtin_amdgcn_make_buffer_rsrc(const_cast<void*>(g.dy), 0, g.dy_bytes, 0x00020000);
-    auto xrsrc = __builtin_amdgcn_make_buffer_rsrc(const_cast<void*>(g.x), 0, g.x_bytes, 0x00020000);
+    auto yrsrc = __builtin_amdgcn_make_buffer_rsrc(const_cast<void*>(pr.dy[lv]), 0, g.dy_bytes, 0x00020000);
+    auto xrsrc = __builtin_amdgcn_make_buffer_rsrc(const_cast<void*>(pr.x[lv]), 0, g.x_bytes, 0x00020000);
 
     auto pix = [&](int j, uint32_t& n, uint32_t& hw) -> bool {
       if ((unsigned)j >= (unsigned)g.Npad) return false;
@@ -253,7 +262,7 @@
     __builtin_amdgcn_s_barrier();
   }
 
-  float* slab = a.partial + ((size_t)z * (size_t)tiles + (size_t)tile) * G9_SLAB + (size_t)wave * (36 * 256) + (size_t)lane * 4;
+  float* slab = a.partial + (size_t)bid * G9_SLAB + (size_t)wave * (36 * 256) + (size_t)lane * 4;
 #pragma unroll
   for (int i = 0; i < 4; ++i)
 #pragma unroll
@@ -265,10 +274,12 @@
   const uint32_t idx = blockIdx.x * 256u + threadIdx.x;
   const int lane = idx & 63;
   const uint32_t fi = idx >> 6;
-  const int tile = (int)(fi / 288u), frag = (int)(fi % 288u);
-  if (tile >= tiles) return;
-  const float* src = a.partial + (size_t)tile * G9_SLAB + (size_t)frag * 256 + (size_t)lane * 4;
-  const size_t zstride = (size_t)tiles * G9_SLAB;
+  const int pt = (int)(fi / 288u), frag = (int)(fi % 288u);
+  if (pt >= a.P * tiles) return;
+  const int p = pt / tiles, tile = pt - p * tiles;
+  float* const dw = a.prob[p].dw;
+  const float* src = a.partial + (size_t)pt * G9_SLAB + (size_t)frag * 256 + (size_t)lane * 4;
+  const size_t zstride = (size_t)a.P * (size_t)tiles * G9_SLAB;
   f32x4_t s0 = {0.f, 0.f, 0.f, 0.f}, s1 = s0, s2 = s0, s3 = s0;
   int zz = 0;
   for (; zz + 4 <= a.nz; zz += 4) {
@@ -288,19 +299,19 @@
   for (int e = 0; e < 4; ++e) {
     const int q = qt * 128 + wr * 64 + i * 16 + fg * 4 + e;
     if (q >= a.K) continue;
-    float* dst = a.dw + ((size_t)q * 9 + tap) * a.C + c;
+    float* dst = dw + ((size_t)q * 9 + tap) * a.C + c;
     *dst += sum[e] * (a.qscale ? a.qscale[q] : 1.f);
   }
 }
 
 int w9_fill(const WgradArgs& a, W9Args& w) {
-  w.nlev = a.nlev; w.dw = a.dw; w.qscale = a.qscale; w.N = a.N; w.C = a.C; w.K = a.K;
+  w.nlev = a.nlev; w.P = 1; w.prob[0].dw = a.dw; w.qscale = a.qscale; w.N = a.N; w.C = a.C; w.K = a.K;
   w.QT = (a.K + 127) / 128; w.CT = a.C / 64;
   int t0 = 0;
   for (int l = 0; l < a.nlev; ++l) {
     const WLevel& s = a.lev[l];
     W9Level& g = w.lev[l];
-    g.dy = s.dy; g.x = s.x; g.dy_bytes = s.dy_bytes; g.x_bytes = s.x_bytes;
+    w.prob[0].dy[l] = s.dy; w.prob[0].x[l] = s.x; g.dy_bytes = s.dy_bytes; g.x_bytes = s.x_bytes;
     g.H = s.Hx; g.W = s.Wx; g.Wp = s.Wx + 1; g.HWp = (s.Hx + 1) * (s.Wx + 1);
     g.Npad = a.N * g.HWp;
     g.T = (g.Npad + 63) / 64; g.t0 = t0; t0 += g.T;
@@ -374,4 +385,43 @@
   return SOD_OK;
 }
 
-}
+int launch_wgrad9_batch(const WgradArgs* probs, int P, int cus, float* ws, long long ws_bytes, hipStream_t st) {
+  if (!probs || P < 1 || P > W9_MAXP) return SOD_EARG;
+  const WgradArgs& a0 = probs[0];
+  for (int i = 0; i < P; ++i) {
+    const WgradArgs& a = probs[i];
+    if (!wgrad9_supported(a) || a.qscale || !a.dw) return SOD_EARG;
+    if (a.nlev != a0.nlev || a.N != a0.N || a.C != a0.C || a.K != a0.K) return SOD_EARG;
+    for (int l = 0; l < a.nlev; ++l) {
+      const WLevel &s = a.lev[l], &r = a0.lev[l];
+      if (s.Hx != r.Hx || s.Wx != r.Wx || s.dy_img_stride != r.dy_img_stride || s.x_img_stride != r.x_img_stride || s.dy_bytes != r.dy_bytes ||
+          s.x_bytes != r.x_bytes)
+        return SOD_EARG;
+    }
+  }
+  W9Args w{};
+  w9_fill(a0, w);
+  w.P = P;
+  for (int i = 1; i < P; ++i) {
+    w.prob[i].dw = probs[i].dw;
+    for (int l = 0; l < a0.nlev; ++l) { w.prob[i].dy[l] = probs[i].lev[l].dy; w.prob[i].x[l] = probs[i].lev[l].x; }
+  }
+  const int tiles = w.QT * w.CT;
+  if ((long long)P * tiles > cus) return SOD_EARG;
+  int nz = cus / (P * tiles); if (nz < 1) nz = 1;
+  if (nz > w.Ttot) nz = w.Ttot;
+  const int per = (w.Ttot + nz - 1) / nz;
+  w.t_per_split = per;
+  w.nz = (w.Ttot + per - 1) / per;
+  const long long need = (long long)w.nz * P * tiles * G9_SLAB * (long long)sizeof(float);
+  if (!ws || need > ws_bytes) return SOD_EARG;
+  w.partial = ws;
+  const hipError_t e = sod_max_dynamic_lds_once<conv_wgrad9_kernel>(G9_LDS + 1024);
+  if (e != hipSuccess) return (int)e;
+  SOD_LAUNCH(conv_wgrad9_kernel, dim3(w.nz * P * tiles), dim3(512), G9_LDS + 1024, st, w);
+  SOD_LAUNCH(wgrad9_reduce_kernel, dim3(P * tiles * 72), dim3(256), 0, st, w);
+  SOD_CHECK_LAUNCH();
+  return SOD_OK;
+}
+
+}
diff --git a/slenderobjdet_amd/csrc/stem_fused.hip b/slenderobjdet_amd/csrc/stem_fused.hip
--- a/slenderobjdet_amd/csrc/stem_fused.hip
+++ b/slenderobjdet_amd/csrc/stem_fused.hip
@@ -9,8 +9,12 @@
 constexpr int ST_CT = 17;
 constexpr int ST_NPX = ST_CT * ST_CT;
 constexpr int ST_OSTR = 72;
+constexpr int ST_LUT_BYTES = 3 * 256 * 2;
 constexpr int ST_PATCH_BYTES = 3 * ST_PT * ST_PSTR * 2;
-constexpr int ST_LDS = ST_PATCH_BYTES + ST_NPX * ST_OSTR * 2;
+constexpr int ST_LDS = ST_LUT_BYTES + 2 * ST_PATCH_BYTES + ST_NPX * ST_OSTR * 2;
+constexpr int ST_WG_PER_CU = 2;
+
+std::atomic<int> g_max_workgroups{0};
 
 struct StemArgs {
   const uint8_t* img[ST_MAX_IMAGES];
@@ -19,20 +23,20 @@
   const float* bias;
   __bf16* out;
   int N, Hc, Wc, Hq, Wq;
+  int tiles_x;
+  uint32_t ntiles;
+  FastDiv div_img, div_tx;
   float mean[3], stdv[3];
 };
 
-__global__ __launch_bounds__(256) void stem_fused_kernel(const StemArgs a) {
+__global__ __launch_bounds__(256, ST_WG_PER_CU) void stem_fused_kernel(const StemArgs a) {
   extern __shared__ __attribute__((aligned(16))) char smem[];
-  __bf16* patch = reinterpret_cast<__bf16*>(smem);
-  __bf16* cout = reinterpret_cast<__bf16*>(smem + ST_PATCH_BYTES);
+  __bf16* lut = reinterpret_cast<__bf16*>(smem);
+  __bf16* cout = reinterpret_cast<__bf16*>(smem + ST_LUT_BYTES + 2 * ST_PATCH_BYTES);
   const int tid = threadIdx.x, lane = tid & 63;
   const int wave = __builtin_amdgcn_readfirstlane(tid >> 6);
-  const int tx = blockIdx.x, ty = blockIdx.y, n = blockIdx.z;
-  const int H = a.H[n], W = a.W[n];
-  const uint8_t* __restrict__ img = a.img[n];
-  const int cy0 = 16 * ty - 1, cx0 = 16 * tx - 1;
-  const int iy0 = 2 * cy0 - 3, ix0 = 2 * cx0 - 3;
+  const uint32_t G = gridDim.x;
+  const uint32_t first = (G & 7u) ? blockIdx.x : (blockIdx.x & 7u) * (G >> 3) + (blockIdx.x >> 3);
 
   const int fr = lane & 15, fg = lane >> 4;
   bf16x8_t af[4][6];
@@ -40,105 +44,140 @@
   for (int mi = 0; mi < 4; ++mi)
 #pragma unroll
     for (int ks = 0; ks < 6; ++ks) af[mi][ks] = *reinterpret_cast<const bf16x8_t*>(a.w + ((mi * 16 + fr) * 24 + ks * 4 + fg) * 8);
-
-  __bf16* lut = cout;
+  float bv[4][4];
+#pragma unroll
+  for (int mi = 0; mi < 4; ++mi)
+#pragma unroll
+    for (int e = 0; e < 4; ++e) bv[mi][e] = a.bias[mi * 16 + fg * 4 + e];
   for (int i = tid; i < 3 * 256; i += 256) lut[i] = (__bf16)(((float)(i & 255) - a.mean[i >> 8]) / a.stdv[i >> 8]);
+
   constexpr int PER_THREAD = (3 * ST_PT + 4) / 5;
   const int px = tid % 48, r0 = tid / 48;
-  const int ix = ix0 + px;
-  const bool colok = tid < 240 && px < ST_PT && (unsigned)ix < (unsigned)W;
-  auto irsrc = __builtin_amdgcn_make_buffer_rsrc(const_cast<uint8_t*>(img), 0, (uint32_t)(3 * H * W), 0x00020000);
   uint8_t raw[PER_THREAD];
-#pragma unroll
-  for (int j = 0; j < PER_THREAD; ++j) {
-    const int t = r0 + 5 * j;
-    const int c = t >= 2 * ST_PT ? 2 : (t >= ST_PT ? 1 : 0), py = t - c * ST_PT;
-    const int iy = iy0 + py;
-    const bool ok = colok && t < 3 * ST_PT && (unsigned)iy < (unsigned)H;
-    raw[j] = __builtin_amdgcn_raw_buffer_load_b8(irsrc, ok ? (uint32_t)((c * H + iy) * W + ix) : SOD_OOB, 0, 0);
+  uint32_t rawok = 0;
+  auto tile_of = [&](uint32_t t, int& n, int& ty, int& tx) {
+    n = (int)fd_div(t, a.div_img);
+    const uint32_t rem = t - (uint32_t)n * a.div_img.d;
+    ty = (int)fd_div(rem, a.div_tx);
+    tx = (int)(rem - (uint32_t)ty * (uint32_t)a.tiles_x);
+  };
+  auto request = [&](uint32_t t) {
+    const bool live = t < a.ntiles;
+    int n, ty, tx;
+    tile_of(live ? t : 0u, n, ty, tx);
+    const int H = a.H[n], W = a.W[n];
+    const int iy0 = 32 * ty - 5, ix0 = 32 * tx - 5;
+    const int ix = ix0 + px;
+    const bool colok = live && tid < 240 && px < ST_PT && (unsigned)ix < (unsigned)W;
+    auto irsrc = __builtin_amdgcn_make_buffer_rsrc(const_cast<uint8_t*>(a.img[n]), 0, (uint32_t)(3 * H * W), 0x00020000);
+    rawok = 0;
+#pragma unroll
+    for (int j = 0; j < PER_THREAD; ++j) {
+      const int pr = r0 + 5 * j;
+      const int c = pr >= 2 * ST_PT ? 2 : (pr >= ST_PT ? 1 : 0), py = pr - c * ST_PT;
+      const int iy = iy0 + py;
+      const bool ok = colok && pr < 3 * ST_PT && (unsigned)iy < (unsigned)H;
+      raw[j] = __builtin_amdgcn_raw_buffer_load_b8(irsrc, ok ? (uint32_t)((c * H + iy) * W + ix) : SOD_OOB, 0, 0);
+      rawok |= ok ? (1u << j) : 0u;
+    }
+  };
+  auto convert = [&](__bf16* patch) {
+#pragma unroll
+    for (int j = 0; j < PER_THREAD; ++j) {
+      const int pr = r0 + 5 * j;
+      if (tid < 240 && pr < 3 * ST_PT) {
+        const int c = pr >= 2 * ST_PT ? 2 : (pr >= ST_PT ? 1 : 0);
+        const __bf16 v = lut[(c << 8) + raw[j]];
+        patch[pr * ST_PSTR + px] = ((rawok >> j) & 1u) ? v : (__bf16)0.f;
+      }
+    }
+  };
+
+  request(first);
+  __syncthreads();
+  convert(reinterpret_cast<__bf16*>(smem + ST_LUT_BYTES));
+  int buf = 0;
+  for (uint32_t t = first; t < a.ntiles; t += G) {
+    int n, ty, tx;
+    tile_of(t, n, ty, tx);
+    const int cy0 = 16 * ty - 1, cx0 = 16 * tx - 1;
+    const __bf16* patch = reinterpret_cast<const __bf16*>(smem + ST_LUT_BYTES + buf * ST_PATCH_BYTES);
+    request(t + G);
+    __syncthreads();
+
+    for (int nt = wave; nt < (ST_NPX + 15) / 16; nt += 4) {
+      const int cpx = nt * 16 + fr;
+      const int pc = cpx < ST_NPX ? cpx : ST_NPX - 1;
+      const int cy = pc / ST_CT, cx = pc - cy * ST_CT;
+      f32x4_t acc[4];
+#pragma unroll
+      for (int mi = 0; mi < 4; ++mi) acc[mi] = f32x4_t{0.f, 0.f, 0.f, 0.f};
+#pragma unroll
+      for (int ks = 0; ks < 6; ++ks) {
+        const int kc = ks * 4 + fg;
+        bf16x8_t bf;
+        if (kc < 21) {
+          const int c = kc / 7, r = kc - c * 7;
+          const uint32_t* src = reinterpret_cast<const uint32_t*>(patch + (c * ST_PT + 2 * cy + r) * ST_PSTR + 2 * cx);
+          typedef __attribute__((ext_vector_type(4))) unsigned int u4;
+          const u4 rawb = {src[0], src[1], src[2], src[3]};
+          bf = __builtin_bit_cast(bf16x8_t, rawb);
+        } else {
+#pragma unroll
+          for (int e = 0; e < 8; ++e) bf[e] = (__bf16)0.f;
+        }
+#pragma unroll
+        for (int mi = 0; mi < 4; ++mi) acc[mi] = __builtin_amdgcn_mfma_f32_16x16x32_bf16(af[mi][ks], bf, acc[mi], 0, 0, 0);
+      }
+      if (cpx < ST_NPX) {
+#pragma unroll
+        for (int mi = 0; mi < 4; ++mi) {
+          bf16x4_t o;
+#pragma unroll
+          for (int e = 0; e < 4; ++e) o[e] = (__bf16)fmaxf(acc[mi][e] + bv[mi][e], 0.f);
+          *reinterpret_cast<bf16x4_t*>(cout + cpx * ST_OSTR + mi * 16 + fg * 4) = o;
+        }
+      }
+    }
+    buf ^= 1;
+    convert(reinterpret_cast<__bf16*>(smem + ST_LUT_BYTES + buf * ST_PATCH_BYTES));
+    __syncthreads();
+
+    for (int item = tid; item < 64 * 8; item += 256) {
+      const int ch = item & 7, pp = item >> 3;
+      const int py = pp >> 3, pxx = pp & 7;
+      const int gy = ty * 8 + py, gx = tx * 8 + pxx;
+      if (gy >= a.Hq || gx >= a.Wq) continue;
+      float m[8];
+#pragma unroll
+      for (int e = 0; e < 8; ++e) m[e] = -3.0e38f;
+#pragma unroll
+      for (int dy = 0; dy < 3; ++dy) {
+        const int ly = 2 * py + dy;
+        if ((unsigned)(cy0 + ly) >= (unsigned)a.Hc) continue;
+#pragma unroll
+        for (int dx = 0; dx < 3; ++dx) {
+          const int lx = 2 * pxx + dx;
+          if ((unsigned)(cx0 + lx) >= (unsigned)a.Wc) continue;
+          const bf16x8_t v = *reinterpret_cast<const bf16x8_t*>(cout + (ly * ST_CT + lx) * ST_OSTR + ch * 8);
+#pragma unroll
+          for (int e = 0; e < 8; ++e) m[e] = fmaxf(m[e], (float)v[e]);
+        }
+      }
+      bf16x8_t o;
+#pragma unroll
+      for (int e = 0; e < 8; ++e) o[e] = (__bf16)m[e];
+      *reinterpret_cast<bf16x8_t*>(a.out + (((long long)n * a.Hq + gy) * a.Wq + gx) * 64 + ch * 8) = o;
+    }
   }
-  __syncthreads();
-#pragma unroll
-  for (int j = 0; j < PER_THREAD; ++j) {
-    const int t = r0 + 5 * j;
-    if (tid < 240 && t < 3 * ST_PT) {
-      const int c = t >= 2 * ST_PT ? 2 : (t >= ST_PT ? 1 : 0), py = t - c * ST_PT;
-      const bool ok = colok && (unsigned)(iy0 + py) < (unsigned)H;
-      const __bf16 v = lut[(c << 8) + raw[j]];
-      patch[t * ST_PSTR + px] = ok ? v : (__bf16)0.f;
-    }
-  }
-  __syncthreads();
-
-  float bv[4][4];
-#pragma unroll
-  for (int mi = 0; mi < 4; ++mi)
-#pragma unroll
-    for (int e = 0; e < 4; ++e) bv[mi][e] = a.bias[mi * 16 + fg * 4 + e];
-  for (int nt = wave; nt < (ST_NPX + 15) / 16; nt += 4) {
-    const int px = nt * 16 + fr;
-    const int pc = px < ST_NPX ? px : ST_NPX - 1;
-    const int cy = pc / ST_CT, cx = pc - cy * ST_CT;
-    f32x4_t acc[4];
-#pragma unroll
-    for (int mi = 0; mi < 4; ++mi) acc[mi] = f32x4_t{0.f, 0.f, 0.f, 0.f};
-#pragma unroll
-    for (int ks = 0; ks < 6; ++ks) {
-      const int kc = ks * 4 + fg;
-      bf16x8_t bf;
-      if (kc < 21) {
-        const int c = kc / 7, r = kc - c * 7;
-        const uint32_t* src = reinterpret_cast<const uint32_t*>(patch + (c * ST_PT + 2 * cy + r) * ST_PSTR + 2 * cx);
-        typedef __attribute__((ext_vector_type(4))) unsigned int u4;
-        const u4 raw = {src[0], src[1], src[2], src[3]};
-        bf = __builtin_bit_cast(bf16x8_t, raw);
-      } else {
-#pragma unroll
-        for (int e = 0; e < 8; ++e) bf[e] = (__bf16)0.f;
-      }
-#pragma unroll
-      for (int mi = 0; mi < 4; ++mi) acc[mi] = __builtin_amdgcn_mfma_f32_16x16x32_bf16(af[mi][ks], bf, acc[mi], 0, 0, 0);
-    }
-    if (px < ST_NPX) {
-#pragma unroll
-      for (int mi = 0; mi < 4; ++mi) {
-        bf16x4_t o;
-#pragma unroll
-        for (int e = 0; e < 4; ++e) o[e] = (__bf16)fmaxf(acc[mi][e] + bv[mi][e], 0.f);
-        *reinterpret_cast<bf16x4_t*>(cout + px * ST_OSTR + mi * 16 + fg * 4) = o;
-      }
-    }
-  }
-  __syncthreads();
-
-  for (int item = tid; item < 64 * 8; item += 256) {
-    const int ch = item & 7, pp = item >> 3;
-    const int py = pp >> 3, pxx = pp & 7;
-    const int gy = ty * 8 + py, gx = tx * 8 + pxx;
-    if (gy >= a.Hq || gx >= a.Wq) continue;
-    float m[8];
-#pragma unroll
-    for (int e = 0; e < 8; ++e) m[e] = -3.0e38f;
-#pragma unroll
-    for (int dy = 0; dy < 3; ++dy) {
-      const int ly = 2 * py + dy;
-      if ((unsigned)(cy0 + ly) >= (unsigned)a.Hc) continue;
-#pragma unroll
-      for (int dx = 0; dx < 3; ++dx) {
-        const int lx = 2 * pxx + dx;
-        if ((unsigned)(cx0 + lx) >= (unsigned)a.Wc) continue;
-        const bf16x8_t v = *reinterpret_cast<const bf16x8_t*>(cout + (ly * ST_CT + lx) * ST_OSTR + ch * 8);
-#pragma unroll
-        for (int e = 0; e < 8; ++e) m[e] = fmaxf(m[e], (float)v[e]);
-      }
-    }
-    bf16x8_t o;
-#pragma unroll
-    for (int e = 0; e < 8; ++e) o[e] = (__bf16)m[e];
-    *reinterpret_cast<bf16x8_t*>(a.out + (((long long)n * a.Hq + gy) * a.Wq + gx) * 64 + ch * 8) = o;
-  }
-}
-
+}
+
+}
+
+extern "C" int sod_stem_set_max_workgroups(int n) {
+  if (n < 0) return SOD_EARG;
+  g_max_workgroups.store(n, std::memory_order_relaxed);
+  return SOD_OK;
 }
 
 extern "C" int sod_stem_fused(int n, const void* const* imgs, const int* H, const int* W, const void* w_packed, const float* bias,
@@ -154,9 +193,19 @@
   a.Hc = (Hp + 6 - 7) / 2 + 1; a.Wc = (Wp + 6 - 7) / 2 + 1;
   a.Hq = (a.Hc + 2 - 3) / 2 + 1; a.Wq = (a.Wc + 2 - 3) / 2 + 1;
   for (int c = 0; c < 3; ++c) { a.mean[c] = mean3[c]; a.stdv[c] = std3[c]; }
+  const int tiles_y = (a.Hq + 7) / 8;
+  a.tiles_x = (a.Wq + 7) / 8;
+  const long long ntiles = (long long)n * tiles_y * a.tiles_x;
+  if (ntiles >= (1ll << 31)) return SOD_ESIZE;
+  a.ntiles = (uint32_t)ntiles;
+  a.div_img = make_fastdiv((uint32_t)(tiles_y * a.tiles_x)); a.div_tx = make_fastdiv((uint32_t)a.tiles_x);
   const hipError_t e = sod_max_dynamic_lds_once<stem_fused_kernel>(ST_LDS);
   if (e != hipSuccess) return (int)e;
-  SOD_LAUNCH(stem_fused_kernel, dim3((a.Wq + 7) / 8, (a.Hq + 7) / 8, n), dim3(256), ST_LDS, (hipStream_t)stream, a);
+  long long grid = (long long)ST_WG_PER_CU * device_cus();
+  const int cap = g_max_workgroups.load(std::memory_order_relaxed);
+  if (cap > 0 && grid > cap) grid = cap;
+  if (grid > ntiles) grid = ntiles;
+  SOD_LAUNCH(stem_fused_kernel, dim3((unsigned)grid), dim3(256), ST_LDS, (hipStream_t)stream, a);
   SOD_CHECK_LAUNCH();
   return SOD_OK;
 }
diff --git a/slenderobjdet_amd/layers/functional.py b/slenderobjdet_amd/layers/functional.py
--- a/slenderobjdet_amd/layers/functional.py
+++ b/slenderobjdet_amd/layers/functional.py
@@ -123,10 +123,36 @@
 HOLD_HEAD_WGRAD = os.environ.get("SOD_HOLD_HEAD_WGRAD", "1") != "0"
 _held = []
 
+WGRAD_GROUP = os.environ.get("SOD_WGRAD_GROUP", "1") != "0"
+WGRAD_GROUP_MAX = 8
+
+
+class HeldWgrad:
+    __slots__ = ("dys", "xs", "dw", "key", "run", "after")
+
+    def __init__(self, dys, xs, dw, ksize, stride, pad, dil, run, after):
+        self.dys, self.xs, self.dw, self.run, self.after = list(dys), list(xs), dw, run, after
+        self.key = _wgrad_group_key(self.dys, self.xs, dw, ksize, stride, pad, dil)
+
+
+def _wgrad_group_key(dys, xs, dw, ksize, stride, pad, dil):
+    if (ksize, stride, pad, dil) != (3, 1, 1, 1) or len(dys) != len(xs) or not xs or len(xs) > 6:
+        return None
+    N, C, K = xs[0].shape[0], xs[0].shape[-1], dys[0].shape[-1]
+    if C % 64 or K % 8 or K < 128 or dw.dtype != torch.float32 or tuple(dw.shape) != (K, 3, 3, C):
+        return None
+    for dy, x in zip(dys, xs):
+        if (dy.dtype != torch.bfloat16 or x.dtype != torch.bfloat16 or x.dim() != 4 or x.shape[0] != N or x.shape[3] != C or x.shape[2] > 190
+                or tuple(dy.shape) != tuple(x.shape[:3]) + (K,) or not dy.is_contiguous() or not x.is_contiguous()):
+            return None
+    return (dw.device.index, N, tuple((x.shape[1], x.shape[2]) for x in xs), C, K)
+
 
 def hold_or_call(fn):
     if HOLD_HEAD_WGRAD and _side_join_queued_or_in_backward():
         _held.append(fn)
+    elif isinstance(fn, HeldWgrad):
+        fn.run()
     else:
         fn()
 
@@ -147,8 +173,28 @@
     if _held:
         items = list(_held)
         _held.clear()
-        for fn in items:
-            fn()
+        group = WGRAD_GROUP and not DETERMINISTIC and not is_f32()
+        i = 0
+        while i < len(items):
+            it = items[i]
+            if not isinstance(it, HeldWgrad):
+                it()
+                i += 1
+                continue
+            j = i + 1
+            if group and it.key is not None:
+                _, _, _, C, K = it.key
+                cap = min(WGRAD_GROUP_MAX, _device_cus(it.dw.device) // (((K + 127) // 128) * (C // 64)))
+                while j < len(items) and j - i < cap and isinstance(items[j], HeldWgrad) and items[j].key == it.key:
+                    j += 1
+            if j - i >= 2:
+                conv2d_wgrad_ml_batch([(r.dys, r.xs, r.dw) for r in items[i:j]])
+                for r in items[i:j]:
+                    r.after()
+            else:
+                it.run()
+                j = i + 1
+            i = j
 
 
 def drop_held():
@@ -486,6 +532,42 @@
     return dw
 
 
+_cus_cache = {}
+
+
+def _device_cus(device):
+    n = _cus_cache.get(device.index)
+    if n is None:
+        n = _cus_cache[device.index] = int(torch.cuda.get_device_properties(device).multi_processor_count)
+    return n
+
+
+def conv2d_wgrad_ml_batch(problems):
+    dys0, xs0, dw0 = problems[0]
+    N, C, K = xs0[0].shape[0], xs0[0].shape[3], dys0[0].shape[-1]
+    hs, ws_ = [x.shape[1] for x in xs0], [x.shape[2] for x in xs0]
+    nl = len(xs0)
+    for dys, xs, dw in problems:
+        _chk(dw, torch.float32, "dw")
+        if len(dys) != nl or len(xs) != nl or tuple(dw.shape) != (K, 3, 3, C):
+            raise _C.SlenderHipError("conv2d_wgrad_ml_batch: the problems must share one geometry")
+        for dy, x, h, w in zip(dys, xs, hs, ws_):
+            _chk(dy, torch.bfloat16, "dy"); _chk(x, torch.bfloat16, "x")
+            if tuple(x.shape) != (N, h, w, C) or tuple(dy.shape) != (N, h, w, K):
+                raise _C.SlenderHipError("conv2d_wgrad_ml_batch: the problems must share one geometry")
+    if _batch_defer(lambda: conv2d_wgrad_ml_batch(problems)):
+        return
+    all_dys = [t for dys, _, _ in problems for t in dys]
+    all_xs = [t for _, xs, _ in problems for t in xs]
+    side = _wgrad_stream(dw0.device, all_dys + all_xs, dw0.data_ptr())
+    ws = wgrad_workspace(dw0.device, side)
+    e0 = _prof_begin(side, "conv_wgrad")
+    call("sod_conv2d_wgrad_ml_batch", len(problems), nl, _ptr_arr(all_dys), _ptr_arr(all_xs), _ptr_arr([dw for _, _, dw in problems]),
+         N, _int_arr(hs), _int_arr(ws_), C, K, ptr(ws), ws.numel(), stream_ptr(side))
+    fl = len(problems) * sum(2.0 * N * h * w * K * 9 * C for h, w in zip(hs, ws_))
+    _prof_end("conv_wgrad", fl, e0, ("ml", N * len(problems), tuple(hs), C, K, 3, 1, tuple(ws_)), side)
+
+
 def weight_prep(w_master, scale=None, want_krsc=True, want_crsk=True, cpad=None):
     _chk(w_master, torch.float32, "w"); _chk(scale, torch.float32, "scale")
     K, R, S, C = w_master.shape
diff --git a/slenderobjdet_amd/layers/nn.py b/slenderobjdet_amd/layers/nn.py
--- a/slenderobjdet_amd/layers/nn.py
+++ b/slenderobjdet_amd/layers/nn.py
@@ -424,10 +424,13 @@
         arena.mark_ready(gn.bias)
         if conv.bias is not None:
             arena.mark_ready(conv.bias)
+        dw = arena.grad_view(conv.weight)
+        def after():
+            arena.mark_ready(conv.weight)
         def wgrad():
-            HF.conv2d_wgrad_ml(dy1s, list(xs), arena.grad_view(conv.weight), k, k, conv.stride, conv.padding, conv.dilation)
-            arena.mark_ready(conv.weight)
-        HF.hold_or_call(wgrad)
+            HF.conv2d_wgrad_ml(dy1s, list(xs), dw, k, k, conv.stride, conv.padding, conv.dilation)
+            after()
+        HF.hold_or_call(HF.HeldWgrad(dy1s, xs, dw, k, conv.stride, conv.padding, conv.dilation, wgrad, after))
         dxs = [None] * nl
         if any(ctx.needs_input_grad[3:]):
             fold, ctx.fold = ctx.fold, None
@@ -501,13 +504,17 @@
             gs = [dy.contiguous() for dy in dys]
         else:
             gs = [HF.relu_bwd(dy.contiguous(), y) for dy, y in zip(dys, ys)]
-        def wgrad():
+        dw = arena.grad_view(conv.weight)
+        def after():
             with HF.wgrad_batch():
-                HF.conv2d_wgrad_ml(gs, list(xs), arena.grad_view(conv.weight), 3, 3, 1, 1, 1)
                 arena.mark_ready(conv.weight)
                 HF.bias_grad_ml(gs, arena.grad_view(conv.bias))
                 arena.mark_ready(conv.bias)
-        HF.hold_or_call(wgrad)
+        def wgrad():
+            with HF.wgrad_batch():
+                HF.conv2d_wgrad_ml(gs, list(xs), dw, 3, 3, 1, 1, 1)
+                after()
+        HF.hold_or_call(HF.HeldWgrad(gs, xs, dw, 3, 1, 1, 1, wgrad, after))
         dxs = [None] * nl
         if any(ctx.needs_input_grad[3:]):
             hw = [(x.shape[1], x.shape[2]) for x in xs]
```

Measured after the change: 667.4 img/s. No clear change (-0.2%).
